# ben-hayes/neural-waveshaping-synthesis

Hardware: AMD Instinct MI355X
Metric: audio_samples_per_sec (higher is better)
Workload: dtype f32 (fp16x2-split MFMA contractions = 22-bit products, fp32 accumulate; FiLM interpolation bf16x3-split MFMA = exact fp32 operands); 1 GPU; NEWT forward, vn checkpoint, FastNEWT LUT, batch 64/GPU x 500 frames (4 s @ 16 kHz), torch.rand F0/control, RNG draws on device; batch_per_gpu=64, frames=500, samples_per_utterance=64000, parallelism=batch-shard x1, exciter_opts=0, streams=2

## Files before the change

### include/nws_hip.h

```cpp
#ifndef NWS_HIP_H
#define NWS_HIP_H

#include <stddef.h>
#include <stdint.h>

#ifdef __cplusplus
extern "C" {
#endif

#define NWS_ABI_VERSION 6

#define NWS_N_HARMONICS 101
#define NWS_N_SHAPERS 64
#define NWS_HIDDEN 128
#define NWS_HOP 128
#define NWS_FIR_LEN 256
#define NWS_N_BANDS 129
#define NWS_FIR_HALF 128
#define NWS_SHAPER_WIDTH 8
#define NWS_FILM_CH 256

enum {
  NWS_OK = 0,
  NWS_ERR_UNSUPPORTED = -1,
  NWS_ERR_BAD_ARG = -2,
  NWS_ERR_WORKSPACE = -3
};

typedef struct NwsWeights {
  const float* gru_w_ih;
  const float* gru_w_hh;
  const float* gru_b_ih;
  const float* gru_b_hh;
  const float* proj_w;
  const float* proj_b;
  const float* mixer_w;
  const float* mixer_b;
  const void* mixer_frags;
  const float* newt_mlp_w[4];
  const float* newt_mlp_b[4];
  const float* newt_ln_g[3];
  const float* newt_ln_b[3];
  const float* hgen_w[4];
  const float* hgen_b[4];
  const float* hgen_ln_g[3];
  const float* hgen_ln_b[3];
  const void* mlp_frags;
  const float* shaper_in_scale;
  const float* shaper_w0;
  const float* shaper_b0;
  const float* shaper_w2;
  const float* shaper_b2;
  const float* shaper_w4;
  const float* shaper_b4;
  const float* shaper_w6;
  const float* shaper_b6;
  const float* shaper_turns;
  const float* lut;
  const float* lut_pairs;
  int32_t lut_size;
  float lut_min;
  float lut_max;
  const float* newt_out_w;
  const float* newt_out_b;
  const float* noise_window;
  int32_t exciter_opts;
  const float* exciter_bound;
} NwsWeights;
#define NWS_EXCITER_VALU_FILM 1
#define NWS_EXCITER_ONE_TERM 2
#define NWS_EXCITER_HYBRID 4
#define NWS_EXCITER_HYBRID_W 8
#define NWS_EXCITER_BANK_NOFRACT 16

int nws_abi_version(void);
size_t nws_sizeof(int which);
const char* nws_error_string(int code);

int nws_selftest_mfma(int32_t* bad_out , void* stream);

int nws_sin(const float* x, float* y, int64_t n, void* stream);

int nws_phase_carry(const float* f0, const float* f0_up, int B, int T, double* carry , void* stream);

int nws_exciter_newt(const NwsWeights* w, const float* f0, const float* f0_up, const double* carry,
                     const float* phase_u, const float* rand_phase, const float* film, int B, int T,
                     float sample_rate, float* exciter_out, float* newt_out, void* stream);
int nws_exciter_newt_add(const NwsWeights* w, const float* f0, const float* f0_up, const double* carry,
                         const float* phase_u, const float* rand_phase, const float* film, const float* add_in, int B,
                         int T, float sample_rate, float* exciter_out, float* newt_out, void* stream);

int nws_control_gru(const NwsWeights* w, const float* control, int B, int C, int T, float* gru_out, void* stream);
int nws_control_gru_state(const NwsWeights* w, const float* control, int B, int C, int T, const float* h0, float* gru_out,
                          float* hT, void* stream);
int nws_control_gru_carry(const NwsWeights* w, const float* control, const float* f0, int B, int C, int T, float* gru_out,
                          double* carry_out, void* stream);
int nws_control_gru_batched(const NwsWeights* w, const float* control, int B, int C, int T, const float* h0, float* gru_out,
                            float* hT, void* stream);

int nws_frame_mlps(const NwsWeights* w, const float* gru_out, const float* fir_design, int B, int T,
                   float* emb_out, float* film_out, float* H_out, float* fir_out, void* stream);

#define NWS_MLP_FRAGS_BYTES 1474560
int nws_mlp_frags(const NwsWeights* w, const float* fir_design , void* frags_out, void* stream);

int nws_fir_design_matrix(const float* window , float* D_out, void* stream);

int nws_fir_noise(const float* fir , const float* noise , const float* add_in ,
                  int B, int T, float* out , void* stream);
int nws_fir_noise_window(const float* fir, const float* noise, int noise_len, int origin, const float* add_in, int B, int T,
                         float* out, void* stream);

int nws_fir_noise_grad(const float* noise , const float* grad_out , int B, int T,
                       float* grad_fir , void* stream);
int nws_fir_from_h_grad(const float* grad_fir , const float* fir_design , int B, int T,
                        float* grad_H , void* stream);
int nws_sum_batch_time(const float* x , int B, int C, int T, float* out , void* stream);

typedef struct NwsReverbPlan {
  int32_t L;
  int32_t N1;
  int32_t N2;
  int32_t Lc;
  int32_t hist;
  int32_t nblk;
  int32_t reserved[2];
} NwsReverbPlan;

int nws_reverb_plan(int N, int ir_len_plus1, NwsReverbPlan* plan );
int nws_reverb_plan_serves(const NwsReverbPlan* plan, int N, int ir_len_plus1);
size_t nws_reverb_table_bytes(const NwsReverbPlan* plan);
size_t nws_reverb_spectrum_bytes(const NwsReverbPlan* plan);
size_t nws_reverb_workspace_bytes(const NwsReverbPlan* plan, int B);
int nws_reverb_build_tables(const NwsReverbPlan* plan, void* tables, void* stream);
int nws_reverb_ir_spectrum(const NwsReverbPlan* plan, const void* tables, const float* ir, int ir_len,
                           void* spectrum, void* workspace, size_t workspace_bytes, void* stream);
int nws_reverb(const NwsReverbPlan* plan, const void* tables, const void* spectrum, const float* x ,
               int B, int N, float* y , void* workspace, size_t workspace_bytes, void* stream);

size_t nws_reverb_grad_workspace_bytes(const NwsReverbPlan* plan, int B, int want_ir);
int nws_reverb_grad_x(const NwsReverbPlan* plan, const void* tables, const void* spectrum, const float* g ,
                      int B, int N, float* dx , void* workspace, size_t workspace_bytes, void* stream);
int nws_reverb_grad_ir(const NwsReverbPlan* plan, const void* tables, const float* x , const float* g ,
                       int B, int N, int ir_len, float* dir , void* workspace, size_t workspace_bytes,
                       void* stream);

int nws_reverb_linear_chunk(const NwsReverbPlan* plan, const void* tables, const void* spectrum, const float* x, int B, int M,
                            const float* tail_in, float* tail_out, int tail_len, float* y, void* workspace,
                            size_t workspace_bytes, void* stream);

size_t nws_stream_state_bytes(int B, int max_frames, int ir_len, const NwsReverbPlan* plan);
int nws_stream_reset(void* state, size_t state_bytes, void* stream);
int nws_stream_out_samples(int K, int first, int final);
long long nws_stream_noise_start(int first, long long frames_seen);
int nws_stream_noise_draws(int K, int first, long long frames_seen);
int nws_stream_step(const NwsWeights* w, const float* fir_design, const NwsReverbPlan* plan, const void* reverb_tables,
                    const void* reverb_spectrum, void* state, size_t state_bytes, int B, int max_frames, const float* f0 ,
                    const float* control , int C, int K, int first, int final, long long frames_seen,
                    long long nz_prev_start, float sample_rate, const float* phase_u, const float* rand_phase,
                    const float* noise_new, const float* noise_all, int noise_all_len, const float* ir, int ir_len,
                    float* out , float* pre_out , void* stream);
int nws_stream_reverb_tail(const NwsReverbPlan* plan, const void* reverb_tables, const void* reverb_spectrum, void* state,
                           size_t state_bytes, int B, int max_frames, int ir_len, float* tail_out ,
                           void* workspace, size_t workspace_bytes, void* stream);

size_t nws_stream_counters_offset(int B, int max_frames, int ir_len);
size_t nws_stream_slot_state_bytes(int B, int max_frames, int ir_len);
#define NWS_SLOT_START 1
#define NWS_SLOT_STOP 2
#define NWS_SLOT_RELEASE 4
#define NWS_SLOT_ACTIVE 8
int nws_stream_step_slots(const NwsWeights* w, const float* fir_design, void* state, size_t state_bytes, int B, int max_frames,
                          const float* f0 , const float* control , int C, int K, long long frames_seen,
                          long long nz_prev_start, float sample_rate, const float* phase_u, const float* rand_phase,
                          const float* noise_new, const float* noise_all, int noise_all_len, const float* ir, int ir_len,
                          const int* events , float* out , float* pre_out ,
                          void* stream);

int nws_oscillator(const float* f0_up, const double* carry, const float* phase_u, const float* rand_phase, int B, int N,
                   float sample_rate, float* out, void* stream);
int nws_newt_apply(const NwsWeights* w, const float* exciter, const float* film, int B, int T, float* out, void* stream);
int nws_td_mlp(const float* x, int B, int in_size, int hidden, int out_size, int depth, int T, const float* const* w,
               const float* const* b, const float* const* ln_g, const float* const* ln_b, float ln_eps, float leaky_slope,
               float* y, void* stream);
int nws_td_layer_norm(const float* x, const float* gain, const float* bias, int B, int C, int T, float eps, float* y,
                      void* stream);
int nws_film(const float* x, const float* gamma, const float* beta, int64_t n, float* y, void* stream);
int nws_fir_from_h(const float* H, const float* fir_design , int B, int T, float* fir_out, void* stream);

int nws_shaper_table(const NwsWeights* w, int table_size, float table_min, float table_max, float* table_out, void* stream);

#define NWS_MIXER_FRAGS_BYTES 28672
int nws_mixer_frags(const float* mixer_w, const float* mixer_b, void* frags_out, void* stream);
int nws_exciter_bound(const float* mixer_w, const float* mixer_b, float* bound_out , void* stream);
#define NWS_SHAPER_TURNS_ROW 176
int nws_shaper_turns(const NwsWeights* w, float* table_out , void* stream);

int nws_lut_pairs(const float* table , int table_size, float* pairs_out , void* stream);

int nws_shaper_apply(const NwsWeights* w, const float* x, int64_t B, int64_t N, float* y, void* stream);

typedef struct NwsForwardAux {
  const float* fir_design;
  const NwsReverbPlan* plan;
  const void* reverb_tables;
  const void* reverb_spectrum;
} NwsForwardAux;

size_t nws_forward_workspace_bytes(const NwsReverbPlan* plan, int B, int T);
int nws_forward(const NwsWeights* w, const NwsForwardAux* aux, const float* f0 , const float* control ,
                int B, int C, int T, float sample_rate, const float* phase_u, const float* rand_phase,
                const float* noise, float* out , void* workspace, size_t workspace_bytes, void* stream);

size_t nws_forward_control_bytes(int B, int T);
int nws_forward_control(const NwsWeights* w, const float* f0, const float* control, int B, int C, int T, int batched_gru,
                        void* workspace, size_t workspace_bytes, void* stream);
int nws_forward_audio(const NwsWeights* w, const NwsForwardAux* aux, const float* f0, int B, int T, float sample_rate,
                      const float* phase_u, const float* rand_phase, const float* noise, float* out, void* workspace,
                      size_t workspace_bytes, void* stream);

int nws_forward_audio_ev(const NwsWeights* w, const NwsForwardAux* aux, const float* f0, int B, int T, float sample_rate,
                         const float* phase_u, const float* rand_phase, const float* noise, float* out, void* workspace,
                         size_t workspace_bytes, void* stream, void* wait_before_exciter, void* record_after_exciter);

int nws_forward_audio_pre(const NwsWeights* w, const NwsForwardAux* aux, const float* f0, int B, int T, float sample_rate,
                          const float* phase_u, const float* rand_phase, const float* noise, void* workspace,
                          size_t workspace_bytes, void* stream);
int nws_forward_reverb_rows(const NwsForwardAux* aux, int B, int T, int row0, int nrows, float* out, void* workspace,
                            size_t workspace_bytes, void* stream);
int nws_forward_audio_blocks(const NwsWeights* w, const NwsForwardAux* aux, const float* f0, int B, int T, float sample_rate,
                             const float* phase_u, const float* rand_phase, const float* noise, float* out, void* workspace,
                             size_t workspace_bytes, void* stream, const int32_t* row0, const int32_t* nrows,
                             void* const* events , int nblocks);

size_t nws_loudness_dft_bytes(int n_fft);
int nws_loudness_dft_matrix(int n_fft, float* dft_out, void* stream);
int nws_loudness_frames(int N, int hop);
size_t nws_loudness_workspace_bytes(int B, int N, int n_fft, int hop);
int nws_loudness(const float* audio, int B, int N, int n_fft, int hop, const float* dft, float amin, float top_db,
                 int normalise, float* out, void* workspace, size_t workspace_bytes, void* stream);

int nws_pyin_frames(int N, int hop);
int nws_pyin_dims(double sample_rate, double fmin, double fmax, int frame_length, int hop, int32_t* dims);
size_t nws_pyin_table_bytes(double sample_rate, double fmin, double fmax, int frame_length, int hop);
int nws_pyin_table(double sample_rate, double fmin, double fmax, int frame_length, int hop, double* table_host);
size_t nws_pyin_workspace_bytes(int B, int N, double sample_rate, double fmin, double fmax, int frame_length, int hop);
int nws_pyin_cmnd(const float* audio, int B, int N, double sample_rate, double fmin, double fmax, int frame_length, int hop,
                  float* yin, void* stream);
int nws_pyin_observe(const float* yin, int B, int T, double sample_rate, double fmin, double fmax, int frame_length, int hop,
                     const double* table, int* cand_bin, double* cand_prob, int* count, double* voiced_prob, void* stream);
int nws_pyin_viterbi(const int* cand_bin, const double* cand_prob, const int* count, const double* voiced_prob, int B, int T,
                     double sample_rate, double fmin, double fmax, int frame_length, int hop, const double* table,
                     int fill_unvoiced, float fill_value, int* states, float* f0, void* workspace, size_t workspace_bytes,
                     void* stream);
int nws_pyin(const float* audio, int B, int N, double sample_rate, double fmin, double fmax, int frame_length, int hop,
             const double* table, int fill_unvoiced, float fill_value, float* f0, double* voiced_prob, int* states,
             void* workspace, size_t workspace_bytes, void* stream);

int nws_resample_dims(int sr_in, int sr_out, int32_t* dims);
int64_t nws_resample_length(int64_t N, int sr_in, int sr_out);
size_t nws_resample_bank_bytes(int sr_in, int sr_out);
int nws_resample_bank(int sr_in, int sr_out, float* bank_host);
int nws_resample(const float* x, int B, int N, int sr_in, int sr_out, const float* bank_dev, float* y, void* stream);

int nws_mfcc_dims(double sample_rate, int n_fft, int n_mfcc, int n_mels, int32_t* dims);
size_t nws_mfcc_table_bytes(double sample_rate, int n_fft, int n_mfcc, int n_mels);
int nws_mfcc_table(double sample_rate, int n_fft, int n_mfcc, int n_mels, float* table_host);
size_t nws_mfcc_workspace_bytes(int B, int N, int n_fft, int hop, int n_mels);
int nws_mfcc(const float* audio, int B, int N, double sample_rate, int n_fft, int hop, int n_mfcc, int n_mels, const float* dft,
             const float* table, float* out, void* workspace, size_t workspace_bytes, void* stream);

#define NWS_STFT_LOSS_MAX_RES 8
size_t nws_stft_loss_dft_bytes(int n_fft, int win_length);
int nws_stft_loss_dft_matrix(int n_fft, int win_length, float* dft_out, void* stream);
size_t nws_stft_loss_workspace_bytes(int B, int N, int R, const int* n_ffts, const int* hops);
int nws_stft_loss(const float* x, const float* y, int B, int N, int R, const int* n_ffts, const int* hops, const int* win_lengths,
                  const float* const* dfts, float w_sc, float w_log_mag, float w_lin_mag, float eps, float* out, void* workspace,
                  size_t workspace_bytes, void* stream);

size_t nws_stft_grad_workspace_bytes(int B, int N, int R, const int* n_ffts, const int* hops, const int* win_lengths);
int nws_stft_grad(const float* x, const float* y, int B, int N, int R, const int* n_ffts, const int* hops, const int* win_lengths,
                  const float* const* dfts, float w_sc, float w_log_mag, float w_lin_mag, float eps, float* grad_out, void* workspace,
                  size_t workspace_bytes, void* stream);

typedef struct NwsShaperDesc {
  int32_t n_shapers, width, depth, lut_size;
  float lut_min, lut_max;
  const float* in_scale;
  const float* w[8];
  const float* b[8];
  const float* lut;
} NwsShaperDesc;

typedef struct NwsGenericModel {
  int32_t control_size;
  int32_t gru_hidden, embedding, n_harmonics, n_shapers;
  int32_t hop;
  int32_t newt_mlp_depth;
  int32_t hgen_depth, hgen_hidden;
  int32_t fir_len;
  int32_t out_channels;
  int32_t ir_len;
  float ln_eps, leaky_slope;
  const float *gru_w_ih, *gru_w_hh, *gru_b_ih, *gru_b_hh;
  const float *proj_w, *proj_b;
  const float *mixer_w, *mixer_b;
  const float* newt_mlp_w[8];
  const float* newt_mlp_b[8];
  const float* newt_ln_g[8];
  const float* newt_ln_b[8];
  const float* hgen_w[8];
  const float* hgen_b[8];
  const float* hgen_ln_g[8];
  const float* hgen_ln_b[8];
  const float *newt_out_w, *newt_out_b;
  const float* noise_window;
  const float* ir;
  NwsShaperDesc shaper;
} NwsGenericModel;

size_t nws_g_gru_workspace_bytes(int hidden);
int nws_g_gru(const float* w_ih, const float* w_hh, const float* b_ih, const float* b_hh, const float* control, int B,
              int C_total, int C_in, int hidden, int T, const float* h0, float* out, float* hT, void* workspace,
              size_t workspace_bytes, void* stream);
int nws_g_bth_to_bht(const float* x, int B, int T, int H, float* y, void* stream);
int nws_g_phase(const float* f0, const float* f0_up, int B, int T, int hop, float sample_rate, float* f0_up_out,
                float* phase_out, void* stream);
int nws_g_upsample(const float* x, int64_t rows, int T, int hop, float* y, void* stream);
int nws_g_oscillator(const float* f0_up, const float* phase, const float* phase_u, const float* rand_phase, int K, int B, int N,
                     float sample_rate, float* out, void* stream);
int nws_g_conv1x1(const float* x, const float* w, const float* bias, int B, int Cin, int Cout, int N, float* y, void* stream);
int nws_g_shaper_apply(const NwsShaperDesc* d, const float* x, int64_t rows, int64_t N, float* y, void* stream);
int nws_g_shaper_table(const NwsShaperDesc* d, int table_size, float table_min, float table_max, float* table_out, void* stream);
int nws_g_film_shaper(const NwsShaperDesc* d, const float* exciter, const float* film, int B, int T, int hop, float* out,
                      void* stream);
int nws_g_fir_design(const float* H, const float* window, int fir_len, int B, int T, float* fir_out, void* stream);
int nws_g_fir_noise(const float* fir, const float* noise, int fir_len, int hop, int B, int T, const float* add_in,
                    int add_channels, float* out, void* stream);
int nws_g_reverb_direct(const float* x, const float* ir, int ir_len, int B, int N, float* y, void* stream);

size_t nws_forward_generic_workspace_bytes(const NwsGenericModel* m, int B, int T);
int nws_forward_generic(const NwsGenericModel* m, const float* f0, const float* control, int B, int C, int T, float sample_rate,
                        const float* phase_u, const float* rand_phase, const float* noise, const NwsReverbPlan* plan,
                        const void* reverb_tables, const void* reverb_spectrum, void* reverb_workspace,
                        size_t reverb_workspace_bytes, float* out, void* workspace, size_t workspace_bytes, void* stream);


#define NWS_N_STAGES 6
int nws_profile_begin(int slots, unsigned stage_mask);
int nws_profile_collect(float* ms_out , int* n_out );
int nws_profile_end(void);

int nws_peer_push(int n, void* const* dst, const void* src, size_t bytes, void* const* streams, void* const* events);
int nws_events_wait(int n, void* const* events);
int nws_streams_wait(int n, void* const* streams);

int nws_queue_probe(void* stream_hold, void* stream_touch, int groups, int spin_us, unsigned long long* scratch, float* frac_out );

#ifdef __cplusplus
}
#endif
#endif
```

### neural-waveshaping-synthesis_amd/_cops.py

```python
from __future__ import annotations

import ctypes as C

import torch

from . import _lib
from ._lib import NwsForwardAux, NwsGenericModel, NwsReverbPlan, NwsShaperDesc, NwsWeights, check, ptr

HOP = _lib.HOP


def _stream(dev):
    return torch.cuda.current_stream(dev).cuda_stream


def _struct(desc: torch.Tensor, cls):
    return cls.from_buffer_copy(desc.numpy())


def _plan(plan: torch.Tensor | None):
    return NwsReverbPlan(*plan.tolist()[:6]) if plan is not None else None


def _ref(struct):
    return C.byref(struct) if struct is not None else None


def _aux(fir_design, plan, tables, spectrum) -> NwsForwardAux:
    aux = NwsForwardAux()
    aux.fir_design = ptr(fir_design)
    aux.plan = C.pointer(_plan(plan))
    aux.reverb_tables = ptr(tables)
    aux.reverb_spectrum = ptr(spectrum)
    return aux


def _new(like: torch.Tensor, *shape, dtype=torch.float32):
    return torch.empty(shape, dtype=dtype, device=like.device)


def _ptrs(tensors):
    return (C.c_void_p * max(1, len(tensors)))(*[t.data_ptr() for t in tensors])


def _pyin_dims(cfg, table=None):
    dims = (C.c_int32 * 8)()
    L = _lib.lib()
    if L.nws_pyin_dims(*cfg, dims) != 0:
        raise RuntimeError(f"pyin: unsupported configuration (sample_rate, fmin, fmax, frame_length, hop) = {cfg}: at most 512 "
                           "lags (frame_length <= 1024), 1024 pitch bins and a transition window of 127; hop <= frame_length")
    n = L.nws_pyin_table_bytes(*cfg) // 8
    if isinstance(table, torch.Tensor) and (not table.is_cuda or table.dtype != torch.float64 or table.numel() != n):
        raise RuntimeError("pyin: table does not belong to this configuration (expected a float64 CUDA tensor of nws_pyin_table)")
    return (*dims, n)


def _resample_dims(sr_in, sr_out):
    dims = (C.c_int32 * 6)()
    if not (1 <= sr_in < 2 ** 31 and 1 <= sr_out < 2 ** 31) or _lib.lib().nws_resample_dims(sr_in, sr_out, dims) != 0:
        raise RuntimeError(f"resample: unsupported rates {sr_in} -> {sr_out}: integers >= 1 whose weight bank (sr_out / gcd rows) "
                           "stays below 64 MB")
    return tuple(dims)


def _mfcc_dims(sample_rate, n_fft, n_mfcc, n_mels):
    dims = (C.c_int32 * 8)()
    ok = all(0 <= v < 2 ** 31 for v in (n_fft, n_mfcc, n_mels))
    if not ok or _lib.lib().nws_mfcc_dims(sample_rate, n_fft, n_mfcc, n_mels, dims) != 0:
        raise RuntimeError(f"mfcc: unsupported configuration (sample_rate {sample_rate}, n_fft {n_fft}, n_mfcc {n_mfcc}, n_mels "
                           f"{n_mels}): sample_rate > 0, n_fft a power of two in [64, 2048], 1 <= n_mfcc <= n_mels <= 1024")
    return tuple(dims)


class CtypesOps:
    def abi_version(self):
        return int(_lib.lib().nws_abi_version())

    def forward(self, wdesc, f0, control, phase_u, rand_phase, noise, fir_design, plan, reverb_tables, reverb_spectrum,
                workspace, sample_rate):
        B, Cc, T = control.shape
        aux = _aux(fir_design, plan, reverb_tables, reverb_spectrum)
        with torch.cuda.device(f0.device):
            out = _new(f0, B, T * HOP)
            check(_lib.lib().nws_forward(C.byref(_struct(wdesc, NwsWeights)), C.byref(aux), ptr(f0), ptr(control), B, Cc, T,
                                         sample_rate, ptr(phase_u), ptr(rand_phase), ptr(noise), ptr(out), ptr(workspace),
                                         workspace.numel(), _stream(f0.device)), "nws_forward")
        return out

    def forward_control(self, wdesc, f0, control, workspace, batched_gru):
        B, Cc, T = control.shape
        with torch.cuda.device(f0.device):
            check(_lib.lib().nws_forward_control(C.byref(_struct(wdesc, NwsWeights)), ptr(f0), ptr(control), B, Cc, T,
                                                 1 if batched_gru else 0, ptr(workspace), workspace.numel(), _stream(f0.device)),
                  "nws_forward_control")

    def forward_audio(self, wdesc, f0, phase_u, rand_phase, noise, fir_design, plan, reverb_tables, reverb_spectrum, workspace,
                      sample_rate, out, wait_event, record_event):
        B, _, T = f0.shape
        aux = _aux(fir_design, plan, reverb_tables, reverb_spectrum)
        with torch.cuda.device(f0.device):
            if out is None:
                out = _new(f0, B, T * HOP)
            check(_lib.lib().nws_forward_audio_ev(C.byref(_struct(wdesc, NwsWeights)), C.byref(aux), ptr(f0), B, T, sample_rate,
                                                  ptr(phase_u), ptr(rand_phase), ptr(noise), ptr(out), ptr(workspace),
                                                  workspace.numel(), _stream(f0.device), wait_event or None, record_event or None),
                  "nws_forward_audio_ev")
        return out

    def forward_audio_pre(self, wdesc, f0, phase_u, rand_phase, noise, fir_design, plan, reverb_tables, reverb_spectrum,
                          workspace, sample_rate):
        B, _, T = f0.shape
        aux = _aux(fir_design, plan, reverb_tables, reverb_spectrum)
        with torch.cuda.device(f0.device):
            check(_lib.lib().nws_forward_audio_pre(C.byref(_struct(wdesc, NwsWeights)), C.byref(aux), ptr(f0), B, T, sample_rate,
                                                   ptr(phase_u), ptr(rand_phase), ptr(noise), ptr(workspace), workspace.numel(),
                                                   _stream(f0.device)), "nws_forward_audio_pre")

    def forward_audio_blocks(self, wdesc, f0, phase_u, rand_phase, noise, fir_design, plan, reverb_tables, reverb_spectrum,
                             workspace, sample_rate, out, row0, nrows, events):
        B, _, T = f0.shape
        n = len(row0)
        aux = _aux(fir_design, plan, reverb_tables, reverb_spectrum)
        with torch.cuda.device(f0.device):
            check(_lib.lib().nws_forward_audio_blocks(C.byref(_struct(wdesc, NwsWeights)), C.byref(aux), ptr(f0), B, T, sample_rate,
                                                      ptr(phase_u), ptr(rand_phase), ptr(noise), ptr(out), ptr(workspace),
                                                      workspace.numel(), _stream(f0.device), (C.c_int32 * n)(*row0),
                                                      (C.c_int32 * n)(*nrows), (C.c_void_p * n)(*events) if events else None, n),
                  "nws_forward_audio_blocks")

    def forward_reverb_rows(self, fir_design, plan, reverb_tables, reverb_spectrum, workspace, T, row0, nrows, out):
        aux = _aux(fir_design, plan, reverb_tables, reverb_spectrum)
        with torch.cuda.device(out.device):
            check(_lib.lib().nws_forward_reverb_rows(C.byref(aux), out.shape[0], T, row0, nrows, ptr(out), ptr(workspace),
                                                     workspace.numel(), _stream(out.device)), "nws_forward_reverb_rows")

    def phase_carry(self, f0, f0_up):
        src = f0 if f0 is not None else f0_up
        B = src.shape[0]
        T = src.shape[-1] if f0 is not None else src.shape[-1] // HOP
        with torch.cuda.device(src.device):
            carry = _new(src, B, T * HOP // 32, dtype=torch.float64)
            check(_lib.lib().nws_phase_carry(ptr(f0), ptr(f0_up), B, T, ptr(carry), _stream(src.device)), "nws_phase_carry")
        return carry

    def exciter_newt(self, wdesc, f0, f0_up, carry, phase_u, rand_phase, film, sample_rate, want_exciter, want_newt):
        src = f0 if f0 is not None else f0_up
        B = src.shape[0]
        T = src.shape[-1] if f0 is not None else src.shape[-1] // HOP
        with torch.cuda.device(src.device):
            exc = _new(src, B, _lib.N_SHAPERS, T * HOP) if want_exciter else None
            out = _new(src, B, T * HOP) if want_newt else None
            check(_lib.lib().nws_exciter_newt(C.byref(_struct(wdesc, NwsWeights)), ptr(f0), ptr(f0_up), ptr(carry), ptr(phase_u),
                                              ptr(rand_phase), ptr(film), B, T, sample_rate, ptr(exc), ptr(out),
                                              _stream(src.device)), "nws_exciter_newt")
        return exc, out

    def oscillator(self, f0_up, phase_u, rand_phase, sample_rate):
        B, N = f0_up.shape
        with torch.cuda.device(f0_up.device):
            st = _stream(f0_up.device)
            carry = _new(f0_up, B, N // 32, dtype=torch.float64)
            out = _new(f0_up, B, _lib.N_HARMONICS, N)
            check(_lib.lib().nws_phase_carry(None, ptr(f0_up), B, N // HOP, ptr(carry), st), "nws_phase_carry")
            check(_lib.lib().nws_oscillator(ptr(f0_up), ptr(carry), ptr(phase_u), ptr(rand_phase), B, N, sample_rate, ptr(out), st),
                  "nws_oscillator")
        return out

    def control_gru(self, wdesc, control, h0, batched):
        B, Cc, T = control.shape
        fn = _lib.lib().nws_control_gru_batched if batched else _lib.lib().nws_control_gru_state
        with torch.cuda.device(control.device):
            out = _new(control, B, T, _lib.HIDDEN)
            hT = _new(control, B, _lib.HIDDEN)
            check(fn(C.byref(_struct(wdesc, NwsWeights)), ptr(control), B, Cc, T, ptr(h0), ptr(out), ptr(hT),
                     _stream(control.device)), "nws_control_gru")
        return out, hT

    def frame_mlps(self, wdesc, gru_out, fir_design, want_emb, want_H):
        B, T, _ = gru_out.shape
        with torch.cuda.device(gru_out.device):
            emb = _new(gru_out, B, _lib.HIDDEN, T) if want_emb else None
            film = _new(gru_out, B, T, _lib.FILM_CH)
            H = _new(gru_out, B, T, _lib.N_BANDS) if want_H else None
            fir = _new(gru_out, B, T, _lib.FIR_HALF)
            check(_lib.lib().nws_frame_mlps(C.byref(_struct(wdesc, NwsWeights)), ptr(gru_out), ptr(fir_design), B, T, ptr(emb),
                                            ptr(film), ptr(H), ptr(fir), _stream(gru_out.device)), "nws_frame_mlps")
        return emb, film, H, fir

    def fir_noise(self, fir, noise, add_in, origin):
        B, T, _ = fir.shape
        with torch.cuda.device(fir.device):
            out = _new(fir, B, T * HOP)
            if origin < 0:
                check(_lib.lib().nws_fir_noise(ptr(fir), ptr(noise), ptr(add_in), B, T, ptr(out), _stream(fir.device)), "nws_fir_noise")
            else:
                check(_lib.lib().nws_fir_noise_window(ptr(fir), ptr(noise), noise.numel(), origin, ptr(add_in), B, T, ptr(out),
                                                      _stream(fir.device)), "nws_fir_noise_window")
        return out

    def fir_from_h(self, H, fir_design):
        B, _, T = H.shape
        with torch.cuda.device(H.device):
            fir = _new(H, B, T, _lib.FIR_HALF)
            check(_lib.lib().nws_fir_from_h(ptr(H), ptr(fir_design), B, T, ptr(fir), _stream(H.device)), "nws_fir_from_h")
        return fir

    def fir_noise_grad(self, noise, grad_out):
        B, N = grad_out.shape
        T = N // HOP
        if N != T * HOP or T < 2 or noise.numel() != N - 1:
            raise RuntimeError(f"fir_noise_grad: grad_out {tuple(grad_out.shape)} must be (B, 128 T) with T >= 2 and noise "
                               f"{tuple(noise.shape)} its {N - 1} samples")
        with torch.cuda.device(grad_out.device):
            grad_fir = _new(grad_out, B, T, _lib.FIR_HALF)
            check(_lib.lib().nws_fir_noise_grad(ptr(noise), ptr(grad_out), B, T, ptr(grad_fir), _stream(grad_out.device)),
                  "nws_fir_noise_grad")
        return grad_fir

    def fir_from_h_grad(self, grad_fir, fir_design):
        B, T, _ = grad_fir.shape
        with torch.cuda.device(grad_fir.device):
            grad_H = _new(grad_fir, B, _lib.N_BANDS, T)
            check(_lib.lib().nws_fir_from_h_grad(ptr(grad_fir), ptr(fir_design), B, T, ptr(grad_H), _stream(grad_fir.device)),
                  "nws_fir_from_h_grad")
        return grad_H

    def sum_batch_time(self, x):
        B, Cc, T = x.shape
        with torch.cuda.device(x.device):
            out = _new(x, Cc)
            check(_lib.lib().nws_sum_batch_time(ptr(x), B, Cc, T, ptr(out), _stream(x.device)), "nws_sum_batch_time")
        return out

    def reverb(self, plan, tables, spectrum, x):
        B, N = x.shape
        p = _plan(plan)
        with torch.cuda.device(x.device):
            nbytes = _lib.lib().nws_reverb_workspace_bytes(C.byref(p), B)
            ws = _new(x, nbytes, dtype=torch.uint8)
            y = torch.empty_like(x)
            check(_lib.lib().nws_reverb(C.byref(p), ptr(tables), ptr(spectrum), ptr(x), B, N, ptr(y), ptr(ws), nbytes,
                                        _stream(x.device)), "nws_reverb")
        return y

    def reverb_grad_x(self, plan, tables, spectrum, grad_out):
        B, N = grad_out.shape
        p = _plan(plan)
        with torch.cuda.device(grad_out.device):
            nbytes = _lib.lib().nws_reverb_grad_workspace_bytes(C.byref(p), B, 0)
            ws = _new(grad_out, nbytes, dtype=torch.uint8)
            dx = torch.empty_like(grad_out)
            check(_lib.lib().nws_reverb_grad_x(C.byref(p), ptr(tables), ptr(spectrum), ptr(grad_out), B, N, ptr(dx), ptr(ws), nbytes,
                                               _stream(grad_out.device)), "nws_reverb_grad_x")
        return dx

    def reverb_grad_ir(self, plan, tables, x, grad_out, ir_len):
        B, N = x.shape
        if tuple(grad_out.shape) != (B, N):
            raise RuntimeError(f"reverb_grad_ir: x {tuple(x.shape)} and grad_out {tuple(grad_out.shape)} differ in shape")
        p = _plan(plan)
        with torch.cuda.device(x.device):
            nbytes = _lib.lib().nws_reverb_grad_workspace_bytes(C.byref(p), B, 1)
            ws = _new(x, nbytes, dtype=torch.uint8)
            dir_ = _new(x, ir_len)
            check(_lib.lib().nws_reverb_grad_ir(C.byref(p), ptr(tables), ptr(x), ptr(grad_out), B, N, ir_len, ptr(dir_), ptr(ws),
                                                nbytes, _stream(x.device)), "nws_reverb_grad_ir")
        return dir_

    def reverb_linear_chunk(self, plan, tables, spectrum, x, tail_in):
        B, M = x.shape
        p = _plan(plan)
        with torch.cuda.device(x.device):
            nfl = (2 * ((B + 1) // 2) + B) * p.L
            ws = _new(x, nfl)
            y, tail_out = torch.empty_like(x), torch.empty_like(tail_in)
            check(_lib.lib().nws_reverb_linear_chunk(C.byref(p), ptr(tables), ptr(spectrum), ptr(x), B, M, ptr(tail_in),
                                                     ptr(tail_out), tail_in.shape[1], ptr(y), ptr(ws), nfl * 4, _stream(x.device)),
                  "nws_reverb_linear_chunk")
        return y, tail_out

    def shaper_apply(self, wdesc, x):
        with torch.cuda.device(x.device):
            y = torch.empty_like(x)
            check(_lib.lib().nws_shaper_apply(C.byref(_struct(wdesc, NwsWeights)), ptr(x), x.shape[0], x.shape[2], ptr(y),
                                              _stream(x.device)), "nws_shaper_apply")
        return y

    def shaper_table(self, wdesc, like, size, tmin, tmax):
        with torch.cuda.device(like.device):
            table = _new(like, _lib.N_SHAPERS, size)
            check(_lib.lib().nws_shaper_table(C.byref(_struct(wdesc, NwsWeights)), size, tmin, tmax, ptr(table), _stream(like.device)),
                  "nws_shaper_table")
        return table

    def newt_apply(self, wdesc, exciter, film):
        B, _, N = exciter.shape
        T = film.shape[2]
        if film.shape[1] != _lib.FILM_CH or N != T * HOP:
            raise RuntimeError(f"NEWT: exciter {tuple(exciter.shape)} and FiLM parameters {tuple(film.shape)} disagree")
        with torch.cuda.device(exciter.device):
            out = _new(exciter, B, 1, N)
            check(_lib.lib().nws_newt_apply(C.byref(_struct(wdesc, NwsWeights)), ptr(exciter), ptr(film), B, T, ptr(out),
                                            _stream(exciter.device)), "nws_newt_apply")
        return out

    def td_mlp(self, x, weights, biases, ln_w, ln_b, eps, slope):
        B, in_size, T = x.shape
        hidden, out_size = weights[0].shape[0], weights[-1].shape[0]
        with torch.cuda.device(x.device):
            y = _new(x, B, out_size, T)
            check(_lib.lib().nws_td_mlp(ptr(x), B, in_size, hidden, out_size, len(weights), T, _ptrs(weights), _ptrs(biases),
                                        _ptrs(ln_w), _ptrs(ln_b), eps, slope, ptr(y), _stream(x.device)), "nws_td_mlp")
        return y

    def td_layer_norm(self, x, weight, bias, eps):
        with torch.cuda.device(x.device):
            y = torch.empty_like(x)
            check(_lib.lib().nws_td_layer_norm(ptr(x), ptr(weight), ptr(bias), x.shape[0], x.shape[1], x.shape[2], eps, ptr(y),
                                               _stream(x.device)), "nws_td_layer_norm")
        return y

    def film(self, x, gamma, beta):
        with torch.cuda.device(x.device):
            y = torch.empty_like(x)
            check(_lib.lib().nws_film(ptr(x), ptr(gamma), ptr(beta), x.numel(), ptr(y), _stream(x.device)), "nws_film")
        return y

    def sine(self, x):
        with torch.cuda.device(x.device):
            y = torch.empty_like(x)
            check(_lib.lib().nws_sin(ptr(x), ptr(y), x.numel(), _stream(x.device)), "nws_sin")
        return y

    def loudness(self, audio, dft, n_fft, hop, amin, top_db, normalise):
        B, N = audio.shape
        L = _lib.lib()
        with torch.cuda.device(audio.device):
            ws = _new(audio, L.nws_loudness_workspace_bytes(B, N, n_fft, hop), dtype=torch.uint8)
            out = _new(audio, B, L.nws_loudness_frames(N, hop))
            check(L.nws_loudness(ptr(audio), B, N, n_fft, hop, ptr(dft), amin, top_db, 1 if normalise else 0, ptr(out), ptr(ws),
                                 ws.numel(), _stream(audio.device)), "nws_loudness")
        return out

    def pyin_table(self, sample_rate, fmin, fmax, frame_length, hop):
        cfg = (sample_rate, fmin, fmax, frame_length, hop)
        table = torch.empty(_pyin_dims(cfg)[8], dtype=torch.float64)
        check(_lib.lib().nws_pyin_table(*cfg, table.data_ptr()), "nws_pyin_table")
        return table

    def pyin_cmnd(self, audio, sample_rate, fmin, fmax, frame_length, hop):
# ... 297 lines not shown
```

### neural-waveshaping-synthesis_amd/_lib.py

```python
from __future__ import annotations

import ctypes as C
import os

_HERE = os.path.dirname(os.path.abspath(__file__))
LIB_PATH = os.path.join(_HERE, "libnws_hip.so")

PROBE_LIB_PATH = os.path.join(_HERE, "libnws_probe.so")

ABI_VERSION = 6
EXCITER_VALU_FILM = 1
EXCITER_ONE_TERM = 2
EXCITER_HYBRID = 4
EXCITER_HYBRID_W = 8
EXCITER_BANK_NOFRACT = 16
N_HARMONICS = 101
N_SHAPERS = 64
HIDDEN = 128
HOP = 128
FIR_LEN = 256
FIR_HALF = 128
MLP_FRAGS_BYTES = 1474560
N_BANDS = 129
FILM_CH = 256
SHAPER_WIDTH = 8
SHAPER_TURNS_ROW = 176
FIR_DESIGN_COLS = 132

_fp = C.c_void_p


class NwsWeights(C.Structure):
    _fields_ = [
        ("gru_w_ih", _fp), ("gru_w_hh", _fp), ("gru_b_ih", _fp), ("gru_b_hh", _fp),
        ("proj_w", _fp), ("proj_b", _fp),
        ("mixer_w", _fp), ("mixer_b", _fp), ("mixer_frags", _fp),
        ("newt_mlp_w", _fp * 4), ("newt_mlp_b", _fp * 4), ("newt_ln_g", _fp * 3), ("newt_ln_b", _fp * 3),
        ("hgen_w", _fp * 4), ("hgen_b", _fp * 4), ("hgen_ln_g", _fp * 3), ("hgen_ln_b", _fp * 3),
        ("mlp_frags", _fp),
        ("shaper_in_scale", _fp),
        ("shaper_w0", _fp), ("shaper_b0", _fp), ("shaper_w2", _fp), ("shaper_b2", _fp),
        ("shaper_w4", _fp), ("shaper_b4", _fp), ("shaper_w6", _fp), ("shaper_b6", _fp), ("shaper_turns", _fp),
        ("lut", _fp), ("lut_pairs", _fp), ("lut_size", C.c_int32), ("lut_min", C.c_float), ("lut_max", C.c_float),
        ("newt_out_w", _fp), ("newt_out_b", _fp),
        ("noise_window", _fp),
        ("exciter_opts", C.c_int32),
        ("exciter_bound", _fp),
    ]


class NwsReverbPlan(C.Structure):
    _fields_ = [("L", C.c_int32), ("N1", C.c_int32), ("N2", C.c_int32), ("Lc", C.c_int32), ("hist", C.c_int32), ("nblk", C.c_int32),
                ("reserved", C.c_int32 * 2)]

    def as_tensor(self):
        import torch
        return torch.tensor([self.L, self.N1, self.N2, self.Lc, self.hist, self.nblk, 0, 0], dtype=torch.int32)


class NwsForwardAux(C.Structure):
    _fields_ = [("fir_design", _fp), ("plan", C.POINTER(NwsReverbPlan)), ("reverb_tables", _fp),
                ("reverb_spectrum", _fp)]


class NwsShaperDesc(C.Structure):
    _fields_ = [("n_shapers", C.c_int32), ("width", C.c_int32), ("depth", C.c_int32), ("lut_size", C.c_int32),
                ("lut_min", C.c_float), ("lut_max", C.c_float),
                ("in_scale", _fp), ("w", _fp * 8), ("b", _fp * 8), ("lut", _fp)]


class NwsGenericModel(C.Structure):
    _fields_ = [("control_size", C.c_int32), ("gru_hidden", C.c_int32), ("embedding", C.c_int32), ("n_harmonics", C.c_int32),
                ("n_shapers", C.c_int32), ("hop", C.c_int32), ("newt_mlp_depth", C.c_int32), ("hgen_depth", C.c_int32),
                ("hgen_hidden", C.c_int32), ("fir_len", C.c_int32), ("out_channels", C.c_int32), ("ir_len", C.c_int32),
                ("ln_eps", C.c_float), ("leaky_slope", C.c_float),
                ("gru_w_ih", _fp), ("gru_w_hh", _fp), ("gru_b_ih", _fp), ("gru_b_hh", _fp),
                ("proj_w", _fp), ("proj_b", _fp), ("mixer_w", _fp), ("mixer_b", _fp),
                ("newt_mlp_w", _fp * 8), ("newt_mlp_b", _fp * 8), ("newt_ln_g", _fp * 8), ("newt_ln_b", _fp * 8),
                ("hgen_w", _fp * 8), ("hgen_b", _fp * 8), ("hgen_ln_g", _fp * 8), ("hgen_ln_b", _fp * 8),
                ("newt_out_w", _fp), ("newt_out_b", _fp), ("noise_window", _fp), ("ir", _fp),
                ("shaper", NwsShaperDesc)]


_PYIN_CFG = (C.c_double, C.c_double, C.c_double, C.c_int, C.c_int)

_MFCC_CFG = (C.c_double, C.c_int, C.c_int, C.c_int)

_PROTOTYPES = {
    "nws_abi_version": (C.c_int, []),
    "nws_sizeof": (C.c_size_t, [C.c_int]),
    "nws_error_string": (C.c_char_p, [C.c_int]),
    "nws_selftest_mfma": (C.c_int, [_fp, _fp]),
    "nws_peer_push": (C.c_int, [C.c_int, C.POINTER(C.c_void_p), _fp, C.c_size_t, C.POINTER(C.c_void_p), C.POINTER(C.c_void_p)]),
    "nws_events_wait": (C.c_int, [C.c_int, C.POINTER(C.c_void_p)]),
    "nws_streams_wait": (C.c_int, [C.c_int, C.POINTER(C.c_void_p)]),
    "nws_queue_probe": (C.c_int, [_fp, _fp, C.c_int, C.c_int, _fp, C.POINTER(C.c_float)]),
    "nws_debug_queue_busy": (C.c_int, [C.c_int, C.c_int, _fp, _fp]),
    "nws_sin": (C.c_int, [_fp, _fp, C.c_int64, _fp]),
    "nws_phase_carry": (C.c_int, [_fp, _fp, C.c_int, C.c_int, _fp, _fp]),
    "nws_exciter_newt": (C.c_int, [C.POINTER(NwsWeights), _fp, _fp, _fp, _fp, _fp, _fp, C.c_int, C.c_int, C.c_float,
                                   _fp, _fp, _fp]),
    "nws_exciter_newt_add": (C.c_int, [C.POINTER(NwsWeights), _fp, _fp, _fp, _fp, _fp, _fp, _fp, C.c_int, C.c_int, C.c_float,
                                       _fp, _fp, _fp]),
    "nws_control_gru": (C.c_int, [C.POINTER(NwsWeights), _fp, C.c_int, C.c_int, C.c_int, _fp, _fp]),
    "nws_control_gru_state": (C.c_int, [C.POINTER(NwsWeights), _fp, C.c_int, C.c_int, C.c_int, _fp, _fp, _fp, _fp]),
    "nws_control_gru_carry": (C.c_int, [C.POINTER(NwsWeights), _fp, _fp, C.c_int, C.c_int, C.c_int, _fp, _fp, _fp]),
    "nws_control_gru_batched": (C.c_int, [C.POINTER(NwsWeights), _fp, C.c_int, C.c_int, C.c_int, _fp, _fp, _fp, _fp]),
    "nws_frame_mlps": (C.c_int, [C.POINTER(NwsWeights), _fp, _fp, C.c_int, C.c_int, _fp, _fp, _fp, _fp, _fp]),
    "nws_mlp_frags": (C.c_int, [C.POINTER(NwsWeights), _fp, _fp, _fp]),
    "nws_debug_frame_mlps_kernel": (C.c_int, [C.c_int]),
    "nws_fir_design_matrix": (C.c_int, [_fp, _fp, _fp]),
    "nws_fir_noise": (C.c_int, [_fp, _fp, _fp, C.c_int, C.c_int, _fp, _fp]),
    "nws_fir_noise_window": (C.c_int, [_fp, _fp, C.c_int, C.c_int, _fp, C.c_int, C.c_int, _fp, _fp]),
    "nws_fir_noise_grad": (C.c_int, [_fp, _fp, C.c_int, C.c_int, _fp, _fp]),
    "nws_fir_from_h_grad": (C.c_int, [_fp, _fp, C.c_int, C.c_int, _fp, _fp]),
    "nws_sum_batch_time": (C.c_int, [_fp, C.c_int, C.c_int, C.c_int, _fp, _fp]),
    "nws_reverb_linear_chunk": (C.c_int, [C.POINTER(NwsReverbPlan), _fp, _fp, _fp, C.c_int, C.c_int, _fp, _fp, C.c_int, _fp, _fp,
                                          C.c_size_t, _fp]),
    "nws_reverb_plan": (C.c_int, [C.c_int, C.c_int, C.POINTER(NwsReverbPlan)]),
    "nws_reverb_plan_serves": (C.c_int, [C.POINTER(NwsReverbPlan), C.c_int, C.c_int]),
    "nws_reverb_table_bytes": (C.c_size_t, [C.POINTER(NwsReverbPlan)]),
    "nws_reverb_spectrum_bytes": (C.c_size_t, [C.POINTER(NwsReverbPlan)]),
    "nws_reverb_workspace_bytes": (C.c_size_t, [C.POINTER(NwsReverbPlan), C.c_int]),
    "nws_reverb_build_tables": (C.c_int, [C.POINTER(NwsReverbPlan), _fp, _fp]),
    "nws_reverb_ir_spectrum": (C.c_int, [C.POINTER(NwsReverbPlan), _fp, _fp, C.c_int, _fp, _fp, C.c_size_t, _fp]),
    "nws_reverb": (C.c_int, [C.POINTER(NwsReverbPlan), _fp, _fp, _fp, C.c_int, C.c_int, _fp, _fp, C.c_size_t, _fp]),
    "nws_reverb_grad_workspace_bytes": (C.c_size_t, [C.POINTER(NwsReverbPlan), C.c_int, C.c_int]),
    "nws_reverb_grad_x": (C.c_int, [C.POINTER(NwsReverbPlan), _fp, _fp, _fp, C.c_int, C.c_int, _fp, _fp, C.c_size_t, _fp]),
    "nws_reverb_grad_ir": (C.c_int, [C.POINTER(NwsReverbPlan), _fp, _fp, _fp, C.c_int, C.c_int, C.c_int, _fp, _fp, C.c_size_t, _fp]),
    "nws_shaper_table": (C.c_int, [C.POINTER(NwsWeights), C.c_int, C.c_float, C.c_float, _fp, _fp]),
    "nws_mixer_frags": (C.c_int, [_fp, _fp, _fp, _fp]),
    "nws_exciter_bound": (C.c_int, [_fp, _fp, _fp, _fp]),
    "nws_shaper_turns": (C.c_int, [_fp, _fp, _fp]),
    "nws_lut_pairs": (C.c_int, [_fp, C.c_int, _fp, _fp]),
    "nws_shaper_apply": (C.c_int, [C.POINTER(NwsWeights), _fp, C.c_int64, C.c_int64, _fp, _fp]),
    "nws_forward_workspace_bytes": (C.c_size_t, [C.POINTER(NwsReverbPlan), C.c_int, C.c_int]),
    "nws_forward": (C.c_int, [C.POINTER(NwsWeights), C.POINTER(NwsForwardAux), _fp, _fp, C.c_int, C.c_int, C.c_int,
                              C.c_float, _fp, _fp, _fp, _fp, _fp, C.c_size_t, _fp]),
    "nws_forward_control_bytes": (C.c_size_t, [C.c_int, C.c_int]),
    "nws_forward_control": (C.c_int, [C.POINTER(NwsWeights), _fp, _fp, C.c_int, C.c_int, C.c_int, C.c_int, _fp, C.c_size_t, _fp]),
    "nws_forward_audio": (C.c_int, [C.POINTER(NwsWeights), C.POINTER(NwsForwardAux), _fp, C.c_int, C.c_int, C.c_float,
                                    _fp, _fp, _fp, _fp, _fp, C.c_size_t, _fp]),
    "nws_forward_audio_ev": (C.c_int, [C.POINTER(NwsWeights), C.POINTER(NwsForwardAux), _fp, C.c_int, C.c_int, C.c_float,
                                       _fp, _fp, _fp, _fp, _fp, C.c_size_t, _fp, _fp, _fp]),
    "nws_forward_audio_pre": (C.c_int, [C.POINTER(NwsWeights), C.POINTER(NwsForwardAux), _fp, C.c_int, C.c_int, C.c_float,
                                        _fp, _fp, _fp, _fp, C.c_size_t, _fp]),
    "nws_forward_reverb_rows": (C.c_int, [C.POINTER(NwsForwardAux), C.c_int, C.c_int, C.c_int, C.c_int, _fp, _fp, C.c_size_t, _fp]),
    "nws_forward_audio_blocks": (C.c_int, [C.POINTER(NwsWeights), C.POINTER(NwsForwardAux), _fp, C.c_int, C.c_int, C.c_float, _fp, _fp, _fp, _fp,
                                           _fp, C.c_size_t, _fp, C.POINTER(C.c_int32), C.POINTER(C.c_int32), C.POINTER(C.c_void_p), C.c_int]),
    "nws_loudness_dft_bytes": (C.c_size_t, [C.c_int]),
    "nws_loudness_dft_matrix": (C.c_int, [C.c_int, _fp, _fp]),
    "nws_loudness_frames": (C.c_int, [C.c_int, C.c_int]),
    "nws_loudness_workspace_bytes": (C.c_size_t, [C.c_int, C.c_int, C.c_int, C.c_int]),
    "nws_loudness": (C.c_int, [_fp, C.c_int, C.c_int, C.c_int, C.c_int, _fp, C.c_float, C.c_float, C.c_int, _fp, _fp,
                               C.c_size_t, _fp]),
    "nws_pyin_frames": (C.c_int, [C.c_int, C.c_int]),
    "nws_pyin_dims": (C.c_int, [*_PYIN_CFG, C.POINTER(C.c_int32)]),
    "nws_pyin_table_bytes": (C.c_size_t, [*_PYIN_CFG]),
    "nws_pyin_table": (C.c_int, [*_PYIN_CFG, C.c_void_p]),
    "nws_pyin_workspace_bytes": (C.c_size_t, [C.c_int, C.c_int, *_PYIN_CFG]),
    "nws_pyin_cmnd": (C.c_int, [_fp, C.c_int, C.c_int, *_PYIN_CFG, _fp, _fp]),
    "nws_pyin_observe": (C.c_int, [_fp, C.c_int, C.c_int, *_PYIN_CFG, _fp, _fp, _fp, _fp, _fp, _fp]),
    "nws_pyin_viterbi": (C.c_int, [_fp, _fp, _fp, _fp, C.c_int, C.c_int, *_PYIN_CFG, _fp, C.c_int, C.c_float, _fp, _fp, _fp,
                                   C.c_size_t, _fp]),
    "nws_pyin": (C.c_int, [_fp, C.c_int, C.c_int, *_PYIN_CFG, _fp, C.c_int, C.c_float, _fp, _fp, _fp, _fp, C.c_size_t, _fp]),
    "nws_resample_dims": (C.c_int, [C.c_int, C.c_int, C.POINTER(C.c_int32)]),
    "nws_resample_length": (C.c_int64, [C.c_int64, C.c_int, C.c_int]),
    "nws_resample_bank_bytes": (C.c_size_t, [C.c_int, C.c_int]),
    "nws_resample_bank": (C.c_int, [C.c_int, C.c_int, C.c_void_p]),
    "nws_resample": (C.c_int, [_fp, C.c_int, C.c_int, C.c_int, C.c_int, _fp, _fp, _fp]),
    "nws_mfcc_dims": (C.c_int, [*_MFCC_CFG, C.POINTER(C.c_int32)]),
    "nws_mfcc_table_bytes": (C.c_size_t, [*_MFCC_CFG]),
    "nws_mfcc_table": (C.c_int, [*_MFCC_CFG, C.c_void_p]),
    "nws_mfcc_workspace_bytes": (C.c_size_t, [C.c_int, C.c_int, C.c_int, C.c_int, C.c_int]),
    "nws_mfcc": (C.c_int, [_fp, C.c_int, C.c_int, C.c_double, C.c_int, C.c_int, C.c_int, C.c_int, _fp, _fp, _fp, _fp, C.c_size_t,
                           _fp]),
    "nws_stft_loss_dft_bytes": (C.c_size_t, [C.c_int, C.c_int]),
    "nws_stft_loss_dft_matrix": (C.c_int, [C.c_int, C.c_int, _fp, _fp]),
    "nws_stft_loss_workspace_bytes": (C.c_size_t, [C.c_int, C.c_int, C.c_int, C.POINTER(C.c_int), C.POINTER(C.c_int)]),
    "nws_stft_loss": (C.c_int, [_fp, _fp, C.c_int, C.c_int, C.c_int, C.POINTER(C.c_int), C.POINTER(C.c_int), C.POINTER(C.c_int),
                                C.POINTER(_fp), C.c_float, C.c_float, C.c_float, C.c_float, _fp, _fp, C.c_size_t, _fp]),
    "nws_stft_grad_workspace_bytes": (C.c_size_t, [C.c_int, C.c_int, C.c_int, C.POINTER(C.c_int), C.POINTER(C.c_int),
                                                   C.POINTER(C.c_int)]),
    "nws_stft_grad": (C.c_int, [_fp, _fp, C.c_int, C.c_int, C.c_int, C.POINTER(C.c_int), C.POINTER(C.c_int), C.POINTER(C.c_int),
                                C.POINTER(_fp), C.c_float, C.c_float, C.c_float, C.c_float, _fp, _fp, C.c_size_t, _fp]),
    "nws_oscillator": (C.c_int, [_fp, _fp, _fp, _fp, C.c_int, C.c_int, C.c_float, _fp, _fp]),
    "nws_newt_apply": (C.c_int, [C.POINTER(NwsWeights), _fp, _fp, C.c_int, C.c_int, _fp, _fp]),
    "nws_td_mlp": (C.c_int, [_fp, C.c_int, C.c_int, C.c_int, C.c_int, C.c_int, C.c_int, C.POINTER(_fp), C.POINTER(_fp),
                             C.POINTER(_fp), C.POINTER(_fp), C.c_float, C.c_float, _fp, _fp]),
    "nws_td_layer_norm": (C.c_int, [_fp, _fp, _fp, C.c_int, C.c_int, C.c_int, C.c_float, _fp, _fp]),
    "nws_film": (C.c_int, [_fp, _fp, _fp, C.c_int64, _fp, _fp]),
    "nws_fir_from_h": (C.c_int, [_fp, _fp, C.c_int, C.c_int, _fp, _fp]),
    "nws_g_gru_workspace_bytes": (C.c_size_t, [C.c_int]),
    "nws_g_gru": (C.c_int, [_fp, _fp, _fp, _fp, _fp, C.c_int, C.c_int, C.c_int, C.c_int, C.c_int, _fp, _fp, _fp, _fp,
                            C.c_size_t, _fp]),
    "nws_g_bth_to_bht": (C.c_int, [_fp, C.c_int, C.c_int, C.c_int, _fp, _fp]),
    "nws_g_phase": (C.c_int, [_fp, _fp, C.c_int, C.c_int, C.c_int, C.c_float, _fp, _fp, _fp]),
    "nws_g_upsample": (C.c_int, [_fp, C.c_int64, C.c_int, C.c_int, _fp, _fp]),
    "nws_g_oscillator": (C.c_int, [_fp, _fp, _fp, _fp, C.c_int, C.c_int, C.c_int, C.c_float, _fp, _fp]),
    "nws_g_conv1x1": (C.c_int, [_fp, _fp, _fp, C.c_int, C.c_int, C.c_int, C.c_int, _fp, _fp]),
    "nws_g_shaper_apply": (C.c_int, [C.POINTER(NwsShaperDesc), _fp, C.c_int64, C.c_int64, _fp, _fp]),
    "nws_g_shaper_table": (C.c_int, [C.POINTER(NwsShaperDesc), C.c_int, C.c_float, C.c_float, _fp, _fp]),
    "nws_g_film_shaper": (C.c_int, [C.POINTER(NwsShaperDesc), _fp, _fp, C.c_int, C.c_int, C.c_int, _fp, _fp]),
    "nws_g_fir_design": (C.c_int, [_fp, _fp, C.c_int, C.c_int, C.c_int, _fp, _fp]),
    "nws_g_fir_noise": (C.c_int, [_fp, _fp, C.c_int, C.c_int, C.c_int, C.c_int, _fp, C.c_int, _fp, _fp]),
    "nws_g_reverb_direct": (C.c_int, [_fp, _fp, C.c_int, C.c_int, C.c_int, _fp, _fp]),
    "nws_forward_generic_workspace_bytes": (C.c_size_t, [C.POINTER(NwsGenericModel), C.c_int, C.c_int]),
    "nws_debug_generic_exciter_plan": (C.c_int, [C.POINTER(NwsGenericModel), C.c_int, C.c_int, C.POINTER(C.c_int)]),
    "nws_debug_generic_gru_plan": (C.c_int, [C.c_int, C.c_int, C.POINTER(C.c_int)]),
    "nws_forward_generic": (C.c_int, [C.POINTER(NwsGenericModel), _fp, _fp, C.c_int, C.c_int, C.c_int, C.c_float, _fp, _fp, _fp,
                                      C.POINTER(NwsReverbPlan), _fp, _fp, _fp, C.c_size_t, _fp, _fp, C.c_size_t, _fp]),
    "nws_stream_state_bytes": (C.c_size_t, [C.c_int, C.c_int, C.c_int, C.POINTER(NwsReverbPlan)]),
    "nws_stream_reset": (C.c_int, [_fp, C.c_size_t, _fp]),
    "nws_stream_out_samples": (C.c_int, [C.c_int, C.c_int, C.c_int]),
    "nws_stream_noise_start": (C.c_longlong, [C.c_int, C.c_longlong]),
    "nws_stream_noise_draws": (C.c_int, [C.c_int, C.c_int, C.c_longlong]),
    "nws_stream_step": (C.c_int, [C.POINTER(NwsWeights), _fp, C.POINTER(NwsReverbPlan), _fp, _fp, _fp, C.c_size_t, C.c_int, C.c_int,
                                  _fp, _fp, C.c_int, C.c_int, C.c_int, C.c_int, C.c_longlong, C.c_longlong, C.c_float, _fp, _fp,
                                  _fp, _fp, C.c_int, _fp, C.c_int, _fp, _fp, _fp]),
    "nws_stream_counters_offset": (C.c_size_t, [C.c_int, C.c_int, C.c_int]),
    "nws_stream_slot_state_bytes": (C.c_size_t, [C.c_int, C.c_int, C.c_int]),
    "nws_stream_step_slots": (C.c_int, [C.POINTER(NwsWeights), _fp, _fp, C.c_size_t, C.c_int, C.c_int, _fp, _fp, C.c_int, C.c_int,
                                        C.c_longlong, C.c_longlong, C.c_float, _fp, _fp, _fp, _fp, C.c_int, _fp, C.c_int, _fp, _fp,
                                        _fp, _fp]),
    "nws_stream_reverb_tail": (C.c_int, [C.POINTER(NwsReverbPlan), _fp, _fp, _fp, C.c_size_t, C.c_int, C.c_int, C.c_int, _fp, _fp,
                                         C.c_size_t, _fp]),
    "nws_profile_begin": (C.c_int, [C.c_int, C.c_uint]),
    "nws_profile_collect": (C.c_int, [C.POINTER(C.c_float), C.POINTER(C.c_int)]),
    "nws_profile_end": (C.c_int, []),
}

_PROBE_PROTOTYPES = {
    "nws_coexec_pk_probe": (C.c_int, [C.c_int, C.c_int, _fp, _fp]),
    "nws_coexec_pk_probe2": (C.c_int, [C.c_int, C.c_int, _fp, _fp]),
    "nws_coexec_pk_probe_mixed": (C.c_int, [C.c_int, C.c_int, C.c_int, _fp, _fp, _fp]),
    "nws_coexec_mfma_load": (C.c_int, [C.c_int, C.c_int, C.c_int, _fp, _fp]),
}

STAGE_NAMES = ("phase_carry", "control_gru", "frame_mlps", "exciter_newt", "fir_noise", "reverb")

EXPORTED_SYMBOLS = tuple(_PROTOTYPES)
PROBE_SYMBOLS = tuple(_PROBE_PROTOTYPES)

_lib = None
_probe = None


class NwsError(RuntimeError):
    pass


def lib():
    global _lib
    if _lib is None:
        if not os.path.exists(LIB_PATH):
            raise NwsError(
                f"{LIB_PATH} not found: build the HIP kernels first "
                "(python __graft_entry__.py build, or python neural-waveshaping-synthesis_amd/build.py). "
                "There is no CPU/PyTorch fallback for the NEWT forward path.")
        handle = C.CDLL(LIB_PATH)
        for name, (res, args) in _PROTOTYPES.items():
            fn = getattr(handle, name)
            fn.restype = res
            fn.argtypes = args
        if handle.nws_abi_version() != ABI_VERSION:
            raise NwsError(f"{LIB_PATH} has ABI version {handle.nws_abi_version()}, this package binds version "
                           f"{ABI_VERSION}: rebuild it (python __graft_entry__.py build)")
        for which, struct in enumerate((NwsWeights, NwsReverbPlan, NwsForwardAux, NwsShaperDesc, NwsGenericModel)):
            if handle.nws_sizeof(which) != C.sizeof(struct):
                raise NwsError(f"struct layout mismatch for {struct.__name__}: library {handle.nws_sizeof(which)} B, "
                               f"binding {C.sizeof(struct)} B")
        _lib = handle
    return _lib


def probe_lib():
    global _probe
    if _probe is None:
        if not os.path.exists(PROBE_LIB_PATH):
            raise NwsError(f"{PROBE_LIB_PATH} not found: python neural-waveshaping-synthesis_amd/build.py builds it next to libnws_hip.so")
        handle = C.CDLL(PROBE_LIB_PATH)
        for name, (res, args) in _PROBE_PROTOTYPES.items():
            fn = getattr(handle, name)
            fn.restype = res
            fn.argtypes = args
        _probe = handle
    return _probe


def check(rc: int, what: str = ""):
    if rc != 0:
        msg = lib().nws_error_string(rc)
        raise NwsError(f"{what or 'nws call'} failed ({rc}): {msg.decode() if msg else '?'}")
# ... 13 lines not shown
```

### neural-waveshaping-synthesis_amd/csrc/fir_noise.hip

```cpp
#include "nws_common.h"
#include "fir_spectral_fft.h"

template <>
struct SpOps<f32x2> {
  static __device__ __forceinline__ f32x2 fma(f32x2 a, f32x2 b, f32x2 c) { return __builtin_elementwise_fma(a, b, c); }
  static __device__ __forceinline__ f32x2 of(float v) { return f32x2{v, v}; }
  static __device__ __forceinline__ f32x2 at(const float* p) { return *reinterpret_cast<const f32x2*>(p); }
};

namespace {

constexpr int kL = NWS_FIR_LEN;
constexpr int kHop = NWS_HOP;
constexpr int kHalf = NWS_FIR_HALF;
constexpr int kHopsPerBlock = 4;

struct NoiseLds {
  float taps[kHopsPerBlock + 1][kL];
  float taps1[kHopsPerBlock + 1][kL];
  float sig[(kHopsPerBlock + 1) * kHop + kHop];
};

__device__ __forceinline__ float padded_noise(const float* __restrict__ noise, int len, int origin, int i) {
  int s = i - origin;
  if (s < 0) s = -s;
  if (s > len - 1) s = 2 * (len - 1) - s;
  s = s < 0 ? 0 : s;
  return noise[s];
}

__device__ __forceinline__ float row_noise(const float* __restrict__ noise, int lo, int hi, int origin, int i) {
  int s = i - origin;
  if (s < lo) s = 2 * lo - s;
  if (s > hi) s = 2 * hi - s;
  s = s < 0 ? 0 : s;
  return noise[s];
}

template <bool ROWS>
__global__ __launch_bounds__(256) void fir_noise_kernel(const float* __restrict__ fir, const float* __restrict__ noise,
                                                        const float* __restrict__ add_in, int T, int len, int origin,
                                                        float* __restrict__ out, const int4* __restrict__ rows) {
  __shared__ __attribute__((aligned(16))) NoiseLds L;
  const int tid = threadIdx.x, lane = tid & 63, wave = tid >> 6;
  const int half = lane >> 5, q = lane & 31;
  const int b = blockIdx.y;
  const int t0 = blockIdx.x * kHopsPerBlock;
  const int N = T * kHop;
  int4 rb = make_int4(0, 0, 0, 0);
  if constexpr (ROWS) rb = rows[b];
  const int t_lo = ROWS ? rb.z : 0;

  for (int e = tid; e < (kHopsPerBlock + 1) * kL; e += 256) {
    const int fr = e >> 8, k = e & 255;
    const int t = t0 - 1 + fr;
    const int d = k >= kHalf ? k - kHalf : kHalf - k;
    const float v = (t >= t_lo && t < T && d < kHalf) ? fir[((size_t)b * T + t) * kHalf + d] : 0.0f;
    L.taps[fr][k] = v;
    L.taps1[fr][(k + 1) & 255] = v;
  }
  for (int e = tid; e < (kHopsPerBlock + 1) * kHop + kHop; e += 256) {
    const int i = (t0 - 1) * kHop + e;
    float v = 0.0f;
    if (i >= 0 && i < N + kL - 1) v = ROWS ? row_noise(noise, rb.x, rb.y, origin, i) : padded_noise(noise, len, origin, i);
    L.sig[e] = v;
  }
  __syncthreads();

  const int t = t0 + wave;
  if (t >= T) return;
  const int slot = wave + 1 - half;
  const int nb = half * kHop + 4 * q;
  const float* f = &L.sig[slot * kHop];
  const float* h = L.taps[slot];

  const float* h1 = L.taps1[slot];
  f32x2 a0 = {0.0f, 0.0f}, a1 = {0.0f, 0.0f}, a2 = {0.0f, 0.0f}, a3 = {0.0f, 0.0f};
  float4 hi0 = *reinterpret_cast<const float4*>(&h[nb & 255]);
  float4 hi1 = *reinterpret_cast<const float4*>(&h1[nb & 255]);
#pragma unroll 4
  for (int m0 = 0; m0 < kL; m0 += 4) {
    const float4 lo0 = *reinterpret_cast<const float4*>(&h[(nb - m0 - 4) & 255]);
    const float4 lo1 = *reinterpret_cast<const float4*>(&h1[(nb - m0 - 4) & 255]);
    const float4 fv = *reinterpret_cast<const float4*>(&f[m0]);
    const f32x2 fs0 = {fv.y, fv.x}, fs1 = {fv.w, fv.z};
    a1 = fma2(fs0, f32x2{hi0.x, hi0.y}, a1);
    a3 = fma2(fs0, f32x2{hi0.z, hi0.w}, a3);
    a1 = fma2(fs1, f32x2{lo0.z, lo0.w}, a1);
    a3 = fma2(fs1, f32x2{hi0.x, hi0.y}, a3);
    a0 = fma2(fs0, f32x2{hi1.x, hi1.y}, a0);
    a2 = fma2(fs0, f32x2{hi1.z, hi1.w}, a2);
    a0 = fma2(fs1, f32x2{lo1.z, lo1.w}, a0);
    a2 = fma2(fs1, f32x2{hi1.x, hi1.y}, a2);
    hi0 = lo0;
    hi1 = lo1;
  }
  const float y0 = a0.x + a0.y, y1 = a1.x + a1.y, y2 = a2.x + a2.y, y3 = a3.x + a3.y;
  const float o0 = y0 + nws_swap_halves(y0);
  const float o1 = y1 + nws_swap_halves(y1);
  const float o2 = y2 + nws_swap_halves(y2);
  const float o3 = y3 + nws_swap_halves(y3);
  if (half == 0) {
    const float inv = t == t_lo ? 1.0f : 0.5f;
    const size_t o = (size_t)b * N + (size_t)t * kHop + 4 * q;
    float4 r = make_float4(o0 * inv, o1 * inv, o2 * inv, o3 * inv);
    if (add_in != nullptr) {
      const float4 a = *reinterpret_cast<const float4*>(&add_in[o]);
      r.x = a.x + r.x;
      r.y = a.y + r.y;
      r.z = a.z + r.z;
      r.w = a.w + r.w;
    }
    *reinterpret_cast<float4*>(&out[o]) = r;
  }
}

constexpr int kSpWaves = 4;
constexpr int kSpUtt = 2 * kSpWaves;
constexpr int kSpPairs = 4;
constexpr int kSpHops = 2 * kSpPairs - 1;

struct SpectralLds {
  float4 sd[kSpPairs][9][16];
  float4 tw[256];
  f32x2 x[kSpWaves][kSpPairs * kSpPlane];
};

__device__ __forceinline__ void sp_wave_sync() {
  __builtin_amdgcn_fence(__ATOMIC_RELEASE, "wavefront");
  __builtin_amdgcn_wave_barrier();
  __builtin_amdgcn_fence(__ATOMIC_ACQUIRE, "wavefront");
}

template <class T>
__device__ __forceinline__ void sp_transpose(T (&v)[16], T* x, int l) {
#pragma unroll
  for (int k = 0; k < 16; ++k) x[k * kSpRow + l] = v[k];
  sp_wave_sync();
#pragma unroll
  for (int j = 0; j < 16; ++j) v[j] = x[l * kSpRow + j];
  sp_wave_sync();
}
template <bool INV, class T>
__device__ __forceinline__ void sp_fft256(C16T<T>& z, const float* tw, T* x, int l) {
  sp_pass1<INV>(z, tw);
  sp_transpose(z.re, x, l);
  sp_transpose(z.im, x, l);
  sp_dft16<INV>(z);
}

__device__ __forceinline__ f32x2 sp_shfl(f32x2 v, int src) { return f32x2{__shfl(v.x, src, 64), __shfl(v.y, src, 64)}; }
__device__ __forceinline__ f32x2 sp_select(bool c, f32x2 a, f32x2 b) { return f32x2{c ? a.x : b.x, c ? a.y : b.y}; }

__device__ __forceinline__ void sp_filter_spectrum(C16T<f32x2>& z, const f32x2 (&ua)[8], const f32x2 (&ub)[8], const float* tw,
                                                   f32x2* x, int lane, int l) {
  const int src = (lane & 48) | ((16 - l) & 15);
  const f32x2 zero = {0.0f, 0.0f};
#pragma unroll
  for (int j = 0; j < 8; ++j) {
    z.re[j] = ua[j];
    z.im[j] = ub[j];
  }
#pragma unroll
  for (int j = 8; j < 16; ++j) {
    const f32x2 ma = sp_shfl(ua[15 - j], src), mb = sp_shfl(ub[15 - j], src);
    const f32x2 oa = j == 8 ? zero : ua[(16 - j) & 7], ob = j == 8 ? zero : ub[(16 - j) & 7];
    z.re[j] = sp_select(l == 0, oa, ma);
    z.im[j] = sp_select(l == 0, ob, mb);
  }
  sp_fft256<false>(z, tw, x, l);
}

__global__ __launch_bounds__(64 * kSpWaves, 3) void fir_noise_spectral_kernel(const float* __restrict__ fir,
                                                                             const float* __restrict__ noise,
                                                                             const float* __restrict__ add_in, int B, int T, int len,
                                                                             int origin, float* __restrict__ out, int nruns, int total) {
  __shared__ __attribute__((aligned(16))) SpectralLds L;
  const int tid = threadIdx.x, lane = tid & 63, wave = tid >> 6;
  const int g = lane >> 4, l = lane & 15;
  const int per_xcd = gridDim.x >> 3;
  const int id = (blockIdx.x & 7) * per_xcd + (blockIdx.x >> 3);
  if (id >= total) return;
  const int run = id % nruns;
  const int b0 = (id / nruns) * kSpUtt + 2 * wave, b1 = b0 + 1;
  const int t0 = run * kSpHops;
  const int ta = t0 - 1 + 2 * g, tb = ta + 1;
  const int N = T * kHop;
  const bool oka = ta >= 0 && ta < T, okb = tb < T;
  const int tac = ta < 0 ? 0 : (ta < T ? ta : T - 1), tbc = tb < T ? tb : T - 1;

  const int bc0 = b0 < B ? b0 : B - 1, bc1 = b1 < B ? b1 : B - 1;
  const float* rowa0 = &fir[((size_t)bc0 * T + tac) * kHalf + l];
  const float* rowb0 = &fir[((size_t)bc0 * T + tbc) * kHalf + l];
  const float* rowa1 = &fir[((size_t)bc1 * T + tac) * kHalf + l];
  const float* rowb1 = &fir[((size_t)bc1 * T + tbc) * kHalf + l];
  f32x2 ua[8], ub[8];
#pragma unroll
  for (int j = 0; j < 8; ++j) {
    ua[j] = f32x2{rowa0[16 * j], rowa1[16 * j]};
    ub[j] = f32x2{rowb0[16 * j], rowb1[16 * j]};
  }
  {
    float c, s;
    sp_twiddle((tid & 15) * (tid >> 4), c, s);
    L.tw[tid] = make_float4(c, c, s, s);
  }
  const float* tw = reinterpret_cast<const float*>(&L.tw[l]);
  __syncthreads();

  f32x2* x = &L.x[wave][g * kSpPlane];
  if (wave == 0) {
    C16 z;
    float* xs = reinterpret_cast<float*>(x);
#pragma unroll
    for (int j = 0; j < 16; ++j) {
      const int i0 = kHop * ta + 16 * j + l, i1 = i0 + kHop;
      const bool in0 = i0 >= 0 && i0 < N + kL - 1, in1 = i1 >= 0 && i1 < N + kL - 1;
      const float v0 = padded_noise(noise, len, origin, in0 ? i0 : origin);
      const float v1 = padded_noise(noise, len, origin, in1 ? i1 : origin);
      z.re[j] = in0 ? v0 : 0.0f;
      z.im[j] = in1 ? v1 : 0.0f;
    }
    sp_fft256<false>(z, tw, xs, l);
    float mr[16], mi[16];
    auto mirror = [&](const float (&v)[16], float (&m)[16]) {
#pragma unroll
      for (int j = 0; j < 16; ++j) xs[l + 16 * j] = v[j];
      sp_wave_sync();
#pragma unroll
      for (int j = 0; j < 16; ++j) m[j] = xs[(256 - (l + 16 * j)) & 255];
      sp_wave_sync();
    };
    mirror(z.re, mr);
    mirror(z.im, mi);
    const float c = (l & 1) ? -(1.0f / 512.0f) : (1.0f / 512.0f);
#pragma unroll
    for (int j = 0; j < 9; ++j)
      L.sd[g][j][l] = make_float4(c * (z.re[j] + mr[j]), c * (z.im[j] - mi[j]), c * (z.re[j] - mr[j]), c * (z.im[j] + mi[j]));
  }
  const f32x2 zero = {0.0f, 0.0f};
#pragma unroll
  for (int j = 0; j < 8; ++j) {
    ua[j] = sp_select(oka, ua[j], zero);
    ub[j] = sp_select(okb, ub[j], zero);
  }
  C16T<f32x2> z;
  sp_filter_spectrum(z, ua, ub, tw, x, lane, l);
  __syncthreads();

  const bool has_add = add_in != nullptr;
  const bool sta = g > 0 && ta < T, stb = tb < T;
  const size_t oa0 = (size_t)bc0 * N + (size_t)tac * kHop + l, ob0 = (size_t)bc0 * N + (size_t)tbc * kHop + l;
  const size_t oa1 = (size_t)bc1 * N + (size_t)tac * kHop + l, ob1 = (size_t)bc1 * N + (size_t)tbc * kHop + l;
  f32x2 adda[8], addb[8];
  if (has_add) {
#pragma unroll
    for (int j = 0; j < 8; ++j) {
      adda[j] = f32x2{add_in[oa0 + 16 * j], add_in[oa1 + 16 * j]};
      addb[j] = f32x2{add_in[ob0 + 16 * j], add_in[ob1 + 16 * j]};
    }
  }
  const float4* sdm = &L.sd[g][l == 0 ? 1 : 0][(16 - l) & 15];
#pragma unroll
  for (int j = 0; j < 16; ++j) {
    const f32x2 ga = z.re[j], gb = z.im[j];
    if (j < 9) {
      const float4 sd = L.sd[g][j][l];
      z.re[j] = f32x2{fmaf(ga.x, sd.x, gb.x * sd.z), fmaf(ga.y, sd.x, gb.y * sd.z)};
      z.im[j] = f32x2{fmaf(ga.x, sd.y, gb.x * sd.w), fmaf(ga.y, sd.y, gb.y * sd.w)};
    } else {
      const float4 sd = sdm[(15 - j) * 16];
      z.re[j] = f32x2{fmaf(ga.x, sd.x, -(gb.x * sd.z)), fmaf(ga.y, sd.x, -(gb.y * sd.z))};
      z.im[j] = f32x2{fmaf(gb.x, sd.w, -(ga.x * sd.y)), fmaf(gb.y, sd.w, -(ga.y * sd.y))};
    }
  }
  sp_fft256<true>(z, tw, x, l);
  const float invb = tb == 0 ? 1.0f : 0.5f;
  f32x2 ha[8], hb[8];
#pragma unroll
  for (int j = 0; j < 8; ++j) {
    const f32x2 ya0 = sp_select(oka, z.re[j], zero), ya1 = sp_select(oka, z.re[j + 8], zero);
    const f32x2 yb0 = sp_select(okb, z.im[j], zero), yb1 = sp_select(okb, z.im[j + 8], zero);
    const f32x2 prev = sp_shfl(yb1, (lane - 16) & 63);
    ha[j] = (ya0 + prev) * 0.5f;
    hb[j] = (yb0 + ya1) * invb;
    if (has_add) {
      ha[j] = adda[j] + ha[j];
      hb[j] = addb[j] + hb[j];
    }
  }
  if (sta) {
    if (b0 < B) {
#pragma unroll
      for (int j = 0; j < 8; ++j) out[oa0 + 16 * j] = ha[j].x;
    }
    if (b1 < B) {
#pragma unroll
      for (int j = 0; j < 8; ++j) out[oa1 + 16 * j] = ha[j].y;
    }
  }
  if (stb) {
    if (b0 < B) {
#pragma unroll
      for (int j = 0; j < 8; ++j) out[ob0 + 16 * j] = hb[j].x;
    }
    if (b1 < B) {
#pragma unroll
      for (int j = 0; j < 8; ++j) out[ob1 + 16 * j] = hb[j].y;
    }
  }
}

}

extern "C" int nws_fir_noise_window(const float* fir, const float* noise, int noise_len, int origin, const float* add_in,
                                    int B, int T, float* out, void* stream) {
  if (!fir || !noise || !out || B <= 0 || T <= 0 || noise_len < 2 || origin < 0) return NWS_ERR_BAD_ARG;
  if (B > 65535) return NWS_ERR_UNSUPPORTED;
  if (B >= 16) {
    const long long nruns = (T + kSpHops - 1) / kSpHops, total = nruns * ((B + kSpUtt - 1) / kSpUtt);
    if (total > (1ll << 30)) return NWS_ERR_UNSUPPORTED;
    const dim3 grid((unsigned)(8 * ((total + 7) / 8)));
    fir_noise_spectral_kernel<<<grid, 64 * kSpWaves, 0, (hipStream_t)stream>>>(fir, noise, add_in, B, T, noise_len, origin, out,
                                                                             (int)nruns, (int)total);
    NWS_CHECK_LAUNCH();
    return NWS_OK;
  }
  const dim3 grid((T + kHopsPerBlock - 1) / kHopsPerBlock, B);
  fir_noise_kernel<false><<<grid, 256, 0, (hipStream_t)stream>>>(fir, noise, add_in, T, noise_len, origin, out, nullptr);
  NWS_CHECK_LAUNCH();
  return NWS_OK;
}

extern "C" int nws_fir_noise_window_rows(const float* fir, const float* noise, int origin, const int4* rows, int B, int T,
                                         float* out, void* stream) {
  if (!fir || !noise || !out || !rows || B <= 0 || T <= 0 || origin < 0) return NWS_ERR_BAD_ARG;
  if (B > 65535) return NWS_ERR_UNSUPPORTED;
  const dim3 grid((T + kHopsPerBlock - 1) / kHopsPerBlock, B);
  fir_noise_kernel<true><<<grid, 256, 0, (hipStream_t)stream>>>(fir, noise, nullptr, T, 0, origin, out, rows);
  NWS_CHECK_LAUNCH();
  return NWS_OK;
}

extern "C" int nws_fir_noise(const float* fir, const float* noise, const float* add_in, int B, int T, float* out,
                             void* stream) {
  return nws_fir_noise_window(fir, noise, T * kHop - 1, kL / 2, add_in, B, T, out, stream);
}
```

### neural-waveshaping-synthesis_amd/csrc/forward.hip

```cpp
#include "nws_common.h"

namespace {

struct Carve {
  char* p;
  size_t left;
  bool ok = true;
  void* take(size_t bytes) {
    bytes = (bytes + 255) & ~size_t(255);
    if (bytes > left) {
      ok = false;
      return nullptr;
    }
    void* r = p;
    p += bytes;
    left -= bytes;
    return r;
  }
};

size_t aligned(size_t b) { return (b + 255) & ~size_t(255); }

constexpr int kStages = 6;
struct Profile {
  int slots = 0;
  int used = 0;
  unsigned mask = 0;
  hipEvent_t* ev = nullptr;
} g_prof;

inline hipEvent_t* prof_events(int stage) {
  if (g_prof.ev == nullptr || g_prof.used >= g_prof.slots || !(g_prof.mask & (1u << stage))) return nullptr;
  return g_prof.ev + ((size_t)g_prof.used * kStages + stage) * 2;
}

}

extern "C" {

size_t nws_forward_workspace_bytes(const NwsReverbPlan* plan, int B, int T) {
  if (!plan || B <= 0 || T <= 0) return 0;
  const size_t N = (size_t)T * NWS_HOP;
  size_t total = 0;
  total += aligned((size_t)B * (N / 32) * sizeof(double));
  total += aligned((size_t)B * T * NWS_HIDDEN * sizeof(float));
  total += aligned((size_t)B * T * NWS_FILM_CH * sizeof(float));
  total += aligned((size_t)B * T * NWS_FIR_HALF * sizeof(float));
  total += aligned((size_t)B * N * sizeof(float));
  total += aligned((size_t)B * N * sizeof(float));
  total += aligned(nws_reverb_workspace_bytes(plan, B));
  return total;
}

}

namespace {

struct Arena {
  double* carry;
  float *gru_out, *film, *fir, *noise_out, *pre;
  void* rv_ws;
  size_t rv_bytes;
  bool ok;
};

Arena carve_arena(const NwsReverbPlan* plan, void* workspace, size_t bytes, int B, int T, bool head_only) {
  const size_t N = (size_t)T * NWS_HOP;
  Carve cv{static_cast<char*>(workspace), bytes};
  Arena a{};
  a.carry = static_cast<double*>(cv.take((size_t)B * (N / 32) * sizeof(double)));
  a.gru_out = static_cast<float*>(cv.take((size_t)B * T * NWS_HIDDEN * sizeof(float)));
  if (!head_only) {
    a.film = static_cast<float*>(cv.take((size_t)B * T * NWS_FILM_CH * sizeof(float)));
    a.fir = static_cast<float*>(cv.take((size_t)B * T * NWS_FIR_HALF * sizeof(float)));
    a.noise_out = static_cast<float*>(cv.take((size_t)B * N * sizeof(float)));
    a.pre = static_cast<float*>(cv.take((size_t)B * N * sizeof(float)));
    a.rv_bytes = nws_reverb_workspace_bytes(plan, B);
    a.rv_ws = cv.take(a.rv_bytes);
  }
  a.ok = cv.ok;
  return a;
}

#define NWS_STAGE(idx, call)                                   \
  do {                                                         \
    hipEvent_t* e__ = prof_events(idx);                        \
    if (e__) (void)hipEventRecord(e__[0], st);                 \
    rc = (call);                                               \
    if (e__) (void)hipEventRecord(e__[1], st);                 \
    if (rc != NWS_OK) return rc;                               \
  } while (0)

int control_half(const NwsWeights* w, const float* f0, const float* control, int B, int C, int T, int batched_gru,
                 const Arena& a, void* stream) {
  hipStream_t st = (hipStream_t)stream;
  int rc = NWS_OK;
  if (batched_gru) {
    NWS_STAGE(0, nws_phase_carry(f0, nullptr, B, T, a.carry, stream));
    NWS_STAGE(1, nws_control_gru_batched(w, control, B, C, T, nullptr, a.gru_out, nullptr, stream));
  } else {
    NWS_STAGE(0, NWS_OK);
    NWS_STAGE(1, nws_control_gru_carry(w, control, f0, B, C, T, a.gru_out, a.carry, stream));
  }
  return NWS_OK;
}

int audio_half(const NwsWeights* w, const NwsForwardAux* aux, const float* f0, int B, int T, float sample_rate,
               const float* phase_u, const float* rand_phase, const float* noise, float* out, const Arena& a, void* stream,
               void* wait_before_exciter = nullptr, void* record_after_exciter = nullptr, bool with_reverb = true) {
  hipStream_t st = (hipStream_t)stream;
  int rc = NWS_OK;
  const size_t N = (size_t)T * NWS_HOP;
  NWS_STAGE(2, nws_frame_mlps(w, a.gru_out, aux->fir_design, B, T, nullptr, a.film, nullptr, a.fir, stream));
  NWS_STAGE(4, nws_fir_noise(a.fir, noise, nullptr, B, T, a.noise_out, stream));
  if (wait_before_exciter != nullptr) {
    const hipError_t e = hipStreamWaitEvent(st, (hipEvent_t)wait_before_exciter, 0);
    if (e != hipSuccess) return (int)e;
  }
  NWS_STAGE(3, nws_exciter_newt_add(w, f0, nullptr, a.carry, phase_u, rand_phase, a.film, a.noise_out, B, T, sample_rate, nullptr, a.pre, stream));
  if (record_after_exciter != nullptr) {
    const hipError_t e = hipEventRecord((hipEvent_t)record_after_exciter, st);
    if (e != hipSuccess) return (int)e;
  }
  if (with_reverb)
    NWS_STAGE(5, nws_reverb(aux->plan, aux->reverb_tables, aux->reverb_spectrum, a.pre, B, (int)N, out, a.rv_ws, a.rv_bytes, stream));
  if (g_prof.ev != nullptr && g_prof.used < g_prof.slots) ++g_prof.used;
  return NWS_OK;
}
#undef NWS_STAGE

bool aux_ok(const NwsForwardAux* aux) {
  return aux && aux->plan && aux->fir_design && aux->reverb_tables && aux->reverb_spectrum;
}

}

extern "C" {

size_t nws_sizeof(int which) {
  switch (which) {
    case 0: return sizeof(NwsWeights);
    case 1: return sizeof(NwsReverbPlan);
    case 2: return sizeof(NwsForwardAux);
    case 3: return sizeof(NwsShaperDesc);
    case 4: return sizeof(NwsGenericModel);
    default: return 0;
  }
}

size_t nws_forward_control_bytes(int B, int T) {
  if (B <= 0 || T <= 0) return 0;
  const size_t N = (size_t)T * NWS_HOP;
  return aligned((size_t)B * (N / 32) * sizeof(double)) + aligned((size_t)B * T * NWS_HIDDEN * sizeof(float));
}

int nws_forward(const NwsWeights* w, const NwsForwardAux* aux, const float* f0, const float* control, int B, int C,
                int T, float sample_rate, const float* phase_u, const float* rand_phase, const float* noise, float* out,
                void* workspace, size_t workspace_bytes, void* stream) {
  if (!w || !aux_ok(aux)) return NWS_ERR_BAD_ARG;
  if (!f0 || !control || !phase_u || !rand_phase || !noise || !out || !workspace) return NWS_ERR_BAD_ARG;
  if (B <= 0 || T < 2 || C < 2) return NWS_ERR_BAD_ARG;
  if (T > (1 << 23) || !nws_reverb_plan_serves(aux->plan, T * NWS_HOP, 0)) return NWS_ERR_BAD_ARG;
  const Arena a = carve_arena(aux->plan, workspace, workspace_bytes, B, T, false);
  if (!a.ok) return NWS_ERR_WORKSPACE;
  const int rc = control_half(w, f0, control, B, C, T, 0, a, stream);
  if (rc != NWS_OK) return rc;
  return audio_half(w, aux, f0, B, T, sample_rate, phase_u, rand_phase, noise, out, a, stream);
}

int nws_forward_control(const NwsWeights* w, const float* f0, const float* control, int B, int C, int T, int batched_gru,
                        void* workspace, size_t workspace_bytes, void* stream) {
  if (!w || !f0 || !control || !workspace) return NWS_ERR_BAD_ARG;
  if (B <= 0 || T < 2 || C < 2) return NWS_ERR_BAD_ARG;
  const Arena a = carve_arena(nullptr, workspace, workspace_bytes, B, T, true);
  if (!a.ok) return NWS_ERR_WORKSPACE;
  return control_half(w, f0, control, B, C, T, batched_gru, a, stream);
}

int nws_forward_audio(const NwsWeights* w, const NwsForwardAux* aux, const float* f0, int B, int T, float sample_rate,
                      const float* phase_u, const float* rand_phase, const float* noise, float* out, void* workspace,
                      size_t workspace_bytes, void* stream) {
  if (!w || !aux_ok(aux)) return NWS_ERR_BAD_ARG;
  if (!f0 || !phase_u || !rand_phase || !noise || !out || !workspace) return NWS_ERR_BAD_ARG;
  if (B <= 0 || T < 2) return NWS_ERR_BAD_ARG;
  if (T > (1 << 23) || !nws_reverb_plan_serves(aux->plan, T * NWS_HOP, 0)) return NWS_ERR_BAD_ARG;
  const Arena a = carve_arena(aux->plan, workspace, workspace_bytes, B, T, false);
  if (!a.ok) return NWS_ERR_WORKSPACE;
  return audio_half(w, aux, f0, B, T, sample_rate, phase_u, rand_phase, noise, out, a, stream);
}

int nws_forward_audio_ev(const NwsWeights* w, const NwsForwardAux* aux, const float* f0, int B, int T, float sample_rate,
                         const float* phase_u, const float* rand_phase, const float* noise, float* out, void* workspace,
                         size_t workspace_bytes, void* stream, void* wait_before_exciter, void* record_after_exciter) {
  if (!w || !aux_ok(aux)) return NWS_ERR_BAD_ARG;
  if (!f0 || !phase_u || !rand_phase || !noise || !out || !workspace) return NWS_ERR_BAD_ARG;
  if (B <= 0 || T < 2) return NWS_ERR_BAD_ARG;
  if (T > (1 << 23) || !nws_reverb_plan_serves(aux->plan, T * NWS_HOP, 0)) return NWS_ERR_BAD_ARG;
  const Arena a = carve_arena(aux->plan, workspace, workspace_bytes, B, T, false);
  if (!a.ok) return NWS_ERR_WORKSPACE;
  return audio_half(w, aux, f0, B, T, sample_rate, phase_u, rand_phase, noise, out, a, stream, wait_before_exciter,
                    record_after_exciter);
}

int nws_forward_audio_pre(const NwsWeights* w, const NwsForwardAux* aux, const float* f0, int B, int T, float sample_rate,
                          const float* phase_u, const float* rand_phase, const float* noise, void* workspace,
                          size_t workspace_bytes, void* stream) {
  if (!w || !aux_ok(aux)) return NWS_ERR_BAD_ARG;
  if (!f0 || !phase_u || !rand_phase || !noise || !workspace) return NWS_ERR_BAD_ARG;
  if (B <= 0 || T < 2) return NWS_ERR_BAD_ARG;
  if (T > (1 << 23) || !nws_reverb_plan_serves(aux->plan, T * NWS_HOP, 0)) return NWS_ERR_BAD_ARG;
  const Arena a = carve_arena(aux->plan, workspace, workspace_bytes, B, T, false);
  if (!a.ok) return NWS_ERR_WORKSPACE;
  return audio_half(w, aux, f0, B, T, sample_rate, phase_u, rand_phase, noise, nullptr, a, stream, nullptr, nullptr, false);
}

int nws_forward_reverb_rows(const NwsForwardAux* aux, int B, int T, int row0, int nrows, float* out ,
                            void* workspace, size_t workspace_bytes, void* stream) {
  if (!aux_ok(aux) || !out || !workspace || B <= 0 || T < 2 || row0 < 0 || nrows <= 0 || row0 + nrows > B) return NWS_ERR_BAD_ARG;
  const Arena a = carve_arena(aux->plan, workspace, workspace_bytes, B, T, false);
  if (!a.ok) return NWS_ERR_WORKSPACE;
  const size_t N = (size_t)T * NWS_HOP;
  if (row0 & 1) return NWS_ERR_BAD_ARG;
  const size_t per_pair = 2 * (size_t)aux->plan->nblk * (size_t)aux->plan->L * sizeof(float);
  char* rv = static_cast<char*>(a.rv_ws) + (size_t)(row0 / 2) * per_pair;
  const size_t left = a.rv_bytes - (size_t)(row0 / 2) * per_pair;
  return nws_reverb(aux->plan, aux->reverb_tables, aux->reverb_spectrum, a.pre + (size_t)row0 * N, nrows, (int)N, out + (size_t)row0 * N, rv,
                    left, stream);
}

int nws_forward_audio_blocks(const NwsWeights* w, const NwsForwardAux* aux, const float* f0, int B, int T, float sample_rate,
                             const float* phase_u, const float* rand_phase, const float* noise, float* out, void* workspace,
                             size_t workspace_bytes, void* stream, const int32_t* row0, const int32_t* nrows, void* const* events,
                             int nblocks) {
  if (!row0 || !nrows || nblocks <= 0 || !out) return NWS_ERR_BAD_ARG;
  int next = 0;
  for (int q = 0; q < nblocks; ++q) {
    if (row0[q] != next || nrows[q] <= 0 || ((nrows[q] & 1) && q != nblocks - 1)) return NWS_ERR_BAD_ARG;
    next += nrows[q];
  }
  if (next != B) return NWS_ERR_BAD_ARG;
  int rc = nws_forward_audio_pre(w, aux, f0, B, T, sample_rate, phase_u, rand_phase, noise, workspace, workspace_bytes, stream);
  if (rc != NWS_OK) return rc;
  for (int q = 0; q < nblocks; ++q) {
    rc = nws_forward_reverb_rows(aux, B, T, row0[q], nrows[q], out, workspace, workspace_bytes, stream);
    if (rc != NWS_OK) return rc;
    if (events != nullptr && events[q] != nullptr) {
      const hipError_t e = hipEventRecord((hipEvent_t)events[q], (hipStream_t)stream);
      if (e != hipSuccess) return (int)e;
    }
  }
  return NWS_OK;
}

int nws_profile_begin(int slots, unsigned stage_mask) {
  nws_profile_end();
  if (slots <= 0) return NWS_ERR_BAD_ARG;
  g_prof.ev = new hipEvent_t[(size_t)slots * kStages * 2];
  for (size_t i = 0; i < (size_t)slots * kStages * 2; ++i) {
    hipError_t e = hipEventCreateWithFlags(&g_prof.ev[i], hipEventDisableSystemFence);
    if (e != hipSuccess) return (int)e;
  }
  g_prof.slots = slots;
  g_prof.used = 0;
  g_prof.mask = stage_mask;
  return NWS_OK;
}

int nws_profile_collect(float* ms_out, int* n_out) {
  if (!ms_out || !n_out) return NWS_ERR_BAD_ARG;
  const int n = g_prof.used;
  for (int i = 0; i < n; ++i)
    for (int s = 0; s < kStages; ++s) {
      float ms = -1.0f;
      if (g_prof.mask & (1u << s)) {
        hipEvent_t* e = g_prof.ev + ((size_t)i * kStages + s) * 2;
        hipError_t err = hipEventSynchronize(e[1]);
        if (err != hipSuccess) return (int)err;
        err = hipEventElapsedTime(&ms, e[0], e[1]);
        if (err != hipSuccess) return (int)err;
      }
      ms_out[(size_t)i * kStages + s] = ms;
    }
  *n_out = n;
  g_prof.used = g_prof.slots;
  return NWS_OK;
}

int nws_profile_end(void) {
  if (g_prof.ev != nullptr) {
    for (size_t i = 0; i < (size_t)g_prof.slots * kStages * 2; ++i) (void)hipEventDestroy(g_prof.ev[i]);
    delete[] g_prof.ev;
  }
  g_prof = Profile();
  return NWS_OK;
}

}
```

### neural-waveshaping-synthesis_amd/csrc/torch_ops.cpp

```cpp
#include <ATen/ATen.h>
#include <ATen/hip/impl/HIPGuardImplMasqueradingAsCUDA.h>
#include <ATen/hip/impl/HIPStreamMasqueradingAsCUDA.h>
#include <torch/library.h>

#include <algorithm>
#include <cstdlib>
#include <tuple>
#include <vector>

#include "../../include/nws_hip.h"
#include "../../include/nws_hip_debug.h"

namespace {

using at::Tensor;
using OptTensor = c10::optional<at::Tensor>;

const NwsWeights* weights_of(const Tensor& wdesc) {
  TORCH_CHECK(wdesc.device().is_cpu() && wdesc.scalar_type() == at::kByte && wdesc.is_contiguous() &&
                  (size_t)wdesc.numel() == sizeof(NwsWeights),
              "wdesc: expected a contiguous CPU uint8 tensor of ", sizeof(NwsWeights), " bytes (one NwsWeights struct), got ",
              wdesc.sizes(), " ", wdesc.scalar_type(), " on ", wdesc.device());
  return reinterpret_cast<const NwsWeights*>(wdesc.data_ptr());
}

void check_dev(const Tensor& t, const char* name, at::ScalarType st = at::kFloat) {
  TORCH_CHECK(t.is_cuda(), name, " lives on ", t.device(),
              ": the NEWT forward path only runs as HIP kernels on an AMD GPU (there is no CPU fallback)");
  TORCH_CHECK(t.scalar_type() == st, name, ": expected ", st, ", got ", t.scalar_type());
  TORCH_CHECK(t.is_contiguous(), name, ": expected a contiguous tensor");
}

void check_same_device(const Tensor& a, const char* an, const Tensor& b, const char* bn) {
  TORCH_CHECK(a.device() == b.device(), an, " is on ", a.device(), " but ", bn, " is on ", b.device(),
              ": all tensors of one call must live on the same GPU");
}

void nws_check(int rc, const char* what) {
  TORCH_CHECK(rc == NWS_OK, what, " failed (", rc, "): ", nws_error_string(rc));
}

const float* fptr(const OptTensor& t) { return t.has_value() ? t->data_ptr<float>() : nullptr; }

struct Launch {
  c10::hip::HIPGuardMasqueradingAsCUDA guard;
  void* stream;
  explicit Launch(const Tensor& t)
      : guard(t.device()), stream(c10::hip::getCurrentHIPStreamMasqueradingAsCUDA(t.device().index()).stream()) {}
};

NwsReverbPlan plan_of(const Tensor& plan) {
  TORCH_CHECK(plan.device().is_cpu() && plan.scalar_type() == at::kInt && plan.is_contiguous() && plan.numel() == 8,
              "plan: expected a CPU int32 tensor [L, N1, N2, Lc, hist, nblk, 0, 0] (the NwsReverbPlan of nws_reverb_plan)");
  const int32_t* p = plan.data_ptr<int32_t>();
  return NwsReverbPlan{p[0], p[1], p[2], p[3], p[4], p[5], {p[6], p[7]}};
}

void check_reverb_buffers(const NwsReverbPlan& plan, const Tensor& tables, const Tensor& spectrum) {
  TORCH_CHECK(plan.L > 0 && plan.N1 > 0 && plan.N2 > 0 && (int64_t)plan.N1 * plan.N2 == plan.L, "plan: inconsistent [L, N1, N2] = [",
              plan.L, ", ", plan.N1, ", ", plan.N2, "]");
  TORCH_CHECK((size_t)tables.numel() * tables.element_size() == nws_reverb_table_bytes(&plan), "reverb_tables: ",
              (size_t)tables.numel() * tables.element_size(), " bytes, the plan (L = ", plan.L, ") needs ", nws_reverb_table_bytes(&plan));
  TORCH_CHECK((size_t)spectrum.numel() * spectrum.element_size() == nws_reverb_spectrum_bytes(&plan), "reverb_spectrum: ",
              (size_t)spectrum.numel() * spectrum.element_size(), " bytes, the plan (L = ", plan.L, ") needs ",
              nws_reverb_spectrum_bytes(&plan), " (Sre | Sim | ir_)");
}

struct Aux {
  NwsReverbPlan plan;
  NwsForwardAux aux;
  Aux(const Tensor& fir_design, const Tensor& plan_t, const Tensor& tables, const Tensor& spectrum) : plan(plan_of(plan_t)) {
    check_dev(fir_design, "fir_design");
    check_dev(tables, "reverb_tables");
    check_dev(spectrum, "reverb_spectrum");
    TORCH_CHECK(fir_design.numel() == NWS_FIR_LEN * 132, "fir_design: expected (256, 132)");
    check_reverb_buffers(plan, tables, spectrum);
    aux.fir_design = fir_design.data_ptr<float>();
    aux.plan = &plan;
    aux.reverb_tables = tables.data_ptr();
    aux.reverb_spectrum = spectrum.data_ptr();
  }
};

void check_inputs(const Tensor& f0, const Tensor& control, int64_t& B, int64_t& C, int64_t& T) {
  check_dev(f0, "f0");
  check_dev(control, "control");
  check_same_device(f0, "f0", control, "control");
  TORCH_CHECK(f0.dim() == 3 && f0.size(1) == 1, "f0: expected (B, 1, T), got ", f0.sizes());
  TORCH_CHECK(control.dim() == 3 && control.size(1) >= 2, "control: expected (B, C>=2, T), got ", control.sizes());
  B = f0.size(0);
  T = f0.size(2);
  C = control.size(1);
  TORCH_CHECK(control.size(0) == B && control.size(2) == T, "f0 ", f0.sizes(), " and control ", control.sizes(),
              " disagree on batch / frames");
  TORCH_CHECK(T >= 2, "need at least 2 control frames (reflect padding of the noise STFT, generators.py:31)");
}

void check_draws(const Tensor& phase_u, const Tensor& rand_phase, const Tensor& noise, int64_t T, const Tensor& like) {
  check_dev(phase_u, "phase_u");
  check_dev(rand_phase, "rand_phase");
  check_dev(noise, "noise");
  check_same_device(like, "f0", phase_u, "phase_u");
  check_same_device(like, "f0", noise, "noise");
  check_same_device(like, "f0", rand_phase, "osc.rand_phase");
  TORCH_CHECK(phase_u.numel() == NWS_N_HARMONICS, "phase_u: expected 101 elements, got ", phase_u.sizes());
  TORCH_CHECK(rand_phase.numel() == NWS_N_HARMONICS, "rand_phase: expected 101 elements, got ", rand_phase.sizes());
  TORCH_CHECK(noise.numel() == NWS_HOP * T - 1, "noise: expected ", NWS_HOP * T - 1, " elements, got ", noise.sizes());
}

struct AudioShape {
  int64_t B, T;
  AudioShape(const Tensor& f0, const Tensor& phase_u, const Tensor& rand_phase, const Tensor& noise, const Tensor& workspace) {
    check_dev(f0, "f0");
    TORCH_CHECK(f0.dim() == 3 && f0.size(1) == 1 && f0.size(2) >= 2, "f0: expected (B, 1, T>=2), got ", f0.sizes());
    B = f0.size(0);
    T = f0.size(2);
    check_draws(phase_u, rand_phase, noise, T, f0);
    check_dev(workspace, "workspace", at::kByte);
    check_same_device(f0, "f0", workspace, "workspace");
  }
};

struct AudioArgs : AudioShape, Aux {
  AudioArgs(const Tensor& f0, const Tensor& phase_u, const Tensor& rand_phase, const Tensor& noise, const Tensor& fir_design,
            const Tensor& plan_t, const Tensor& tables, const Tensor& spectrum, const Tensor& workspace)
      : AudioShape(f0, phase_u, rand_phase, noise, workspace), Aux(fir_design, plan_t, tables, spectrum) {}
};

Tensor forward(const Tensor& wdesc, const Tensor& f0, const Tensor& control, const Tensor& phase_u, const Tensor& rand_phase,
               const Tensor& noise, const Tensor& fir_design, const Tensor& plan, const Tensor& reverb_tables,
               const Tensor& reverb_spectrum, Tensor& workspace, double sample_rate) {
  const NwsWeights* w = weights_of(wdesc);
  int64_t B, C, T;
  check_inputs(f0, control, B, C, T);
  check_draws(phase_u, rand_phase, noise, T, f0);
  check_dev(workspace, "workspace", at::kByte);
  check_same_device(f0, "f0", workspace, "workspace");
  Aux a(fir_design, plan, reverb_tables, reverb_spectrum);
  check_same_device(f0, "f0", fir_design, "the model's tables");
  Launch L(f0);
  Tensor out = at::empty({B, T * NWS_HOP}, f0.options());
  nws_check(nws_forward(w, &a.aux, f0.data_ptr<float>(), control.data_ptr<float>(), (int)B, (int)C, (int)T, (float)sample_rate,
                        phase_u.data_ptr<float>(), rand_phase.data_ptr<float>(), noise.data_ptr<float>(), out.data_ptr<float>(),
                        workspace.data_ptr(), (size_t)workspace.numel(), L.stream),
            "nws_forward");
  return out;
}

void forward_control(const Tensor& wdesc, const Tensor& f0, const Tensor& control, Tensor& workspace, bool batched_gru) {
  const NwsWeights* w = weights_of(wdesc);
  int64_t B, C, T;
  check_inputs(f0, control, B, C, T);
  check_dev(workspace, "workspace", at::kByte);
  check_same_device(f0, "f0", workspace, "workspace");
  Launch L(f0);
  nws_check(nws_forward_control(w, f0.data_ptr<float>(), control.data_ptr<float>(), (int)B, (int)C, (int)T, batched_gru ? 1 : 0,
                                workspace.data_ptr(), (size_t)workspace.numel(), L.stream),
            "nws_forward_control");
}

Tensor forward_audio(const Tensor& wdesc, const Tensor& f0, const Tensor& phase_u, const Tensor& rand_phase, const Tensor& noise,
                     const Tensor& fir_design, const Tensor& plan, const Tensor& reverb_tables, const Tensor& reverb_spectrum,
                     Tensor& workspace, double sample_rate, const OptTensor& out_opt, int64_t wait_event, int64_t record_event) {
  const NwsWeights* w = weights_of(wdesc);
  AudioArgs a(f0, phase_u, rand_phase, noise, fir_design, plan, reverb_tables, reverb_spectrum, workspace);
  const int64_t B = a.B, T = a.T;
  Launch L(f0);
  Tensor out;
  if (out_opt.has_value()) {
    out = *out_opt;
    check_dev(out, "out");
    check_same_device(f0, "f0", out, "out");
    TORCH_CHECK(out.dim() == 2 && out.size(0) == B && out.size(1) == T * NWS_HOP, "out: expected (", B, ", ", T * NWS_HOP, ")");
  } else {
    out = at::empty({B, T * NWS_HOP}, f0.options());
  }
  nws_check(nws_forward_audio_ev(w, &a.aux, f0.data_ptr<float>(), (int)B, (int)T, (float)sample_rate, phase_u.data_ptr<float>(),
                                 rand_phase.data_ptr<float>(), noise.data_ptr<float>(), out.data_ptr<float>(), workspace.data_ptr(),
                                 (size_t)workspace.numel(), L.stream, reinterpret_cast<void*>(wait_event),
                                 reinterpret_cast<void*>(record_event)),
            "nws_forward_audio");
  return out;
}

void forward_audio_pre(const Tensor& wdesc, const Tensor& f0, const Tensor& phase_u, const Tensor& rand_phase, const Tensor& noise,
                       const Tensor& fir_design, const Tensor& plan, const Tensor& reverb_tables, const Tensor& reverb_spectrum,
                       Tensor& workspace, double sample_rate) {
  const NwsWeights* w = weights_of(wdesc);
  AudioArgs a(f0, phase_u, rand_phase, noise, fir_design, plan, reverb_tables, reverb_spectrum, workspace);
  const int64_t B = a.B, T = a.T;
  Launch L(f0);
  nws_check(nws_forward_audio_pre(w, &a.aux, f0.data_ptr<float>(), (int)B, (int)T, (float)sample_rate, phase_u.data_ptr<float>(),
                                  rand_phase.data_ptr<float>(), noise.data_ptr<float>(), workspace.data_ptr(),
                                  (size_t)workspace.numel(), L.stream), "nws_forward_audio_pre");
}

void forward_reverb_rows(const Tensor& fir_design, const Tensor& plan, const Tensor& reverb_tables, const Tensor& reverb_spectrum,
                         Tensor& workspace, int64_t T, int64_t row0, int64_t nrows, Tensor& out) {
  check_dev(workspace, "workspace", at::kByte);
  check_dev(out, "out");
  check_same_device(out, "out", workspace, "workspace");
  TORCH_CHECK(out.dim() == 2 && out.size(1) == T * NWS_HOP, "out: expected (B, ", T * NWS_HOP, "), got ", out.sizes());
  TORCH_CHECK(row0 >= 0 && nrows > 0 && row0 + nrows <= out.size(0) && (row0 & 1) == 0, "forward_reverb_rows: bad row block");
  Aux a(fir_design, plan, reverb_tables, reverb_spectrum);
  Launch L(out);
  nws_check(nws_forward_reverb_rows(&a.aux, (int)out.size(0), (int)T, (int)row0, (int)nrows, out.data_ptr<float>(), workspace.data_ptr(),
                                    (size_t)workspace.numel(), L.stream), "nws_forward_reverb_rows");
}

void forward_audio_blocks(const Tensor& wdesc, const Tensor& f0, const Tensor& phase_u, const Tensor& rand_phase, const Tensor& noise,
                          const Tensor& fir_design, const Tensor& plan, const Tensor& reverb_tables, const Tensor& reverb_spectrum,
                          Tensor& workspace, double sample_rate, Tensor& out, at::IntArrayRef row0, at::IntArrayRef nrows,
                          at::IntArrayRef events) {
  const NwsWeights* w = weights_of(wdesc);
  AudioArgs a(f0, phase_u, rand_phase, noise, fir_design, plan, reverb_tables, reverb_spectrum, workspace);
  const int64_t B = a.B, T = a.T;
  check_dev(out, "out");
  check_same_device(f0, "f0", out, "out");
  TORCH_CHECK(out.dim() == 2 && out.size(0) == B && out.size(1) == T * NWS_HOP && out.is_contiguous(), "out: expected a contiguous (", B, ", ",
              T * NWS_HOP, "), got ", out.sizes());
  TORCH_CHECK(!row0.empty() && row0.size() == nrows.size() && (events.empty() || events.size() == row0.size()),
              "forward_audio_blocks: row0 / nrows / events must have one entry per block");
  std::vector<int32_t> r0(row0.begin(), row0.end()), nr(nrows.begin(), nrows.end());
  std::vector<void*> ev(events.size());
  for (size_t q = 0; q < events.size(); ++q) ev[q] = reinterpret_cast<void*>(static_cast<uintptr_t>(events[q]));
  Launch L(f0);
  nws_check(nws_forward_audio_blocks(w, &a.aux, f0.data_ptr<float>(), (int)B, (int)T, (float)sample_rate, phase_u.data_ptr<float>(),
                                     rand_phase.data_ptr<float>(), noise.data_ptr<float>(), out.data_ptr<float>(), workspace.data_ptr(),
                                     (size_t)workspace.numel(), L.stream, r0.data(), nr.data(), ev.empty() ? nullptr : ev.data(), (int)r0.size()),
            "nws_forward_audio_blocks");
}

Tensor phase_carry(const OptTensor& f0, const OptTensor& f0_up) {
  TORCH_CHECK(f0.has_value() != f0_up.has_value(), "phase_carry: give exactly one of f0 (B, T) and f0_up (B, 128 T)");
  const Tensor& src = f0.has_value() ? *f0 : *f0_up;
  check_dev(src, f0.has_value() ? "f0" : "f0_up");
  TORCH_CHECK(src.dim() == 2, "phase_carry: expected a 2-D tensor, got ", src.sizes());
  const int64_t B = src.size(0);
  TORCH_CHECK(f0.has_value() || src.size(1) % NWS_HOP == 0, "f0_up: the sample count must be a multiple of ", NWS_HOP);
  const int64_t T = f0.has_value() ? src.size(1) : src.size(1) / NWS_HOP;
  Launch L(src);
  Tensor carry = at::empty({B, T * NWS_HOP / 32}, src.options().dtype(at::kDouble));
  nws_check(nws_phase_carry(fptr(f0), fptr(f0_up), (int)B, (int)T, carry.data_ptr<double>(), L.stream), "nws_phase_carry");
  return carry;
}

std::tuple<Tensor, Tensor> exciter_newt(const Tensor& wdesc, const OptTensor& f0, const OptTensor& f0_up, const Tensor& carry,
                                        const Tensor& phase_u, const Tensor& rand_phase, const OptTensor& film,
                                        double sample_rate, bool want_exciter, bool want_newt) {
  const NwsWeights* w = weights_of(wdesc);
  TORCH_CHECK(f0.has_value() != f0_up.has_value(), "exciter_newt: give exactly one of f0 (B, T) and f0_up (B, 128 T)");
  TORCH_CHECK(want_exciter || want_newt, "exciter_newt: nothing to compute");
  const Tensor& src = f0.has_value() ? *f0 : *f0_up;
  check_dev(src, "f0");
  check_dev(carry, "carry", at::kDouble);
  check_dev(phase_u, "phase_u");
  check_dev(rand_phase, "rand_phase");
  check_same_device(src, "f0", carry, "carry");
  check_same_device(src, "f0", phase_u, "phase_u");
  TORCH_CHECK(src.dim() == 2, "exciter_newt: f0 / f0_up must be 2-D, got ", src.sizes());
  const int64_t B = src.size(0);
  const int64_t T = f0.has_value() ? src.size(1) : src.size(1) / NWS_HOP;
  const int64_t N = T * NWS_HOP;
  TORCH_CHECK(f0.has_value() || src.size(1) == N, "f0_up: the sample count must be a multiple of ", NWS_HOP);
  TORCH_CHECK(carry.numel() == B * (N / 32), "carry: expected (", B, ", ", N / 32, "), got ", carry.sizes());
  TORCH_CHECK(phase_u.numel() == NWS_N_HARMONICS && rand_phase.numel() == NWS_N_HARMONICS, "phase_u / rand_phase: 101 elements each");
  if (want_newt) {
    TORCH_CHECK(film.has_value(), "exciter_newt: the waveshaper bank needs the FiLM parameters (film)");
    check_dev(*film, "film");
    check_same_device(src, "f0", *film, "film");
    TORCH_CHECK(film->numel() == B * T * NWS_FILM_CH, "film: expected (", B, ", ", T, ", 256), got ", film->sizes());
  }
  Launch L(src);
  Tensor exc = want_exciter ? at::empty({B, NWS_N_SHAPERS, N}, src.options()) : at::empty({0}, src.options());
  Tensor out = want_newt ? at::empty({B, N}, src.options()) : at::empty({0}, src.options());
  nws_check(nws_exciter_newt(w, fptr(f0), fptr(f0_up), carry.data_ptr<double>(), phase_u.data_ptr<float>(),
                             rand_phase.data_ptr<float>(), fptr(film), (int)B, (int)T, (float)sample_rate,
                             want_exciter ? exc.data_ptr<float>() : nullptr, want_newt ? out.data_ptr<float>() : nullptr, L.stream),
            "nws_exciter_newt");
  return {exc, out};
}

Tensor oscillator(const Tensor& f0_up, const Tensor& phase_u, const Tensor& rand_phase, double sample_rate) {
  check_dev(f0_up, "f0");
  check_dev(phase_u, "phase_u");
  check_dev(rand_phase, "rand_phase");
  check_same_device(f0_up, "f0", phase_u, "phase_u");
  check_same_device(f0_up, "f0", rand_phase, "rand_phase");
  TORCH_CHECK(f0_up.dim() == 2, "HarmonicOscillator: expected f0 of shape (B, N), got ", f0_up.sizes());
  TORCH_CHECK(f0_up.size(1) % NWS_HOP == 0 && f0_up.size(1) > 0,
              "HarmonicOscillator on the HIP path: the sample count must be a multiple of ", NWS_HOP, ", got ", f0_up.size(1));
  TORCH_CHECK(phase_u.numel() == NWS_N_HARMONICS && rand_phase.numel() == NWS_N_HARMONICS,
              "kernels are specialised for 101 harmonics (gin/models/newt.gin)");
  const int64_t B = f0_up.size(0), N = f0_up.size(1);
  Launch L(f0_up);
  Tensor carry = at::empty({B, N / 32}, f0_up.options().dtype(at::kDouble));
  nws_check(nws_phase_carry(nullptr, f0_up.data_ptr<float>(), (int)B, (int)(N / NWS_HOP), carry.data_ptr<double>(), L.stream),
            "nws_phase_carry");
  Tensor out = at::empty({B, NWS_N_HARMONICS, N}, f0_up.options());
  nws_check(nws_oscillator(f0_up.data_ptr<float>(), carry.data_ptr<double>(), phase_u.data_ptr<float>(),
                           rand_phase.data_ptr<float>(), (int)B, (int)N, (float)sample_rate, out.data_ptr<float>(), L.stream),
            "nws_oscillator");
  return out;
}

std::tuple<Tensor, Tensor> control_gru(const Tensor& wdesc, const Tensor& control, const OptTensor& h0, bool batched) {
  const NwsWeights* w = weights_of(wdesc);
  check_dev(control, "control");
  TORCH_CHECK(control.dim() == 3 && control.size(1) >= 2, "control: expected (B, C>=2, T), got ", control.sizes());
  const int64_t B = control.size(0), C = control.size(1), T = control.size(2);
  TORCH_CHECK(T >= 1, "control: need at least one frame");
  if (h0.has_value()) {
    check_dev(*h0, "h0");
    check_same_device(control, "control", *h0, "h0");
    TORCH_CHECK(h0->numel() == B * NWS_HIDDEN, "h0: expected (", B, ", 128), got ", h0->sizes());
  }
  Launch L(control);
  Tensor out = at::empty({B, T, NWS_HIDDEN}, control.options());
  Tensor hT = at::empty({B, NWS_HIDDEN}, control.options());
  if (batched)
    nws_check(nws_control_gru_batched(w, control.data_ptr<float>(), (int)B, (int)C, (int)T, fptr(h0), out.data_ptr<float>(),
                                      hT.data_ptr<float>(), L.stream), "nws_control_gru_batched");
  else
    nws_check(nws_control_gru_state(w, control.data_ptr<float>(), (int)B, (int)C, (int)T, fptr(h0), out.data_ptr<float>(),
                                    hT.data_ptr<float>(), L.stream), "nws_control_gru_state");
  return {out, hT};
}

std::tuple<Tensor, Tensor, Tensor, Tensor> frame_mlps(const Tensor& wdesc, const Tensor& gru_out, const Tensor& fir_design,
                                                       bool want_emb, bool want_H) {
  const NwsWeights* w = weights_of(wdesc);
  check_dev(gru_out, "gru_out");
  check_dev(fir_design, "fir_design");
  check_same_device(gru_out, "gru_out", fir_design, "fir_design");
  TORCH_CHECK(gru_out.dim() == 3 && gru_out.size(2) == NWS_HIDDEN, "gru_out: expected (B, T, 128), got ", gru_out.sizes());
  TORCH_CHECK(fir_design.numel() == NWS_FIR_LEN * 132, "fir_design: expected (256, 132)");
  const int64_t B = gru_out.size(0), T = gru_out.size(1);
  Launch L(gru_out);
  const auto o = gru_out.options();
  Tensor emb = want_emb ? at::empty({B, NWS_HIDDEN, T}, o) : at::empty({0}, o);
  Tensor film = at::empty({B, T, NWS_FILM_CH}, o);
  Tensor H = want_H ? at::empty({B, T, NWS_N_BANDS}, o) : at::empty({0}, o);
  Tensor fir = at::empty({B, T, NWS_FIR_HALF}, o);
  nws_check(nws_frame_mlps(w, gru_out.data_ptr<float>(), fir_design.data_ptr<float>(), (int)B, (int)T,
                           want_emb ? emb.data_ptr<float>() : nullptr, film.data_ptr<float>(),
                           want_H ? H.data_ptr<float>() : nullptr, fir.data_ptr<float>(), L.stream), "nws_frame_mlps");
  return {emb, film, H, fir};
}

Tensor fir_noise(const Tensor& fir, const Tensor& noise, const OptTensor& add_in, int64_t origin) {
  check_dev(fir, "fir");
  check_dev(noise, "noise");
  check_same_device(fir, "fir", noise, "noise");
  TORCH_CHECK(fir.dim() == 3 && fir.size(2) == NWS_FIR_HALF, "fir: expected (B, T, 128) upper half-taps (nws_frame_mlps), got ", fir.sizes());
  const int64_t B = fir.size(0), T = fir.size(1);
  if (add_in.has_value()) {
    check_dev(*add_in, "add_in");
    check_same_device(fir, "fir", *add_in, "add_in");
    TORCH_CHECK(add_in->numel() == B * T * NWS_HOP, "add_in: expected (", B, ", ", T * NWS_HOP, "), got ", add_in->sizes());
  }
  Launch L(fir);
  Tensor out = at::empty({B, T * NWS_HOP}, fir.options());
  if (origin < 0) {
    TORCH_CHECK(noise.numel() == T * NWS_HOP - 1, "noise: expected ", T * NWS_HOP - 1, " samples, got ", noise.sizes());
    nws_check(nws_fir_noise(fir.data_ptr<float>(), noise.data_ptr<float>(), fptr(add_in), (int)B, (int)T, out.data_ptr<float>(),
                            L.stream), "nws_fir_noise");
  } else {
    nws_check(nws_fir_noise_window(fir.data_ptr<float>(), noise.data_ptr<float>(), (int)noise.numel(), (int)origin, fptr(add_in),
                                   (int)B, (int)T, out.data_ptr<float>(), L.stream), "nws_fir_noise_window");
  }
  return out;
}

Tensor fir_from_h(const Tensor& H, const Tensor& fir_design) {
  check_dev(H, "H");
  check_dev(fir_design, "fir_design");
  check_same_device(H, "H", fir_design, "fir_design");
  TORCH_CHECK(H.dim() == 3 && H.size(1) == NWS_N_BANDS, "FIRNoiseSynth: expected H of shape (B, 129, T), got ", H.sizes());
  TORCH_CHECK(fir_design.numel() == NWS_FIR_LEN * 132, "fir_design: expected (256, 132)");
  Launch L(H);
  Tensor fir = at::empty({H.size(0), H.size(2), NWS_FIR_HALF}, H.options());
  nws_check(nws_fir_from_h(H.data_ptr<float>(), fir_design.data_ptr<float>(), (int)H.size(0), (int)H.size(2), fir.data_ptr<float>(),
                           L.stream), "nws_fir_from_h");
  return fir;
}

Tensor fir_noise_grad(const Tensor& noise, const Tensor& grad_out) {
  check_dev(noise, "noise");
  check_dev(grad_out, "grad_out");
  check_same_device(grad_out, "grad_out", noise, "noise");
  TORCH_CHECK(grad_out.dim() == 2 && grad_out.size(1) % NWS_HOP == 0 && grad_out.size(1) >= 2 * NWS_HOP,
              "fir_noise_grad: expected grad_out (B, 128 T) with T >= 2, got ", grad_out.sizes());
  const int64_t B = grad_out.size(0), T = grad_out.size(1) / NWS_HOP;
  TORCH_CHECK(noise.numel() == T * NWS_HOP - 1, "noise: expected ", T * NWS_HOP - 1, " samples, got ", noise.sizes());
  Launch L(grad_out);
  Tensor grad_fir = at::empty({B, T, NWS_FIR_HALF}, grad_out.options());
  nws_check(nws_fir_noise_grad(noise.data_ptr<float>(), grad_out.data_ptr<float>(), (int)B, (int)T, grad_fir.data_ptr<float>(),
                               L.stream), "nws_fir_noise_grad");
  return grad_fir;
}

Tensor fir_from_h_grad(const Tensor& grad_fir, const Tensor& fir_design) {
  check_dev(grad_fir, "grad_fir");
  check_dev(fir_design, "fir_design");
  check_same_device(grad_fir, "grad_fir", fir_design, "fir_design");
  TORCH_CHECK(grad_fir.dim() == 3 && grad_fir.size(2) == NWS_FIR_HALF, "fir_from_h_grad: expected grad_fir (B, T, 128), got ", grad_fir.sizes());
  TORCH_CHECK(fir_design.numel() == NWS_FIR_LEN * 132, "fir_design: expected (256, 132)");
  Launch L(grad_fir);
  Tensor grad_H = at::empty({grad_fir.size(0), NWS_N_BANDS, grad_fir.size(1)}, grad_fir.options());
  nws_check(nws_fir_from_h_grad(grad_fir.data_ptr<float>(), fir_design.data_ptr<float>(), (int)grad_fir.size(0), (int)grad_fir.size(1),
                                grad_H.data_ptr<float>(), L.stream), "nws_fir_from_h_grad");
  return grad_H;
}

Tensor sum_batch_time(const Tensor& x) {
  check_dev(x, "x");
  TORCH_CHECK(x.dim() == 3, "sum_batch_time: expected (B, C, T), got ", x.sizes());
  Launch L(x);
  Tensor out = at::empty({x.size(1)}, x.options());
  nws_check(nws_sum_batch_time(x.data_ptr<float>(), (int)x.size(0), (int)x.size(1), (int)x.size(2), out.data_ptr<float>(), L.stream),
            "nws_sum_batch_time");
  return out;
}

Tensor reverb(const Tensor& plan_t, const Tensor& tables, const Tensor& spectrum, const Tensor& x) {
  NwsReverbPlan plan = plan_of(plan_t);
  check_dev(x, "x");
  check_dev(tables, "reverb_tables");
  check_dev(spectrum, "reverb_spectrum");
  check_same_device(x, "x", tables, "reverb tables");
  check_same_device(x, "x", spectrum, "reverb.ir spectrum");
  TORCH_CHECK(x.dim() == 2, "Reverb: expected (B, N), got ", x.sizes());
  check_reverb_buffers(plan, tables, spectrum);
  const int64_t B = x.size(0), N = x.size(1);
  TORCH_CHECK(nws_reverb_plan_serves(&plan, (int)N, 0), "Reverb: the plan [L ", plan.L, ", Lc ", plan.Lc, ", hist ", plan.hist, ", nblk ", plan.nblk,
              "] was not made for ", N, " samples");
  Launch L(x);
  const size_t nbytes = nws_reverb_workspace_bytes(&plan, (int)B);
  Tensor ws = at::empty({(int64_t)nbytes}, x.options().dtype(at::kByte));
  Tensor y = at::empty_like(x);
  nws_check(nws_reverb(&plan, tables.data_ptr(), spectrum.data_ptr(), x.data_ptr<float>(), (int)B, (int)N, y.data_ptr<float>(),
                       ws.data_ptr(), nbytes, L.stream), "nws_reverb");
  return y;
}

Tensor reverb_grad_x(const Tensor& plan_t, const Tensor& tables, const Tensor& spectrum, const Tensor& grad_out) {
  NwsReverbPlan plan = plan_of(plan_t);
  check_dev(grad_out, "grad_out");
  check_dev(tables, "reverb_tables");
  check_dev(spectrum, "reverb_spectrum");
  check_same_device(grad_out, "grad_out", tables, "reverb tables");
  check_same_device(grad_out, "grad_out", spectrum, "reverb.ir spectrum");
  TORCH_CHECK(grad_out.dim() == 2, "reverb_grad_x: expected (B, N), got ", grad_out.sizes());
  check_reverb_buffers(plan, tables, spectrum);
  const int64_t B = grad_out.size(0), N = grad_out.size(1);
  TORCH_CHECK(nws_reverb_plan_serves(&plan, (int)N, 0), "reverb_grad_x: the plan [L ", plan.L, ", Lc ", plan.Lc, ", hist ", plan.hist,
              ", nblk ", plan.nblk, "] was not made for ", N, " samples");
  Launch L(grad_out);
  const size_t nbytes = nws_reverb_grad_workspace_bytes(&plan, (int)B, 0);
  Tensor ws = at::empty({(int64_t)nbytes}, grad_out.options().dtype(at::kByte));
  Tensor dx = at::empty_like(grad_out);
  nws_check(nws_reverb_grad_x(&plan, tables.data_ptr(), spectrum.data_ptr(), grad_out.data_ptr<float>(), (int)B, (int)N,
                              dx.data_ptr<float>(), ws.data_ptr(), nbytes, L.stream), "nws_reverb_grad_x");
  return dx;
}

Tensor reverb_grad_ir(const Tensor& plan_t, const Tensor& tables, const Tensor& x, const Tensor& grad_out, int64_t ir_len) {
  NwsReverbPlan plan = plan_of(plan_t);
  check_dev(x, "x");
  check_dev(grad_out, "grad_out");
  check_dev(tables, "reverb_tables");
  check_same_device(x, "x", tables, "reverb tables");
  check_same_device(x, "x", grad_out, "grad_out");
  TORCH_CHECK(x.dim() == 2 && grad_out.sizes() == x.sizes(), "reverb_grad_ir: x ", x.sizes(), " and grad_out ", grad_out.sizes(),
              " differ in shape");
  TORCH_CHECK((size_t)tables.numel() * tables.element_size() == nws_reverb_table_bytes(&plan), "reverb_tables: ",
              (size_t)tables.numel() * tables.element_size(), " bytes, the plan (L = ", plan.L, ") needs ", nws_reverb_table_bytes(&plan));
  const int64_t B = x.size(0), N = x.size(1);
  TORCH_CHECK(ir_len > 0 && ir_len < (1 << 30) && nws_reverb_plan_serves(&plan, (int)N, (int)ir_len + 1), "reverb_grad_ir: the plan [L ",
              plan.L, ", Lc ", plan.Lc, ", hist ", plan.hist, ", nblk ", plan.nblk, "] was not made for ", N, " samples and an impulse response of ",
              ir_len);
  Launch L(x);
  const size_t nbytes = nws_reverb_grad_workspace_bytes(&plan, (int)B, 1);
  Tensor ws = at::empty({(int64_t)nbytes}, x.options().dtype(at::kByte));
  Tensor dir = at::empty({ir_len}, x.options());
  nws_check(nws_reverb_grad_ir(&plan, tables.data_ptr(), x.data_ptr<float>(), grad_out.data_ptr<float>(), (int)B, (int)N, (int)ir_len,
                               dir.data_ptr<float>(), ws.data_ptr(), nbytes, L.stream), "nws_reverb_grad_ir");
  return dir;
}

std::tuple<Tensor, Tensor> reverb_linear_chunk(const Tensor& plan_t, const Tensor& tables, const Tensor& spectrum, const Tensor& x,
                                               const Tensor& tail_in) {
  NwsReverbPlan plan = plan_of(plan_t);
  check_dev(x, "x");
  check_dev(tail_in, "tail_in");
  check_dev(tables, "reverb_tables");
  check_dev(spectrum, "reverb_spectrum");
  check_same_device(x, "x", tail_in, "tail_in");
  check_same_device(x, "x", tables, "reverb tables");
  TORCH_CHECK(x.dim() == 2 && tail_in.dim() == 2 && tail_in.size(0) == x.size(0), "reverb_linear_chunk: x (B, M), tail_in (B, tail)");
  const int64_t B = x.size(0), M = x.size(1), tail_len = tail_in.size(1);
  check_reverb_buffers(plan, tables, spectrum);
  check_same_device(x, "x", spectrum, "reverb.ir spectrum");
  TORCH_CHECK(plan.Lc == 0, "reverb_linear_chunk: needs a direct plan (one transform of M + tail_len samples)");
  TORCH_CHECK(M + tail_len <= plan.L, "reverb_linear_chunk: chunk of ", M, " + tail of ", tail_len, " samples wraps around L = ", plan.L);
  Launch L(x);
  const size_t nbytes = (size_t)(2 * ((B + 1) / 2) * plan.L + B * plan.L) * sizeof(float);
  Tensor ws = at::empty({(int64_t)nbytes}, x.options().dtype(at::kByte));
  Tensor y = at::empty_like(x);
  Tensor tail_out = at::empty_like(tail_in);
  nws_check(nws_reverb_linear_chunk(&plan, tables.data_ptr(), spectrum.data_ptr(), x.data_ptr<float>(), (int)B, (int)M,
                                    tail_in.data_ptr<float>(), tail_out.data_ptr<float>(), (int)tail_len, y.data_ptr<float>(),
                                    ws.data_ptr(), nbytes, L.stream), "nws_reverb_linear_chunk");
  return {y, tail_out};
}

Tensor shaper_apply(const Tensor& wdesc, const Tensor& x) {
  const NwsWeights* w = weights_of(wdesc);
  check_dev(x, "x");
  TORCH_CHECK(x.dim() == 3 && x.size(1) == NWS_N_SHAPERS, "expected (B, 64, N), got ", x.sizes());
  Launch L(x);
  Tensor y = at::empty_like(x);
  nws_check(nws_shaper_apply(w, x.data_ptr<float>(), x.size(0), x.size(2), y.data_ptr<float>(), L.stream), "nws_shaper_apply");
// ... 553 lines not shown
  TORCH_CHECK(T > 0 && N % T == 0, "NEWT: ", N, " samples are not a whole multiple of ", T, " control frames");
  TORCH_CHECK(mix_w.numel() % S == 0 && mix_b.numel() == mix_w.numel() / S, "NEWT: mixer weight ", mix_w.sizes(), " / bias ", mix_b.sizes());
  const int64_t O = mix_w.numel() / S;
  Launch L(exciter);
  Tensor shaped = at::empty_like(exciter);
  nws_check(nws_g_film_shaper(d, exciter.data_ptr<float>(), film.data_ptr<float>(), (int)B, (int)T, (int)(N / T),
                              shaped.data_ptr<float>(), L.stream), "nws_g_film_shaper");
  Tensor out = at::empty({B, O, N}, exciter.options());
  nws_check(nws_g_conv1x1(shaped.data_ptr<float>(), mix_w.data_ptr<float>(), mix_b.data_ptr<float>(), (int)B, (int)S, (int)O, (int)N,
                          out.data_ptr<float>(), L.stream), "nws_g_conv1x1");
  return out;
}

Tensor g_fir_noise(const Tensor& H, const Tensor& window, const Tensor& noise, int64_t hop) {
  check_dev(H, "H");
  check_dev(window, "window");
  check_dev(noise, "noise");
  check_same_device(H, "H", window, "noise_synth.window");
  check_same_device(H, "H", noise, "noise");
  const int64_t Lf = window.numel();
  TORCH_CHECK(H.dim() == 3 && H.size(1) == Lf / 2 + 1, "FIRNoiseSynth: expected H of shape (B, ", Lf / 2 + 1, ", T), got ", H.sizes());
  const int64_t B = H.size(0), T = H.size(2);
  TORCH_CHECK(noise.numel() == hop * T - 1, "noise: expected ", hop * T - 1, " samples, got ", noise.sizes());
  Launch L(H);
  Tensor fir = at::empty({B, T, Lf}, H.options());
  nws_check(nws_g_fir_design(H.data_ptr<float>(), window.data_ptr<float>(), (int)Lf, (int)B, (int)T, fir.data_ptr<float>(), L.stream),
            "nws_g_fir_design");
  Tensor out = at::empty({B, hop * T}, H.options());
  nws_check(nws_g_fir_noise(fir.data_ptr<float>(), noise.data_ptr<float>(), (int)Lf, (int)hop, (int)B, (int)T, nullptr, 0,
                            out.data_ptr<float>(), L.stream), "nws_g_fir_noise");
  return out;
}

Tensor g_reverb_direct(const Tensor& x, const Tensor& ir) {
  check_dev(x, "x");
  check_dev(ir, "reverb.ir");
  check_same_device(x, "x", ir, "reverb.ir");
  TORCH_CHECK(x.dim() == 2, "Reverb: expected (B, N), got ", x.sizes());
  Launch L(x);
  Tensor y = at::empty_like(x);
  nws_check(nws_g_reverb_direct(x.data_ptr<float>(), ir.data_ptr<float>(), (int)ir.numel(), (int)x.size(0), (int)x.size(1),
                                y.data_ptr<float>(), L.stream), "nws_g_reverb_direct");
  return y;
}

struct StepDims {
  int64_t B, K, C;
};

StepDims check_step_tensors(const char* op, const Tensor& f0, const Tensor& control, const Tensor& fir_design, const Tensor& state,
                            const Tensor& phase_u, const Tensor& rand_phase, const Tensor& ir, const Tensor& out) {
  check_dev(f0, "f0");
  check_dev(control, "control");
  check_dev(fir_design, "fir_design");
  check_dev(state, "state", at::kByte);
  check_dev(phase_u, "phase_u");
  check_dev(rand_phase, "rand_phase");
  check_dev(ir, "reverb.ir");
  check_dev(out, "out");
  check_same_device(f0, "f0", control, "control");
  check_same_device(f0, "f0", state, "state");
  check_same_device(f0, "f0", out, "out");
  check_same_device(f0, "f0", ir, "reverb.ir");
  TORCH_CHECK(f0.dim() == 2 && control.dim() == 3 && control.size(0) == f0.size(0) && control.size(2) == f0.size(1) && control.size(1) >= 2,
              op, ": f0 (B, K), control (B, C>=2, K); got ", f0.sizes(), " / ", control.sizes());
  return {f0.size(0), f0.size(1), control.size(1)};
}

void check_step_io(const char* op, const StepDims& d, bool first, bool final, int64_t frames_seen, const Tensor& phase_u,
                   const Tensor& rand_phase, const OptTensor& noise_new, const OptTensor& noise_all, const Tensor& out,
                   const OptTensor& pre_out) {
  TORCH_CHECK(phase_u.numel() == NWS_N_HARMONICS && rand_phase.numel() == NWS_N_HARMONICS, "phase_u / rand_phase: 101 elements each");
  TORCH_CHECK(noise_new.has_value() != noise_all.has_value(), op, ": give exactly one of noise_new and noise_all");
  const int M = nws_stream_out_samples((int)d.K, first, final);
  TORCH_CHECK(out.numel() == d.B * M, "out: expected (", d.B, ", ", M, "), got ", out.sizes());
  if (pre_out.has_value()) {
    check_dev(*pre_out, "pre_out");
    TORCH_CHECK(pre_out->numel() == d.B * M, "pre_out: expected (", d.B, ", ", M, ")");
  }
  if (noise_new.has_value()) {
    check_dev(*noise_new, "noise_new");
    TORCH_CHECK(noise_new->numel() >= nws_stream_noise_draws((int)d.K, first, frames_seen), "noise_new: expected ",
                nws_stream_noise_draws((int)d.K, first, frames_seen), " fresh samples");
  } else {
    check_dev(*noise_all, "noise_all");
  }
}

void stream_step(const Tensor& wdesc, const Tensor& fir_design, const OptTensor& plan_t, const OptTensor& tables,
                 const OptTensor& spectrum, Tensor& state, int64_t max_frames, const Tensor& f0, const Tensor& control, bool first,
                 bool final, int64_t frames_seen, int64_t nz_prev_start, double sample_rate, const Tensor& phase_u,
                 const Tensor& rand_phase, const OptTensor& noise_new, const OptTensor& noise_all, const Tensor& ir, Tensor& out,
                 const OptTensor& pre_out) {
  const NwsWeights* w = weights_of(wdesc);
  const StepDims d = check_step_tensors("stream_step", f0, control, fir_design, state, phase_u, rand_phase, ir, out);
  const int64_t B = d.B, K = d.K, C = d.C;
  TORCH_CHECK(K >= 1 && K <= max_frames, "stream_step: chunk of ", K, " frames, the stream was sized for ", max_frames);
  check_step_io("stream_step", d, first, final, frames_seen, phase_u, rand_phase, noise_new, noise_all, out, pre_out);
  NwsReverbPlan plan{};
  const bool fft = plan_t.has_value();
  if (fft) {
    TORCH_CHECK(tables.has_value() && spectrum.has_value(), "stream_step: plan without tables / spectrum");
    plan = plan_of(*plan_t);
    check_dev(*tables, "reverb_tables");
    check_dev(*spectrum, "reverb_spectrum");
    check_reverb_buffers(plan, *tables, *spectrum);
  }
  TORCH_CHECK((size_t)state.numel() >= nws_stream_state_bytes((int)B, (int)max_frames, (int)ir.numel(), fft ? &plan : nullptr),
              "stream_step: state blob too small");
  Launch L(f0);
  nws_check(nws_stream_step(w, fir_design.data_ptr<float>(), fft ? &plan : nullptr, fft ? tables->data_ptr() : nullptr,
                            fft ? spectrum->data_ptr() : nullptr, state.data_ptr(), (size_t)state.numel(), (int)B, (int)max_frames,
                            f0.data_ptr<float>(), control.data_ptr<float>(), (int)C, (int)K, first ? 1 : 0, final ? 1 : 0,
                            (long long)frames_seen, (long long)nz_prev_start, (float)sample_rate, phase_u.data_ptr<float>(),
                            rand_phase.data_ptr<float>(), fptr(noise_new), fptr(noise_all),
                            noise_all.has_value() ? (int)noise_all->numel() : 0, ir.data_ptr<float>(), (int)ir.numel(),
                            out.data_ptr<float>(), pre_out.has_value() ? pre_out->data_ptr<float>() : nullptr, L.stream),
            "nws_stream_step");
}

void stream_step_slots(const Tensor& wdesc, const Tensor& fir_design, Tensor& state, int64_t max_frames, const Tensor& f0,
                       const Tensor& control, int64_t frames_seen, int64_t nz_prev_start, double sample_rate, const Tensor& phase_u,
                       const Tensor& rand_phase, const OptTensor& noise_new, const OptTensor& noise_all, const Tensor& ir,
                       const Tensor& events, Tensor& out, const OptTensor& pre_out) {
  const NwsWeights* w = weights_of(wdesc);
  const StepDims d = check_step_tensors("stream_step_slots", f0, control, fir_design, state, phase_u, rand_phase, ir, out);
  const int64_t B = d.B, K = d.K, C = d.C;
  check_dev(events, "events", at::kInt);
  check_same_device(f0, "f0", events, "events");
  TORCH_CHECK(K >= 1 && K <= 16 && K <= max_frames, "stream_step_slots: hops of 1 .. 16 frames (sized for ", max_frames, "), got ", K);
  TORCH_CHECK(events.numel() == B, "stream_step_slots: events: one int32 word per slot, expected ", B, ", got ", events.numel());
  check_step_io("stream_step_slots", d, frames_seen == 0, false, frames_seen, phase_u, rand_phase, noise_new, noise_all, out, pre_out);
  TORCH_CHECK((size_t)state.numel() >= nws_stream_slot_state_bytes((int)B, (int)max_frames, (int)ir.numel()),
              "stream_step_slots: state blob too small");
  Launch L(f0);
  nws_check(nws_stream_step_slots(w, fir_design.data_ptr<float>(), state.data_ptr(), (size_t)state.numel(), (int)B, (int)max_frames,
                                  f0.data_ptr<float>(), control.data_ptr<float>(), (int)C, (int)K, (long long)frames_seen,
                                  (long long)nz_prev_start, (float)sample_rate, phase_u.data_ptr<float>(), rand_phase.data_ptr<float>(),
                                  fptr(noise_new), fptr(noise_all), noise_all.has_value() ? (int)noise_all->numel() : 0,
                                  ir.data_ptr<float>(), (int)ir.numel(), events.data_ptr<int>(), out.data_ptr<float>(),
                                  pre_out.has_value() ? pre_out->data_ptr<float>() : nullptr, L.stream),
            "nws_stream_step_slots");
}

int64_t abi_version() { return nws_abi_version(); }

}

TORCH_LIBRARY(newt_hip, m) {
  m.def("abi_version() -> int", &abi_version);
  m.def("forward(Tensor wdesc, Tensor f0, Tensor control, Tensor phase_u, Tensor rand_phase, Tensor noise, Tensor fir_design, "
        "Tensor plan, Tensor reverb_tables, Tensor reverb_spectrum, Tensor(a!) workspace, float sample_rate) -> Tensor", &forward);
  m.def("forward_control(Tensor wdesc, Tensor f0, Tensor control, Tensor(a!) workspace, bool batched_gru) -> ()", &forward_control);
  m.def("forward_audio(Tensor wdesc, Tensor f0, Tensor phase_u, Tensor rand_phase, Tensor noise, Tensor fir_design, Tensor plan, "
        "Tensor reverb_tables, Tensor reverb_spectrum, Tensor(a!) workspace, float sample_rate, Tensor? out, int wait_event, "
        "int record_event) -> Tensor", &forward_audio);
  m.def("forward_audio_pre(Tensor wdesc, Tensor f0, Tensor phase_u, Tensor rand_phase, Tensor noise, Tensor fir_design, Tensor plan, "
        "Tensor reverb_tables, Tensor reverb_spectrum, Tensor(a!) workspace, float sample_rate) -> ()", &forward_audio_pre);
  m.def("forward_audio_blocks(Tensor wdesc, Tensor f0, Tensor phase_u, Tensor rand_phase, Tensor noise, Tensor fir_design, Tensor plan, "
        "Tensor reverb_tables, Tensor reverb_spectrum, Tensor(a!) workspace, float sample_rate, Tensor(b!) out, int[] row0, int[] nrows, "
        "int[] events) -> ()", &forward_audio_blocks);
  m.def("forward_reverb_rows(Tensor fir_design, Tensor plan, Tensor reverb_tables, Tensor reverb_spectrum, Tensor(a!) workspace, int T, "
        "int row0, int nrows, Tensor(b!) out) -> ()", &forward_reverb_rows);
  m.def("phase_carry(Tensor? f0, Tensor? f0_up) -> Tensor", &phase_carry);
  m.def("exciter_newt(Tensor wdesc, Tensor? f0, Tensor? f0_up, Tensor carry, Tensor phase_u, Tensor rand_phase, Tensor? film, "
        "float sample_rate, bool want_exciter, bool want_newt) -> (Tensor, Tensor)", &exciter_newt);
  m.def("oscillator(Tensor f0_up, Tensor phase_u, Tensor rand_phase, float sample_rate) -> Tensor", &oscillator);
  m.def("control_gru(Tensor wdesc, Tensor control, Tensor? h0, bool batched) -> (Tensor, Tensor)", &control_gru);
  m.def("frame_mlps(Tensor wdesc, Tensor gru_out, Tensor fir_design, bool want_emb, bool want_H) -> (Tensor, Tensor, Tensor, Tensor)",
        &frame_mlps);
  m.def("fir_noise(Tensor fir, Tensor noise, Tensor? add_in, int origin) -> Tensor", &fir_noise);
  m.def("fir_from_h(Tensor H, Tensor fir_design) -> Tensor", &fir_from_h);
  m.def("fir_noise_grad(Tensor noise, Tensor grad_out) -> Tensor", &fir_noise_grad);
  m.def("fir_from_h_grad(Tensor grad_fir, Tensor fir_design) -> Tensor", &fir_from_h_grad);
  m.def("sum_batch_time(Tensor x) -> Tensor", &sum_batch_time);
  m.def("reverb(Tensor plan, Tensor tables, Tensor spectrum, Tensor x) -> Tensor", &reverb);
  m.def("reverb_grad_x(Tensor plan, Tensor tables, Tensor spectrum, Tensor grad_out) -> Tensor", &reverb_grad_x);
  m.def("reverb_grad_ir(Tensor plan, Tensor tables, Tensor x, Tensor grad_out, int ir_len) -> Tensor", &reverb_grad_ir);
  m.def("reverb_linear_chunk(Tensor plan, Tensor tables, Tensor spectrum, Tensor x, Tensor tail_in) -> (Tensor, Tensor)",
        &reverb_linear_chunk);
  m.def("shaper_apply(Tensor wdesc, Tensor x) -> Tensor", &shaper_apply);
  m.def("shaper_table(Tensor wdesc, Tensor like, int size, float tmin, float tmax) -> Tensor", &shaper_table);
  m.def("newt_apply(Tensor wdesc, Tensor exciter, Tensor film) -> Tensor", &newt_apply);
  m.def("td_mlp(Tensor x, Tensor[] weights, Tensor[] biases, Tensor[] ln_w, Tensor[] ln_b, float eps, float slope) -> Tensor", &td_mlp);
  m.def("td_layer_norm(Tensor x, Tensor weight, Tensor bias, float eps) -> Tensor", &td_layer_norm);
  m.def("film(Tensor x, Tensor gamma, Tensor beta) -> Tensor", &film);
  m.def("sine(Tensor x) -> Tensor", &sine);
  m.def("forward_generic(Tensor gdesc, Tensor f0, Tensor control, Tensor phase_u, Tensor rand_phase, Tensor noise, Tensor? plan, "
        "Tensor? reverb_tables, Tensor? reverb_spectrum, Tensor(a!) reverb_workspace, Tensor(b!) workspace, float sample_rate) -> Tensor",
        &forward_generic);
  m.def("g_gru(Tensor w_ih, Tensor w_hh, Tensor b_ih, Tensor b_hh, Tensor control, Tensor? h0) -> (Tensor, Tensor)", &g_gru);
  m.def("g_oscillator(Tensor f0_up, Tensor phase_u, Tensor rand_phase, float sample_rate) -> Tensor", &g_oscillator);
  m.def("g_conv1x1(Tensor x, Tensor weight, Tensor? bias) -> Tensor", &g_conv1x1);
  m.def("g_upsample(Tensor x, int hop) -> Tensor", &g_upsample);
  m.def("g_shaper_apply(Tensor sdesc, Tensor x) -> Tensor", &g_shaper_apply);
  m.def("g_shaper_table(Tensor sdesc, Tensor like, int size, float tmin, float tmax) -> Tensor", &g_shaper_table);
  m.def("g_newt_apply(Tensor sdesc, Tensor exciter, Tensor film, Tensor mix_w, Tensor mix_b) -> Tensor", &g_newt_apply);
  m.def("g_fir_noise(Tensor H, Tensor window, Tensor noise, int hop) -> Tensor", &g_fir_noise);
  m.def("g_reverb_direct(Tensor x, Tensor ir) -> Tensor", &g_reverb_direct);
  m.def("stream_step(Tensor wdesc, Tensor fir_design, Tensor? plan, Tensor? reverb_tables, Tensor? reverb_spectrum, Tensor(a!) state, "
        "int max_frames, Tensor f0, Tensor control, bool first, bool final, int frames_seen, int nz_prev_start, float sample_rate, "
        "Tensor phase_u, Tensor rand_phase, Tensor? noise_new, Tensor? noise_all, Tensor ir, Tensor(b!) out, Tensor(c!)? pre_out) -> ()",
        &stream_step);
  m.def("stream_step_slots(Tensor wdesc, Tensor fir_design, Tensor(a!) state, int max_frames, Tensor f0, Tensor control, int frames_seen, "
        "int nz_prev_start, float sample_rate, Tensor phase_u, Tensor rand_phase, Tensor? noise_new, Tensor? noise_all, Tensor ir, "
        "Tensor events, Tensor(b!) out, Tensor(c!)? pre_out) -> ()",
        &stream_step_slots);
  m.def("loudness(Tensor audio, Tensor dft, int n_fft, int hop, float amin, float top_db, bool normalise) -> Tensor", &loudness);
  m.def("pyin_table(float sample_rate, float fmin, float fmax, int frame_length, int hop) -> Tensor", &pyin_table);
  m.def("pyin_cmnd(Tensor audio, float sample_rate, float fmin, float fmax, int frame_length, int hop) -> Tensor", &pyin_cmnd);
  m.def("pyin_observe(Tensor yin, Tensor table, float sample_rate, float fmin, float fmax, int frame_length, int hop) -> "
        "(Tensor, Tensor, Tensor, Tensor)", &pyin_observe);
  m.def("pyin_viterbi(Tensor cand_bin, Tensor cand_prob, Tensor count, Tensor voiced_prob, Tensor table, float sample_rate, "
        "float fmin, float fmax, int frame_length, int hop, bool fill_unvoiced, float fill_value) -> (Tensor, Tensor)", &pyin_viterbi);
  m.def("pyin(Tensor audio, Tensor table, float sample_rate, float fmin, float fmax, int frame_length, int hop, bool fill_unvoiced, "
        "float fill_value) -> (Tensor, Tensor, Tensor)", &pyin);
  m.def("resample_bank(int sr_in, int sr_out) -> Tensor", &resample_bank);
  m.def("resample(Tensor audio, Tensor bank, int sr_in, int sr_out) -> Tensor", &resample);
  m.def("mfcc_table(float sample_rate, int n_fft, int n_mfcc, int n_mels) -> Tensor", &mfcc_table);
  m.def("stft_loss_dft(int n_fft, int win_length) -> Tensor", &stft_loss_dft);
  m.def("stft_loss(Tensor x, Tensor y, Tensor[] dfts, int[] n_ffts, int[] hops, int[] win_lengths, float w_sc, float w_log_mag, "
        "float w_lin_mag, float eps) -> Tensor[]", &stft_loss);
  m.def("stft_loss_grad(Tensor x, Tensor y, Tensor[] dfts, int[] n_ffts, int[] hops, int[] win_lengths, float w_sc, float w_log_mag, "
        "float w_lin_mag, float eps) -> Tensor", &stft_loss_grad);
  m.def("mfcc(Tensor audio, Tensor dft, Tensor table, float sample_rate, int n_fft, int hop, int n_mfcc, int n_mels) -> Tensor", &mfcc);
}
```

### neural-waveshaping-synthesis_amd/engine.py

```python
from __future__ import annotations

import ctypes as C
import itertools
import math
import os
from typing import NamedTuple

import torch

from . import _lib
from ._lib import NwsReverbPlan, NwsWeights, check, ptr


def _req(t: torch.Tensor, name: str, numel: int | None = None) -> torch.Tensor:
    if not isinstance(t, torch.Tensor):
        raise TypeError(f"{name}: expected a tensor")
    if t.device.type != "cuda":
        raise _lib.NwsError(
            f"{name} lives on {t.device}: the NEWT forward path only runs as HIP kernels on an AMD GPU "
            "(move the model and inputs with .to('cuda')); there is no CPU fallback.")
    if t.dtype != torch.float32:
        raise TypeError(f"{name}: expected float32, got {t.dtype}")
    if not t.is_contiguous():
        raise ValueError(f"{name}: expected a contiguous tensor")
# ... 267 lines not shown
            if table is not None:
                size = int(m.newt.table_size)
                w.lut = P(table, "newt.lookup_table", 64 * size)
                pairs = torch.empty((64, size, 2), dtype=torch.float32, device=table.device)
                check(L.nws_lut_pairs(w.lut, size, ptr(pairs), st), "nws_lut_pairs")
                keep.append(pairs)
                w.lut_pairs = pairs.data_ptr()
                w.lut_size = size
                w.lut_min = float(m.newt.table_min)
                w.lut_max = float(m.newt.table_max)
            else:
                w.lut = None
                w.lut_pairs = None
                w.lut_size, w.lut_min, w.lut_max = 0, 0.0, 0.0
            w.exciter_opts = self.exciter_opts()
            if getattr(m.newt, "lookup_table", None) is None and self.bank_nofract_safe():
                w.exciter_opts |= _lib.EXCITER_BANK_NOFRACT
            w.newt_out_w = P(m.newt.mixer[0].weight, "newt.mixer.0.weight", 64)
            w.newt_out_b = P(m.newt.mixer[0].bias, "newt.mixer.0.bias", 1)
            w.noise_window = P(m.noise_synth.window, "noise_synth.window", 256)
            fd = torch.empty(_lib.FIR_LEN * _lib.FIR_DESIGN_COLS, dtype=torch.float32, device=dev)
            check(L.nws_fir_design_matrix(w.noise_window, ptr(fd), st), "nws_fir_design_matrix")
            keep.append(fd)
            w.mlp_frags = None
            if self.fp16_mlp_safe():
                frags = torch.empty(_lib.MLP_FRAGS_BYTES, dtype=torch.uint8, device=dev)
                check(L.nws_mlp_frags(C.byref(w), ptr(fd), ptr(frags), st), "nws_mlp_frags")
                keep.append(frags)
                w.mlp_frags = frags.data_ptr()
            rand_phase = _req(m.osc.rand_phase.detach(), "osc.rand_phase", 101)
            ir = _req(m.reverb.ir.detach(), "reverb.ir")
            keep += [rand_phase, ir]
            devs = {t.device for t in keep}
            if len(devs) != 1:
                raise RuntimeError(f"model parameters are spread over several devices: {devs}")
            torch.cuda.current_stream(dev).synchronize()
        wdesc = torch.frombuffer(bytearray(bytes(w)), dtype=torch.uint8)
        self._w = Weights(w, wdesc, dev, rand_phase, ir, fd, keep)
        self._fp = fp
        return self._w

    HYBRID_W_BOUND = 1e-5

    def exciter_opts(self) -> int:
        v = getattr(self._model_ref, "exciter_opts", None)
        if v is None:
            v = os.environ.get("NWS_EXCITER_OPTS")
        if v is not None and str(v) != "auto":
            return int(v)
        b = self.hybrid_w_bound()
        return _lib.EXCITER_HYBRID_W if (b is not None and b["bound"] <= self.HYBRID_W_BOUND) else 0

    def bank_nofract_safe(self, limit_turns: float = 128.0) -> bool:
        sh = self._model_ref.newt._modules.get("shaping_fn")
        if sh is None or getattr(sh, "depth", 0) != 4:
            return False
        with torch.no_grad():
            worst = 0.0
            for i in (2, 4, 6):
                wt, b = sh.net[i].weight.detach(), sh.net[i].bias.detach()
                worst = max(worst, float((wt.abs().flatten(1).sum(1) + b.abs()).max()) / (2.0 * math.pi))
        return math.isfinite(worst) and worst < limit_turns

    def hybrid_w_bound(self):
        from . import precision

        m = self._model_ref
        table = getattr(m.newt, "lookup_table", None)
        if table is None:
            return None
        return precision.hybrid_w_error_bound(m, table, float(m.newt.table_min), float(m.newt.table_max))

    def fp16_mlp_safe(self, limit: float = 3.0e4) -> bool:
        m = self._model_ref
        with torch.no_grad():
            def l1(wt, b, scale):
                return float((wt.detach().abs().flatten(1).sum(1) * scale + b.detach().abs()).max())

            def ln(mod):
                return float(math.sqrt(_lib.HIDDEN - 1) * mod.layer_norm.weight.detach().abs().max()
                             + mod.layer_norm.bias.detach().abs().max())

            bounds = [l1(m.embedding.proj.weight, m.embedding.proj.bias, 1.0)]
            for mlp in (m.newt.mlp, m.h_generator):
                bounds += [ln(mlp.net[1]), ln(mlp.net[4]), ln(mlp.net[7])]
            bounds.append(l1(m.h_generator.net[9].weight, m.h_generator.net[9].bias, ln(m.h_generator.net[7])))
            wmax = max(float(p.detach().abs().max()) for mlp in (m.newt.mlp, m.h_generator) for p in mlp.parameters())
        return max(bounds + [wmax]) < limit and all(b == b for b in bounds)

    @property
    def device(self):
        return self._wd().device

    def rand_phase(self):
        return self._wd().rand_phase

    def ir(self):
        return self._wd().ir

    def fir_design(self):
        return self._wd().fir_design

    def osc_sample_rate(self) -> float:
        m = self._model_ref
        return float(getattr(getattr(m, "osc", None), "sample_rate", m.sample_rate))

    def reverb_aux(self, n_samples: int):
        self._wd()
        return self._reverb_aux(n_samples)

    def _reverb_aux(self, n_samples: int):
        ir, dev = self._w.ir, self._w.device
        plan, tables, plan_t = reverb_plan_and_tables(dev, n_samples, ir.numel() + 1)
        skey = (plan.L, plan.N1, plan.N2)
        spec = self._spectra.get(skey)
        if spec is None:
            with torch.cuda.device(dev):
                spec = torch.empty(_lib.lib().nws_reverb_spectrum_bytes(C.byref(plan)) // 4, dtype=torch.float32, device=dev)
                nbytes = _lib.lib().nws_reverb_workspace_bytes(C.byref(plan), 1)
                ws = torch.empty(nbytes, dtype=torch.uint8, device=dev)
                check(_lib.lib().nws_reverb_ir_spectrum(C.byref(plan), ptr(tables), ptr(ir), ir.numel(), ptr(spec), ptr(ws),
                                                        nbytes, stream_ptr(dev)), "nws_reverb_ir_spectrum")
                torch.cuda.current_stream(dev).synchronize()
            self._spectra[skey] = spec
        return plan, tables, spec, plan_t

    def phase_carry(self, f0=None, f0_up=None):
        return binding().phase_carry(f0, f0_up)

    def exciter_newt(self, f0, f0_up, carry, phase_u, film, want_exciter=False, want_newt=True):
        r = self._wd()
        same_device(r.device, f0=f0 if f0 is not None else f0_up, carry=carry, phase_u=phase_u, film=film)
        exc, out = binding().exciter_newt(r.wdesc, f0, f0_up, carry, phase_u, r.rand_phase, film, self.osc_sample_rate(),
                                          want_exciter, want_newt)
        return (exc if want_exciter else None), (out if want_newt else None)

    def control_gru(self, control, batched=False, h0=None, return_state=False):
        r = self._wd()
        same_device(r.device, control=control, h0=h0)
        out, hT = binding().control_gru(r.wdesc, control, h0, bool(batched))
        return (out, hT) if return_state else out

    def frame_mlps(self, gru_out, want_emb=False, want_H=False):
        r = self._wd()
        same_device(r.device, gru_out=gru_out)
        emb, film, H, fir = binding().frame_mlps(r.wdesc, gru_out, r.fir_design, want_emb, want_H)
        return (emb if want_emb else None), film, (H if want_H else None), fir

    def fir_noise(self, fir, noise, add_in=None, origin=None, noise_len=None):
        same_device(fir.device, noise=noise, add_in=add_in)
        nz = noise if noise_len is None or noise_len == noise.numel() else noise[:noise_len]
        return binding().fir_noise(fir, nz, add_in, -1 if origin is None else int(origin))

    def reverb(self, x):
        same_device(self._wd().device, x=x)
        _, tables, spec, plan_t = self._reverb_aux(x.shape[1])
        return binding().reverb(plan_t, tables, spec, x)

    def reverb_linear_chunk(self, plan_aux, x, tail_in):
        _, tables, spec, plan_t = plan_aux
        same_device(tables.device, x=x, tail_in=tail_in)
        return binding().reverb_linear_chunk(plan_t, tables, spec, x, tail_in)

    def shaper_table(self, size, tmin, tmax):
        r = self._wd()
        return binding().shaper_table(r.wdesc, r.rand_phase, int(size), float(tmin), float(tmax))

    def shaper_apply(self, x):
        r = self._wd()
        same_device(r.device, x=x)
        return binding().shaper_apply(r.wdesc, x)

    def newt_apply(self, exciter, film):
        r = self._wd()
        same_device(r.device, exciter=exciter, film=film)
        return binding().newt_apply(r.wdesc, exciter, film)

    def new_workspace(self, B, T):
        dev = self._wd().device
        plan, _, _, _ = self._reverb_aux(T * _lib.HOP)
        return torch.empty(_lib.lib().nws_forward_workspace_bytes(C.byref(plan), B, T), dtype=torch.uint8, device=dev)

    def forward_control(self, f0, control, ws, batched_gru=True):
        r = self._wd()
        same_device(r.device, f0=f0, control=control, workspace=ws)
        binding().forward_control(r.wdesc, f0, control, ws, bool(batched_gru))

    def forward_audio(self, f0, B, T, phase_u, noise, ws, out=None, wait_event=None, record_event=None, row_blocks=None,
                      on_block=None, block_events=None):
        r = self._wd()
        dev = r.device
        same_device(dev, f0=f0, phase_u=phase_u, noise=noise, workspace=ws, out=out)
        if block_events is not None and (row_blocks is None or len(row_blocks) < 2 or on_block is not None):
            raise RuntimeError("block_events are recorded by the one-call block path only: pass row_blocks of two or more blocks and "
                               "no on_block callback")
        N = T * _lib.HOP
        _, tables, spec, plan_t = self._reverb_aux(N)
        b = binding()
        audio = (r.wdesc, f0, phase_u, r.rand_phase, noise, r.fir_design, plan_t, tables, spec, ws, self.osc_sample_rate())
        if row_blocks is None or len(row_blocks) < 2:
            return b.forward_audio(*audio, out, wait_event.cuda_event if wait_event is not None else 0,
                                   record_event.cuda_event if record_event is not None else 0)
        nxt = 0
        for k, (row0, nrows) in enumerate(row_blocks):
            if int(row0) != nxt or int(nrows) <= 0 or (int(nrows) % 2 and k != len(row_blocks) - 1):
                raise RuntimeError(f"row_blocks must tile [0, {B}) in order, even sizes except the last, got {list(row_blocks)}")
            nxt += int(nrows)
        if nxt != B:
            raise RuntimeError(f"row_blocks cover {nxt} of {B} rows: {list(row_blocks)}")
        if wait_event is not None or record_event is not None:
            raise RuntimeError("wait_event / record_event hook the single-call form; they cannot be combined with row_blocks")
        if block_events is not None and len(block_events) != len(row_blocks):
            raise RuntimeError("block_events: one torch.cuda.Event per row block")
        with torch.cuda.device(dev):
            if out is None:
                out = torch.empty((B, N), dtype=torch.float32, device=dev)
            if block_events is not None:
                for ev in block_events:
                    if not ev.cuda_event:
                        ev.record()
                b.forward_audio_blocks(*audio, out, [int(r0) for r0, _ in row_blocks], [int(n) for _, n in row_blocks],
                                       [int(ev.cuda_event) for ev in block_events])
                return out
            b.forward_audio_pre(*audio)
            for row0, nrows in row_blocks:
                b.forward_reverb_rows(r.fir_design, plan_t, tables, spec, ws, T, int(row0), int(nrows), out)
                if on_block is not None:
                    on_block(int(row0), int(nrows), out)
        return out

    def forward(self, f0, control, phase_u, noise):
        if not self.specialised():
            return self.generic.forward(f0, control, phase_u, noise)
        r = self._wd()
        dev = r.device
        same_device(dev, f0=f0, control=control, phase_u=phase_u, noise=noise)
        B, _, T = control.shape
        plan, tables, spec, plan_t = self._reverb_aux(T * _lib.HOP)
        key = (B, T, stream_ptr(dev))
        ws = self._workspaces.get(key)
        if ws is None:
            nbytes = _lib.lib().nws_forward_workspace_bytes(C.byref(plan), B, T)
            ws = torch.empty(nbytes, dtype=torch.uint8, device=dev)
            if len(self._workspaces) >= 16:
                self._workspaces.pop(next(iter(self._workspaces)))
            self._workspaces[key] = ws
        return binding().forward(r.wdesc, f0, control, phase_u, r.rand_phase, noise, r.fir_design, plan_t, tables, spec, ws,
                                 self.osc_sample_rate())
```

### neural-waveshaping-synthesis_amd/pipeline.py

```python
from __future__ import annotations

import os

import torch

from . import _lib
from .engine import _req


class _Slot:
    __slots__ = ("ws", "ev_control", "ev_audio", "ev_exciter", "used", "keep", "pu", "nz")

    def __init__(self):
        self.ws = None
        self.pu = None
        self.nz = None
        self.ev_control = torch.cuda.Event()
        self.ev_audio = torch.cuda.Event()
        self.ev_exciter = torch.cuda.Event()
        self.used = False
        self.keep = None


_PLACED = {}
# ... 144 lines not shown
                          f"every kernel launch slows down by an order of magnitude; 16 is what this package is measured with",
                          RuntimeWarning, stacklevel=2)
        got, kept = None, []
        with torch.cuda.device(key):
            if mode != "order" and not os.environ.get("NWS_STREAM_ORDER"):
                got = _place_by_measurement(d, rep)
                kept = rep.pop("spare", [])
                if got is None or not rep.get("verified"):
                    rep["ok"] = False
                    warnings.warn(f"ForwardPipeline: no verified placement of the stream set on the command processor's pipes ({rep}); "
                                  f"{'falling back to first-use order' if got is None else 'using the unverified choice'} - the step can "
                                  f"be 12-35 % slower", RuntimeWarning, stacklevel=2)
            if got is None:
                rep["mode"] = "order" if (mode == "order" or os.environ.get("NWS_STREAM_ORDER")) else "order (fallback)"
                got = _place_in_fixed_order(d, rep)
                got = got[:3] + (got[3] + kept,)
        pl.exchange, pl.audio, pl.control, pl.spare = got
        pl.audio_anchors = rep.pop("_audio_anchors", None)
        pl.side = []
        pl.cur = torch.cuda.current_stream(d)
        rep["ms"] = round((time.perf_counter() - t0) * 1e3, 2)
        pl.report = rep
        _PLACED[key] = pl
    return pl.exchange, pl.audio[:audio_streams], pl.control[:control_streams]


def side_streams(dev, n: int, max_candidates: int = 0):
    d = torch.device(dev)
    key = d.index if d.index is not None else torch.cuda.current_device()
    placed_streams(d)
    pl = _PLACED[key]
    max_candidates = max_candidates or 2 * n + 2
    rep = pl.report.setdefault("side", {"kept": 0, "rejected": 0, "plain": 0, "reused": 0})
    with torch.cuda.device(key):
        if len(pl.side) < n and pl.audio_anchors:
            touch = torch.zeros(64, device=d)
            scratch = torch.zeros(4, dtype=torch.int64, device=d)
            torch.cuda.synchronize(d)
            while len(pl.side) < n and rep["kept"] + rep["rejected"] < max_candidates:
                st = torch.cuda.Stream(device=d)
                _first_use(st, touch)
                if any(_blocks(h, st, scratch) for h in pl.audio_anchors):
                    pl.spare.append(st)
                    rep["rejected"] += 1
                else:
                    pl.side.append(st)
                    rep["kept"] += 1
        if len(pl.side) < n:
            if pl.side and pl.audio_anchors:
                k = len(pl.side)
                rep["reused"] = n - k
                return [pl.side[i % k] for i in range(n)]
            while len(pl.side) < n:
                pl.side.append(torch.cuda.Stream(device=d))
                rep["plain"] += 1
    return pl.side[:n]


def placement_report(dev=None):
    d = torch.device(dev if dev is not None else "cuda")
    pl = _PLACED.get(d.index if d.index is not None else torch.cuda.current_device())
    return dict(pl.report) if pl is not None else None


def verify_placement(dev=None):
    d = torch.device(dev if dev is not None else "cuda")
    key = d.index if d.index is not None else torch.cuda.current_device()
    pl = _PLACED[key]
    with torch.cuda.device(key):
        scratch = torch.zeros(4, dtype=torch.int64, device=d)
        torch.cuda.synchronize(d)
        named = {"cur": pl.cur, "x": pl.exchange, "a0": pl.audio[0], "a1": pl.audio[1]}
        want = {"c0 blocks cur": True, "c0 blocks x": False, "c0 blocks a0": False, "c0 blocks a1": False,
                "c1 blocks cur": False, "c1 blocks x": True, "c1 blocks a0": False, "c1 blocks a1": False}
        seen = {k: _blocks(pl.control[int(k[1])], named[k.split()[-1]], scratch) for k in want}
    return {"ok": seen == want, "seen": seen, "want": want}


class ForwardPipeline:

    def __init__(self, model, depth: int = 4, audio_streams: int = 2, control_streams: int = 2, batched_gru: bool = False,
                 chain_exciters: bool = False, streams=None):
        if depth < 2 or audio_streams < 1 or control_streams < 1:
            raise ValueError("need depth >= 2 and at least one stream of each kind")
        self.model = model
        self.eng = model._engine
        _, _, dev = self.eng.weights()
        self.dev = dev
        if streams is not None:
            xs, au, co = streams
            if not au or not co:
                raise ValueError("streams=(exchange, audio streams, control streams) needs at least one stream of each kind")
            self.exchange, self.audio, self.control = xs, list(au), list(co)
            audio_streams = len(self.audio)
        else:
            self.exchange, self.audio, self.control = placed_streams(dev, audio_streams, control_streams)
        self.slots = [_Slot() for _ in range(depth)]
        self.batched_gru = batched_gru
        self.chain_exciters = bool(chain_exciters) and audio_streams > 1
        self._last_exciter = None
        self._n = 0
        self._shape = None
        self._outstanding = []

    def _prepare(self, B, T):
        if self._shape != (B, T):
            self.synchronize()
            for s in self.slots:
                s.ws = self.eng.new_workspace(B, T)
                s.used = False
                s.pu = torch.empty(_lib.N_HARMONICS, dtype=torch.float32, device=self.dev)
                s.nz = torch.empty(_lib.HOP * T - 1, dtype=torch.float32, device=self.dev)
            self._shape = (B, T)

    def next_audio_stream(self):
        return self.audio[self._n % len(self.audio)]

    @staticmethod
    def row_blocks(B: int, chunks: int):
        if chunks <= 1 or B % chunks or (B // chunks) % 2 or B // chunks < 4:
            return None
        n = B // chunks
        return [(q * n, n) for q in range(chunks)]

    def submit(self, f0, control, *, phase_u=None, noise=None, out=None, row_blocks=None, on_block=None, generator=None,
               block_events=None):
        m = self.model
        f0 = _req(f0 if f0.is_contiguous() else f0.contiguous(), "f0")
        control = _req(control if control.is_contiguous() else control.contiguous(), "control")
        if f0.dim() != 3 or f0.shape[1] != 1 or control.dim() != 3 or control.shape[1] < 2:
            raise RuntimeError(f"expected f0 (B,1,T) and control (B,C>=2,T), got {tuple(f0.shape)} / {tuple(control.shape)}")
        B, _, T = f0.shape
        if control.shape[0] != B or control.shape[2] != T or T < 2:
            raise RuntimeError("f0 and control disagree on batch / frames (or fewer than 2 frames)")
        if block_events is not None and (self.chain_exciters or on_block is not None or row_blocks is None or len(row_blocks) < 2):
            raise ValueError("block_events are recorded by the one-call block path only: they need row_blocks of two or more blocks, "
                             "no on_block callback and chain_exciters off")
        self._prepare(B, T)
        i = self._n
        self._n += 1
        slot = self.slots[i % len(self.slots)]
        cs = self.control[i % len(self.control)]
        au = self.audio[i % len(self.audio)]
        batched = bool(self.batched_gru)
        ready = torch.cuda.current_stream(self.dev).record_event()
        with torch.cuda.stream(cs):
            cs.wait_event(ready)
            if slot.used:
                cs.wait_event(slot.ev_audio)
            pu = torch.rand(_lib.N_HARMONICS, out=slot.pu, generator=generator) if phase_u is None else phase_u
            pu = _req(pu.reshape(-1), "phase_u", _lib.N_HARMONICS)
            nz = torch.rand(m.control_hop * T - 1, out=slot.nz, generator=generator) if noise is None else noise
            nz = _req(nz, "noise", m.control_hop * T - 1)
            self.eng.forward_control(f0, control, slot.ws, batched_gru=batched)
            slot.ev_control.record(cs)
        with torch.cuda.stream(au):
            au.wait_event(ready)
            au.wait_event(slot.ev_control)
            if self.chain_exciters:
                out = self.eng.forward_audio(f0, B, T, pu, nz, slot.ws, out=out, wait_event=self._last_exciter,
                                             record_event=slot.ev_exciter)
                self._last_exciter = slot.ev_exciter
            else:
                out = self.eng.forward_audio(f0, B, T, pu, nz, slot.ws, out=out, row_blocks=row_blocks, on_block=on_block,
                                             block_events=block_events)
            slot.ev_audio.record(au)
        slot.used = True
        slot.keep = (f0, control, pu, nz)
        self._outstanding.append((out, slot.ev_audio))
        if len(self._outstanding) > len(self.slots):
            del self._outstanding[:-len(self.slots)]
        return out

    def join_current_stream(self):
        cur = torch.cuda.current_stream(self.dev)
        for out, ev in self._outstanding[-len(self.slots):]:
            cur.wait_event(ev)
            out.record_stream(cur)
        self._outstanding.clear()

    def synchronize(self):
        for s in self.audio + self.control:
            s.synchronize()
        self._outstanding.clear()
```

Before: 10.73 billion samples/s.

## Precompute noise spectra on control stream and reuse them in the FIR noise kernel

Moves the FFT of the shared noise signal out of the per-utterance FIR-noise spectral kernel into a separate noise_spectra kernel launched on the control stream alongside the GRU. The spectral kernel gains a PREP template variant that loads the precomputed spectra from global memory instead of recomputing them in wave 0, and drops one block barrier. The noise is shared across the batch, so the old kernel recomputed the same spectra in every block, and wave 0's FFT serialized the block. The cost is an extra workspace buffer, an extra launch, and a cross-stream dependency.

```diff
diff --git a/include/nws_hip.h b/include/nws_hip.h
--- a/include/nws_hip.h
+++ b/include/nws_hip.h
@@ -111,6 +111,11 @@
 int nws_fir_noise_window(const float* fir, const float* noise, int noise_len, int origin, const float* add_in, int B, int T,
                          float* out, void* stream);
 
+size_t nws_noise_spectra_bytes(int T);
+int nws_noise_spectra(const float* noise , int T, void* spectra_out, void* stream);
+int nws_fir_noise_prepared(const float* fir, const float* noise, const void* spectra, const float* add_in, int B, int T,
+                           float* out , void* stream);
+
 int nws_fir_noise_grad(const float* noise , const float* grad_out , int B, int T,
                        float* grad_fir , void* stream);
 int nws_fir_from_h_grad(const float* grad_fir , const float* fir_design , int B, int T,
@@ -218,6 +223,14 @@
 int nws_forward_audio(const NwsWeights* w, const NwsForwardAux* aux, const float* f0, int B, int T, float sample_rate,
                       const float* phase_u, const float* rand_phase, const float* noise, float* out, void* workspace,
                       size_t workspace_bytes, void* stream);
+
+#define NWS_AUDIO_NOISE_SPECTRA_READY 1u
+int nws_forward_control_noise(const NwsWeights* w, const float* f0, const float* control, const float* noise, int B, int C, int T,
+                              int batched_gru, void* workspace, size_t workspace_bytes, void* stream);
+int nws_forward_audio_flags(const NwsWeights* w, const NwsForwardAux* aux, const float* f0, int B, int T, float sample_rate,
+                            const float* phase_u, const float* rand_phase, const float* noise, float* out, void* workspace,
+                            size_t workspace_bytes, void* stream, void* wait_before_exciter, void* record_after_exciter,
+                            unsigned flags);
 
 int nws_forward_audio_ev(const NwsWeights* w, const NwsForwardAux* aux, const float* f0, int B, int T, float sample_rate,
                          const float* phase_u, const float* rand_phase, const float* noise, float* out, void* workspace,
diff --git a/neural-waveshaping-synthesis_amd/_cops.py b/neural-waveshaping-synthesis_amd/_cops.py
--- a/neural-waveshaping-synthesis_amd/_cops.py
+++ b/neural-waveshaping-synthesis_amd/_cops.py
@@ -105,6 +105,28 @@
                                                   ptr(phase_u), ptr(rand_phase), ptr(noise), ptr(out), ptr(workspace),
                                                   workspace.numel(), _stream(f0.device), wait_event or None, record_event or None),
                   "nws_forward_audio_ev")
+        return out
+
+    def forward_control_noise(self, wdesc, f0, control, noise, workspace, batched_gru):
+        B, Cc, T = control.shape
+        if noise.numel() != HOP * T - 1:
+            raise RuntimeError(f"noise: expected {HOP * T - 1} elements, got {tuple(noise.shape)}")
+        with torch.cuda.device(f0.device):
+            check(_lib.lib().nws_forward_control_noise(C.byref(_struct(wdesc, NwsWeights)), ptr(f0), ptr(control), ptr(noise), B, Cc, T,
+                                                       1 if batched_gru else 0, ptr(workspace), workspace.numel(),
+                                                       _stream(f0.device)), "nws_forward_control_noise")
+
+    def forward_audio_flags(self, wdesc, f0, phase_u, rand_phase, noise, fir_design, plan, reverb_tables, reverb_spectrum, workspace,
+                            sample_rate, out, wait_event, record_event, flags):
+        B, _, T = f0.shape
+        aux = _aux(fir_design, plan, reverb_tables, reverb_spectrum)
+        with torch.cuda.device(f0.device):
+            if out is None:
+                out = _new(f0, B, T * HOP)
+            check(_lib.lib().nws_forward_audio_flags(C.byref(_struct(wdesc, NwsWeights)), C.byref(aux), ptr(f0), B, T, sample_rate,
+                                                     ptr(phase_u), ptr(rand_phase), ptr(noise), ptr(out), ptr(workspace),
+                                                     workspace.numel(), _stream(f0.device), wait_event or None, record_event or None,
+                                                     int(flags)), "nws_forward_audio_flags")
         return out
 
     def forward_audio_pre(self, wdesc, f0, phase_u, rand_phase, noise, fir_design, plan, reverb_tables, reverb_spectrum,
@@ -196,6 +218,24 @@
             else:
                 check(_lib.lib().nws_fir_noise_window(ptr(fir), ptr(noise), noise.numel(), origin, ptr(add_in), B, T, ptr(out),
                                                       _stream(fir.device)), "nws_fir_noise_window")
+        return out
+
+    def noise_spectra(self, noise, T):
+        if T < 1 or noise.numel() != HOP * T - 1:
+            raise RuntimeError(f"noise_spectra: noise {tuple(noise.shape)} must hold the {HOP * T - 1} samples of {T} frames")
+        with torch.cuda.device(noise.device):
+            out = _new(noise, _lib.lib().nws_noise_spectra_bytes(T) // 4)
+            check(_lib.lib().nws_noise_spectra(ptr(noise), T, ptr(out), _stream(noise.device)), "nws_noise_spectra")
+        return out
+
+    def fir_noise_prepared(self, fir, noise, spectra, add_in):
+        B, T, _ = fir.shape
+        if spectra.numel() * 4 != _lib.lib().nws_noise_spectra_bytes(T):
+            raise RuntimeError(f"spectra: expected the {_lib.lib().nws_noise_spectra_bytes(T)} bytes of noise_spectra(noise, {T})")
+        with torch.cuda.device(fir.device):
+            out = _new(fir, B, T * HOP)
+            check(_lib.lib().nws_fir_noise_prepared(ptr(fir), ptr(noise), ptr(spectra), ptr(add_in), B, T, ptr(out),
+                                                    _stream(fir.device)), "nws_fir_noise_prepared")
         return out
 
     def fir_from_h(self, H, fir_design):
diff --git a/neural-waveshaping-synthesis_amd/_lib.py b/neural-waveshaping-synthesis_amd/_lib.py
--- a/neural-waveshaping-synthesis_amd/_lib.py
+++ b/neural-waveshaping-synthesis_amd/_lib.py
@@ -14,6 +14,7 @@
 EXCITER_HYBRID = 4
 EXCITER_HYBRID_W = 8
 EXCITER_BANK_NOFRACT = 16
+AUDIO_NOISE_SPECTRA_READY = 1
 N_HARMONICS = 101
 N_SHAPERS = 64
 HIDDEN = 128
@@ -112,6 +113,9 @@
     "nws_fir_design_matrix": (C.c_int, [_fp, _fp, _fp]),
     "nws_fir_noise": (C.c_int, [_fp, _fp, _fp, C.c_int, C.c_int, _fp, _fp]),
     "nws_fir_noise_window": (C.c_int, [_fp, _fp, C.c_int, C.c_int, _fp, C.c_int, C.c_int, _fp, _fp]),
+    "nws_noise_spectra_bytes": (C.c_size_t, [C.c_int]),
+    "nws_noise_spectra": (C.c_int, [_fp, C.c_int, _fp, _fp]),
+    "nws_fir_noise_prepared": (C.c_int, [_fp, _fp, _fp, _fp, C.c_int, C.c_int, _fp, _fp]),
     "nws_fir_noise_grad": (C.c_int, [_fp, _fp, C.c_int, C.c_int, _fp, _fp]),
     "nws_fir_from_h_grad": (C.c_int, [_fp, _fp, C.c_int, C.c_int, _fp, _fp]),
     "nws_sum_batch_time": (C.c_int, [_fp, C.c_int, C.c_int, C.c_int, _fp, _fp]),
@@ -139,6 +143,10 @@
                               C.c_float, _fp, _fp, _fp, _fp, _fp, C.c_size_t, _fp]),
     "nws_forward_control_bytes": (C.c_size_t, [C.c_int, C.c_int]),
     "nws_forward_control": (C.c_int, [C.POINTER(NwsWeights), _fp, _fp, C.c_int, C.c_int, C.c_int, C.c_int, _fp, C.c_size_t, _fp]),
+    "nws_forward_control_noise": (C.c_int, [C.POINTER(NwsWeights), _fp, _fp, _fp, C.c_int, C.c_int, C.c_int, C.c_int, _fp, C.c_size_t,
+                                            _fp]),
+    "nws_forward_audio_flags": (C.c_int, [C.POINTER(NwsWeights), C.POINTER(NwsForwardAux), _fp, C.c_int, C.c_int, C.c_float,
+                                          _fp, _fp, _fp, _fp, _fp, C.c_size_t, _fp, _fp, _fp, C.c_uint]),
     "nws_forward_audio": (C.c_int, [C.POINTER(NwsWeights), C.POINTER(NwsForwardAux), _fp, C.c_int, C.c_int, C.c_float,
                                     _fp, _fp, _fp, _fp, _fp, C.c_size_t, _fp]),
     "nws_forward_audio_ev": (C.c_int, [C.POINTER(NwsWeights), C.POINTER(NwsForwardAux), _fp, C.c_int, C.c_int, C.c_float,
diff --git a/neural-waveshaping-synthesis_amd/csrc/fir_noise.hip b/neural-waveshaping-synthesis_amd/csrc/fir_noise.hip
--- a/neural-waveshaping-synthesis_amd/csrc/fir_noise.hip
+++ b/neural-waveshaping-synthesis_amd/csrc/fir_noise.hip
@@ -171,10 +171,61 @@
   sp_fft256<false>(z, tw, x, l);
 }
 
+__device__ __forceinline__ void sp_noise_spectra(const float* __restrict__ noise, int len, int origin, int N, int ta, int l,
+                                                 const float* tw, float* xs, float4* sd) {
+  C16 z;
+#pragma unroll
+  for (int j = 0; j < 16; ++j) {
+    const int i0 = kHop * ta + 16 * j + l, i1 = i0 + kHop;
+    const bool in0 = i0 >= 0 && i0 < N + kL - 1, in1 = i1 >= 0 && i1 < N + kL - 1;
+    const float v0 = padded_noise(noise, len, origin, in0 ? i0 : origin);
+    const float v1 = padded_noise(noise, len, origin, in1 ? i1 : origin);
+    z.re[j] = in0 ? v0 : 0.0f;
+    z.im[j] = in1 ? v1 : 0.0f;
+  }
+  sp_fft256<false>(z, tw, xs, l);
+  float mr[16], mi[16];
+  auto mirror = [&](const float (&v)[16], float (&m)[16]) {
+#pragma unroll
+    for (int j = 0; j < 16; ++j) xs[l + 16 * j] = v[j];
+    sp_wave_sync();
+#pragma unroll
+    for (int j = 0; j < 16; ++j) m[j] = xs[(256 - (l + 16 * j)) & 255];
+    sp_wave_sync();
+  };
+  mirror(z.re, mr);
+  mirror(z.im, mi);
+  const float c = (l & 1) ? -(1.0f / 512.0f) : (1.0f / 512.0f);
+#pragma unroll
+  for (int j = 0; j < 9; ++j)
+    sd[16 * j + l] = make_float4(c * (z.re[j] + mr[j]), c * (z.im[j] - mi[j]), c * (z.re[j] - mr[j]), c * (z.im[j] + mi[j]));
+}
+
+constexpr int kSpRunSd = kSpPairs * 9 * 16;
+
+__global__ __launch_bounds__(64) void noise_spectra_kernel(const float* __restrict__ noise, int T, int len, int origin,
+                                                           float4* __restrict__ spectra) {
+  __shared__ __attribute__((aligned(16))) float4 tws[256];
+  __shared__ float xs[kSpPairs][kSpPlane];
+  const int lane = threadIdx.x, g = lane >> 4, l = lane & 15;
+  for (int e = lane; e < 256; e += 64) {
+    float c, s;
+    sp_twiddle((e & 15) * (e >> 4), c, s);
+    tws[e] = make_float4(c, c, s, s);
+  }
+  __syncthreads();
+  const int run = blockIdx.x;
+  const int ta = run * kSpHops - 1 + 2 * g;
+  sp_noise_spectra(noise, len, origin, T * kHop, ta, l, reinterpret_cast<const float*>(&tws[l]), xs[g],
+                   spectra + (size_t)run * kSpRunSd + g * (9 * 16));
+}
+
+template <bool PREP>
 __global__ __launch_bounds__(64 * kSpWaves, 3) void fir_noise_spectral_kernel(const float* __restrict__ fir,
                                                                              const float* __restrict__ noise,
                                                                              const float* __restrict__ add_in, int B, int T, int len,
-                                                                             int origin, float* __restrict__ out, int nruns, int total) {
+                                                                             int origin, float* __restrict__ out, int nruns, int total,
+                                                                             const float4* __restrict__ spectra) {
   __shared__ __attribute__((aligned(16))) SpectralLds L;
   const int tid = threadIdx.x, lane = tid & 63, wave = tid >> 6;
   const int g = lane >> 4, l = lane & 15;
@@ -189,6 +240,13 @@
   const bool oka = ta >= 0 && ta < T, okb = tb < T;
   const int tac = ta < 0 ? 0 : (ta < T ? ta : T - 1), tbc = tb < T ? tb : T - 1;
 
+  float4 sdv[3];
+  if constexpr (PREP) {
+    const float4* sp = spectra + (size_t)run * kSpRunSd;
+    sdv[0] = sp[tid];
+    sdv[1] = sp[tid + 256];
+    sdv[2] = sp[tid < kSpRunSd - 512 ? tid + 512 : tid];
+  }
   const int bc0 = b0 < B ? b0 : B - 1, bc1 = b1 < B ? b1 : B - 1;
   const float* rowa0 = &fir[((size_t)bc0 * T + tac) * kHalf + l];
   const float* rowb0 = &fir[((size_t)bc0 * T + tbc) * kHalf + l];
@@ -206,38 +264,17 @@
     L.tw[tid] = make_float4(c, c, s, s);
   }
   const float* tw = reinterpret_cast<const float*>(&L.tw[l]);
+  if constexpr (PREP) {
+    float4* sdl = &L.sd[0][0][0];
+    sdl[tid] = sdv[0];
+    sdl[tid + 256] = sdv[1];
+    if (tid < kSpRunSd - 512) sdl[tid + 512] = sdv[2];
+  }
   __syncthreads();
 
   f32x2* x = &L.x[wave][g * kSpPlane];
-  if (wave == 0) {
-    C16 z;
-    float* xs = reinterpret_cast<float*>(x);
-#pragma unroll
-    for (int j = 0; j < 16; ++j) {
-      const int i0 = kHop * ta + 16 * j + l, i1 = i0 + kHop;
-      const bool in0 = i0 >= 0 && i0 < N + kL - 1, in1 = i1 >= 0 && i1 < N + kL - 1;
-      const float v0 = padded_noise(noise, len, origin, in0 ? i0 : origin);
-      const float v1 = padded_noise(noise, len, origin, in1 ? i1 : origin);
-      z.re[j] = in0 ? v0 : 0.0f;
-      z.im[j] = in1 ? v1 : 0.0f;
-    }
-    sp_fft256<false>(z, tw, xs, l);
-    float mr[16], mi[16];
-    auto mirror = [&](const float (&v)[16], float (&m)[16]) {
-#pragma unroll
-      for (int j = 0; j < 16; ++j) xs[l + 16 * j] = v[j];
-      sp_wave_sync();
-#pragma unroll
-      for (int j = 0; j < 16; ++j) m[j] = xs[(256 - (l + 16 * j)) & 255];
-      sp_wave_sync();
-    };
-    mirror(z.re, mr);
-    mirror(z.im, mi);
-    const float c = (l & 1) ? -(1.0f / 512.0f) : (1.0f / 512.0f);
-#pragma unroll
-    for (int j = 0; j < 9; ++j)
-      L.sd[g][j][l] = make_float4(c * (z.re[j] + mr[j]), c * (z.im[j] - mi[j]), c * (z.re[j] - mr[j]), c * (z.im[j] + mi[j]));
-  }
+  if (!PREP && wave == 0)
+    sp_noise_spectra(noise, len, origin, N, ta, l, tw, reinterpret_cast<float*>(x), &L.sd[g][0][0]);
   const f32x2 zero = {0.0f, 0.0f};
 #pragma unroll
   for (int j = 0; j < 8; ++j) {
@@ -246,7 +283,7 @@
   }
   C16T<f32x2> z;
   sp_filter_spectrum(z, ua, ub, tw, x, lane, l);
-  __syncthreads();
+  if constexpr (!PREP) __syncthreads();
 
   const bool has_add = add_in != nullptr;
   const bool sta = g > 0 && ta < T, stb = tb < T;
@@ -313,16 +350,22 @@
 
 }
 
-extern "C" int nws_fir_noise_window(const float* fir, const float* noise, int noise_len, int origin, const float* add_in,
-                                    int B, int T, float* out, void* stream) {
+namespace {
+
+int fir_noise_window(const float* fir, const float* noise, int noise_len, int origin, const float* add_in, int B, int T, float* out,
+                     const float4* spectra, void* stream) {
   if (!fir || !noise || !out || B <= 0 || T <= 0 || noise_len < 2 || origin < 0) return NWS_ERR_BAD_ARG;
   if (B > 65535) return NWS_ERR_UNSUPPORTED;
   if (B >= 16) {
     const long long nruns = (T + kSpHops - 1) / kSpHops, total = nruns * ((B + kSpUtt - 1) / kSpUtt);
     if (total > (1ll << 30)) return NWS_ERR_UNSUPPORTED;
     const dim3 grid((unsigned)(8 * ((total + 7) / 8)));
-    fir_noise_spectral_kernel<<<grid, 64 * kSpWaves, 0, (hipStream_t)stream>>>(fir, noise, add_in, B, T, noise_len, origin, out,
-                                                                             (int)nruns, (int)total);
+    if (spectra != nullptr)
+      fir_noise_spectral_kernel<true><<<grid, 64 * kSpWaves, 0, (hipStream_t)stream>>>(fir, noise, add_in, B, T, noise_len, origin, out,
+                                                                                       (int)nruns, (int)total, spectra);
+    else
+      fir_noise_spectral_kernel<false><<<grid, 64 * kSpWaves, 0, (hipStream_t)stream>>>(fir, noise, add_in, B, T, noise_len, origin, out,
+                                                                                        (int)nruns, (int)total, nullptr);
     NWS_CHECK_LAUNCH();
     return NWS_OK;
   }
@@ -330,6 +373,33 @@
   fir_noise_kernel<false><<<grid, 256, 0, (hipStream_t)stream>>>(fir, noise, add_in, T, noise_len, origin, out, nullptr);
   NWS_CHECK_LAUNCH();
   return NWS_OK;
+}
+
+}
+
+extern "C" int nws_fir_noise_window(const float* fir, const float* noise, int noise_len, int origin, const float* add_in,
+                                    int B, int T, float* out, void* stream) {
+  return fir_noise_window(fir, noise, noise_len, origin, add_in, B, T, out, nullptr, stream);
+}
+
+extern "C" size_t nws_noise_spectra_bytes(int T) {
+  if (T <= 0) return 0;
+  return (size_t)((T + kSpHops - 1) / kSpHops) * kSpRunSd * sizeof(float4);
+}
+
+extern "C" int nws_noise_spectra(const float* noise, int T, void* spectra_out, void* stream) {
+  if (!noise || !spectra_out || T <= 0 || T * kHop - 1 < 2) return NWS_ERR_BAD_ARG;
+  if (T > (1 << 23)) return NWS_ERR_UNSUPPORTED;
+  noise_spectra_kernel<<<(T + kSpHops - 1) / kSpHops, 64, 0, (hipStream_t)stream>>>(noise, T, T * kHop - 1, kL / 2,
+                                                                                  static_cast<float4*>(spectra_out));
+  NWS_CHECK_LAUNCH();
+  return NWS_OK;
+}
+
+extern "C" int nws_fir_noise_prepared(const float* fir, const float* noise, const void* spectra, const float* add_in, int B, int T,
+                                      float* out, void* stream) {
+  if (!spectra) return NWS_ERR_BAD_ARG;
+  return fir_noise_window(fir, noise, T * kHop - 1, kL / 2, add_in, B, T, out, static_cast<const float4*>(spectra), stream);
 }
 
 extern "C" int nws_fir_noise_window_rows(const float* fir, const float* noise, int origin, const int4* rows, int B, int T,
diff --git a/neural-waveshaping-synthesis_amd/csrc/forward.hip b/neural-waveshaping-synthesis_amd/csrc/forward.hip
--- a/neural-waveshaping-synthesis_amd/csrc/forward.hip
+++ b/neural-waveshaping-synthesis_amd/csrc/forward.hip
@@ -44,6 +44,7 @@
   size_t total = 0;
   total += aligned((size_t)B * (N / 32) * sizeof(double));
   total += aligned((size_t)B * T * NWS_HIDDEN * sizeof(float));
+  total += aligned(nws_noise_spectra_bytes(T));
   total += aligned((size_t)B * T * NWS_FILM_CH * sizeof(float));
   total += aligned((size_t)B * T * NWS_FIR_HALF * sizeof(float));
   total += aligned((size_t)B * N * sizeof(float));
@@ -59,6 +60,7 @@
 struct Arena {
   double* carry;
   float *gru_out, *film, *fir, *noise_out, *pre;
+  void* noise_sd;
   void* rv_ws;
   size_t rv_bytes;
   bool ok;
@@ -70,6 +72,7 @@
   Arena a{};
   a.carry = static_cast<double*>(cv.take((size_t)B * (N / 32) * sizeof(double)));
   a.gru_out = static_cast<float*>(cv.take((size_t)B * T * NWS_HIDDEN * sizeof(float)));
+  a.noise_sd = cv.take(nws_noise_spectra_bytes(T));
   if (!head_only) {
     a.film = static_cast<float*>(cv.take((size_t)B * T * NWS_FILM_CH * sizeof(float)));
     a.fir = static_cast<float*>(cv.take((size_t)B * T * NWS_FIR_HALF * sizeof(float)));
@@ -91,10 +94,16 @@
     if (rc != NWS_OK) return rc;                               \
   } while (0)
 
-int control_half(const NwsWeights* w, const float* f0, const float* control, int B, int C, int T, int batched_gru,
-                 const Arena& a, void* stream) {
+bool uses_noise_spectra(int B) { return B >= 16; }
+
+int control_half(const NwsWeights* w, const float* f0, const float* control, const float* noise, int B, int C, int T,
+                 int batched_gru, const Arena& a, void* stream) {
   hipStream_t st = (hipStream_t)stream;
   int rc = NWS_OK;
+  if (noise != nullptr && uses_noise_spectra(B)) {
+    rc = nws_noise_spectra(noise, T, a.noise_sd, stream);
+    if (rc != NWS_OK) return rc;
+  }
   if (batched_gru) {
     NWS_STAGE(0, nws_phase_carry(f0, nullptr, B, T, a.carry, stream));
     NWS_STAGE(1, nws_control_gru_batched(w, control, B, C, T, nullptr, a.gru_out, nullptr, stream));
@@ -107,12 +116,16 @@
 
 int audio_half(const NwsWeights* w, const NwsForwardAux* aux, const float* f0, int B, int T, float sample_rate,
                const float* phase_u, const float* rand_phase, const float* noise, float* out, const Arena& a, void* stream,
-               void* wait_before_exciter = nullptr, void* record_after_exciter = nullptr, bool with_reverb = true) {
+               void* wait_before_exciter = nullptr, void* record_after_exciter = nullptr, bool with_reverb = true,
+               bool noise_spectra_ready = false) {
   hipStream_t st = (hipStream_t)stream;
   int rc = NWS_OK;
   const size_t N = (size_t)T * NWS_HOP;
   NWS_STAGE(2, nws_frame_mlps(w, a.gru_out, aux->fir_design, B, T, nullptr, a.film, nullptr, a.fir, stream));
-  NWS_STAGE(4, nws_fir_noise(a.fir, noise, nullptr, B, T, a.noise_out, stream));
+  if (noise_spectra_ready && uses_noise_spectra(B))
+    NWS_STAGE(4, nws_fir_noise_prepared(a.fir, noise, a.noise_sd, nullptr, B, T, a.noise_out, stream));
+  else
+    NWS_STAGE(4, nws_fir_noise(a.fir, noise, nullptr, B, T, a.noise_out, stream));
   if (wait_before_exciter != nullptr) {
     const hipError_t e = hipStreamWaitEvent(st, (hipEvent_t)wait_before_exciter, 0);
     if (e != hipSuccess) return (int)e;
@@ -151,7 +164,8 @@
 size_t nws_forward_control_bytes(int B, int T) {
   if (B <= 0 || T <= 0) return 0;
   const size_t N = (size_t)T * NWS_HOP;
-  return aligned((size_t)B * (N / 32) * sizeof(double)) + aligned((size_t)B * T * NWS_HIDDEN * sizeof(float));
+  return aligned((size_t)B * (N / 32) * sizeof(double)) + aligned((size_t)B * T * NWS_HIDDEN * sizeof(float)) +
+         aligned(nws_noise_spectra_bytes(T));
 }
 
 int nws_forward(const NwsWeights* w, const NwsForwardAux* aux, const float* f0, const float* control, int B, int C,
@@ -163,7 +177,7 @@
   if (T > (1 << 23) || !nws_reverb_plan_serves(aux->plan, T * NWS_HOP, 0)) return NWS_ERR_BAD_ARG;
   const Arena a = carve_arena(aux->plan, workspace, workspace_bytes, B, T, false);
   if (!a.ok) return NWS_ERR_WORKSPACE;
-  const int rc = control_half(w, f0, control, B, C, T, 0, a, stream);
+  const int rc = control_half(w, f0, control, nullptr, B, C, T, 0, a, stream);
   if (rc != NWS_OK) return rc;
   return audio_half(w, aux, f0, B, T, sample_rate, phase_u, rand_phase, noise, out, a, stream);
 }
@@ -174,7 +188,16 @@
   if (B <= 0 || T < 2 || C < 2) return NWS_ERR_BAD_ARG;
   const Arena a = carve_arena(nullptr, workspace, workspace_bytes, B, T, true);
   if (!a.ok) return NWS_ERR_WORKSPACE;
-  return control_half(w, f0, control, B, C, T, batched_gru, a, stream);
+  return control_half(w, f0, control, nullptr, B, C, T, batched_gru, a, stream);
+}
+
+int nws_forward_control_noise(const NwsWeights* w, const float* f0, const float* control, const float* noise, int B, int C, int T,
+                              int batched_gru, void* workspace, size_t workspace_bytes, void* stream) {
+  if (!w || !f0 || !control || !noise || !workspace) return NWS_ERR_BAD_ARG;
+  if (B <= 0 || T < 2 || C < 2) return NWS_ERR_BAD_ARG;
+  const Arena a = carve_arena(nullptr, workspace, workspace_bytes, B, T, true);
+  if (!a.ok) return NWS_ERR_WORKSPACE;
+  return control_half(w, f0, control, noise, B, C, T, batched_gru, a, stream);
 }
 
 int nws_forward_audio(const NwsWeights* w, const NwsForwardAux* aux, const float* f0, int B, int T, float sample_rate,
@@ -200,6 +223,20 @@
   if (!a.ok) return NWS_ERR_WORKSPACE;
   return audio_half(w, aux, f0, B, T, sample_rate, phase_u, rand_phase, noise, out, a, stream, wait_before_exciter,
                     record_after_exciter);
+}
+
+int nws_forward_audio_flags(const NwsWeights* w, const NwsForwardAux* aux, const float* f0, int B, int T, float sample_rate,
+                            const float* phase_u, const float* rand_phase, const float* noise, float* out, void* workspace,
+                            size_t workspace_bytes, void* stream, void* wait_before_exciter, void* record_after_exciter,
+                            unsigned flags) {
+  if (!w || !aux_ok(aux)) return NWS_ERR_BAD_ARG;
+  if (!f0 || !phase_u || !rand_phase || !noise || !out || !workspace) return NWS_ERR_BAD_ARG;
+  if (B <= 0 || T < 2 || (flags & ~NWS_AUDIO_NOISE_SPECTRA_READY) != 0) return NWS_ERR_BAD_ARG;
+  if (T > (1 << 23) || !nws_reverb_plan_serves(aux->plan, T * NWS_HOP, 0)) return NWS_ERR_BAD_ARG;
+  const Arena a = carve_arena(aux->plan, workspace, workspace_bytes, B, T, false);
+  if (!a.ok) return NWS_ERR_WORKSPACE;
+  return audio_half(w, aux, f0, B, T, sample_rate, phase_u, rand_phase, noise, out, a, stream, wait_before_exciter,
+                    record_after_exciter, true, (flags & NWS_AUDIO_NOISE_SPECTRA_READY) != 0);
 }
 
 int nws_forward_audio_pre(const NwsWeights* w, const NwsForwardAux* aux, const float* f0, int B, int T, float sample_rate,
diff --git a/neural-waveshaping-synthesis_amd/csrc/torch_ops.cpp b/neural-waveshaping-synthesis_amd/csrc/torch_ops.cpp
--- a/neural-waveshaping-synthesis_amd/csrc/torch_ops.cpp
+++ b/neural-waveshaping-synthesis_amd/csrc/torch_ops.cpp
@@ -157,6 +157,48 @@
   nws_check(nws_forward_control(w, f0.data_ptr<float>(), control.data_ptr<float>(), (int)B, (int)C, (int)T, batched_gru ? 1 : 0,
                                 workspace.data_ptr(), (size_t)workspace.numel(), L.stream),
             "nws_forward_control");
+}
+
+void forward_control_noise(const Tensor& wdesc, const Tensor& f0, const Tensor& control, const Tensor& noise, Tensor& workspace,
+                           bool batched_gru) {
+  const NwsWeights* w = weights_of(wdesc);
+  int64_t B, C, T;
+  check_inputs(f0, control, B, C, T);
+  check_dev(noise, "noise");
+  check_same_device(f0, "f0", noise, "noise");
+  TORCH_CHECK(noise.numel() == NWS_HOP * T - 1, "noise: expected ", NWS_HOP * T - 1, " elements, got ", noise.sizes());
+  check_dev(workspace, "workspace", at::kByte);
+  check_same_device(f0, "f0", workspace, "workspace");
+  Launch L(f0);
+  nws_check(nws_forward_control_noise(w, f0.data_ptr<float>(), control.data_ptr<float>(), noise.data_ptr<float>(), (int)B, (int)C, (int)T,
+                                      batched_gru ? 1 : 0, workspace.data_ptr(), (size_t)workspace.numel(), L.stream),
+            "nws_forward_control_noise");
+}
+
+Tensor forward_audio_flags(const Tensor& wdesc, const Tensor& f0, const Tensor& phase_u, const Tensor& rand_phase, const Tensor& noise,
+                           const Tensor& fir_design, const Tensor& plan, const Tensor& reverb_tables, const Tensor& reverb_spectrum,
+                           Tensor& workspace, double sample_rate, const OptTensor& out_opt, int64_t wait_event, int64_t record_event,
+                           int64_t flags) {
+  const NwsWeights* w = weights_of(wdesc);
+  AudioArgs a(f0, phase_u, rand_phase, noise, fir_design, plan, reverb_tables, reverb_spectrum, workspace);
+  const int64_t B = a.B, T = a.T;
+  TORCH_CHECK(flags >= 0 && flags <= NWS_AUDIO_NOISE_SPECTRA_READY, "forward_audio_flags: unknown flags ", flags);
+  Launch L(f0);
+  Tensor out;
+  if (out_opt.has_value()) {
+    out = *out_opt;
+    check_dev(out, "out");
+    check_same_device(f0, "f0", out, "out");
+    TORCH_CHECK(out.dim() == 2 && out.size(0) == B && out.size(1) == T * NWS_HOP, "out: expected (", B, ", ", T * NWS_HOP, ")");
+  } else {
+    out = at::empty({B, T * NWS_HOP}, f0.options());
+  }
+  nws_check(nws_forward_audio_flags(w, &a.aux, f0.data_ptr<float>(), (int)B, (int)T, (float)sample_rate, phase_u.data_ptr<float>(),
+                                    rand_phase.data_ptr<float>(), noise.data_ptr<float>(), out.data_ptr<float>(), workspace.data_ptr(),
+                                    (size_t)workspace.numel(), L.stream, reinterpret_cast<void*>(wait_event),
+                                    reinterpret_cast<void*>(record_event), (unsigned)flags),
+            "nws_forward_audio_flags");
+  return out;
 }
 
 Tensor forward_audio(const Tensor& wdesc, const Tensor& f0, const Tensor& phase_u, const Tensor& rand_phase, const Tensor& noise,
@@ -369,6 +411,39 @@
     nws_check(nws_fir_noise_window(fir.data_ptr<float>(), noise.data_ptr<float>(), (int)noise.numel(), (int)origin, fptr(add_in),
                                    (int)B, (int)T, out.data_ptr<float>(), L.stream), "nws_fir_noise_window");
   }
+  return out;
+}
+
+Tensor noise_spectra(const Tensor& noise, int64_t T) {
+  check_dev(noise, "noise");
+  TORCH_CHECK(T >= 1 && T <= (1 << 23) && noise.numel() == T * NWS_HOP - 1, "noise_spectra: noise ", noise.sizes(), " must hold the ",
+              T * NWS_HOP - 1, " samples of ", T, " frames");
+  Launch L(noise);
+  Tensor out = at::empty({(int64_t)(nws_noise_spectra_bytes((int)T) / sizeof(float))}, noise.options());
+  nws_check(nws_noise_spectra(noise.data_ptr<float>(), (int)T, out.data_ptr(), L.stream), "nws_noise_spectra");
+  return out;
+}
+
+Tensor fir_noise_prepared(const Tensor& fir, const Tensor& noise, const Tensor& spectra, const OptTensor& add_in) {
+  check_dev(fir, "fir");
+  check_dev(noise, "noise");
+  check_dev(spectra, "spectra");
+  check_same_device(fir, "fir", noise, "noise");
+  check_same_device(fir, "fir", spectra, "spectra");
+  TORCH_CHECK(fir.dim() == 3 && fir.size(2) == NWS_FIR_HALF, "fir: expected (B, T, 128) upper half-taps (nws_frame_mlps), got ", fir.sizes());
+  const int64_t B = fir.size(0), T = fir.size(1);
+  TORCH_CHECK(noise.numel() == T * NWS_HOP - 1, "noise: expected ", T * NWS_HOP - 1, " samples, got ", noise.sizes());
+  TORCH_CHECK((size_t)spectra.numel() * sizeof(float) == nws_noise_spectra_bytes((int)T), "spectra: expected the ",
+              nws_noise_spectra_bytes((int)T), " bytes of noise_spectra(noise, ", T, "), got ", spectra.sizes());
+  if (add_in.has_value()) {
+    check_dev(*add_in, "add_in");
+    check_same_device(fir, "fir", *add_in, "add_in");
+    TORCH_CHECK(add_in->numel() == B * T * NWS_HOP, "add_in: expected (", B, ", ", T * NWS_HOP, "), got ", add_in->sizes());
+  }
+  Launch L(fir);
+  Tensor out = at::empty({B, T * NWS_HOP}, fir.options());
+  nws_check(nws_fir_noise_prepared(fir.data_ptr<float>(), noise.data_ptr<float>(), spectra.data_ptr(), fptr(add_in), (int)B, (int)T,
+                                   out.data_ptr<float>(), L.stream), "nws_fir_noise_prepared");
   return out;
 }
 
@@ -1228,6 +1303,11 @@
   m.def("forward(Tensor wdesc, Tensor f0, Tensor control, Tensor phase_u, Tensor rand_phase, Tensor noise, Tensor fir_design, "
         "Tensor plan, Tensor reverb_tables, Tensor reverb_spectrum, Tensor(a!) workspace, float sample_rate) -> Tensor", &forward);
   m.def("forward_control(Tensor wdesc, Tensor f0, Tensor control, Tensor(a!) workspace, bool batched_gru) -> ()", &forward_control);
+  m.def("forward_control_noise(Tensor wdesc, Tensor f0, Tensor control, Tensor noise, Tensor(a!) workspace, bool batched_gru) -> ()",
+        &forward_control_noise);
+  m.def("forward_audio_flags(Tensor wdesc, Tensor f0, Tensor phase_u, Tensor rand_phase, Tensor noise, Tensor fir_design, Tensor plan, "
+        "Tensor reverb_tables, Tensor reverb_spectrum, Tensor(a!) workspace, float sample_rate, Tensor? out, int wait_event, "
+        "int record_event, int flags) -> Tensor", &forward_audio_flags);
   m.def("forward_audio(Tensor wdesc, Tensor f0, Tensor phase_u, Tensor rand_phase, Tensor noise, Tensor fir_design, Tensor plan, "
         "Tensor reverb_tables, Tensor reverb_spectrum, Tensor(a!) workspace, float sample_rate, Tensor? out, int wait_event, "
         "int record_event) -> Tensor", &forward_audio);
@@ -1246,6 +1326,8 @@
   m.def("frame_mlps(Tensor wdesc, Tensor gru_out, Tensor fir_design, bool want_emb, bool want_H) -> (Tensor, Tensor, Tensor, Tensor)",
         &frame_mlps);
   m.def("fir_noise(Tensor fir, Tensor noise, Tensor? add_in, int origin) -> Tensor", &fir_noise);
+  m.def("noise_spectra(Tensor noise, int T) -> Tensor", &noise_spectra);
+  m.def("fir_noise_prepared(Tensor fir, Tensor noise, Tensor spectra, Tensor? add_in) -> Tensor", &fir_noise_prepared);
   m.def("fir_from_h(Tensor H, Tensor fir_design) -> Tensor", &fir_from_h);
   m.def("fir_noise_grad(Tensor noise, Tensor grad_out) -> Tensor", &fir_noise_grad);
   m.def("fir_from_h_grad(Tensor grad_fir, Tensor fir_design) -> Tensor", &fir_from_h_grad);
diff --git a/neural-waveshaping-synthesis_amd/engine.py b/neural-waveshaping-synthesis_amd/engine.py
--- a/neural-waveshaping-synthesis_amd/engine.py
+++ b/neural-waveshaping-synthesis_amd/engine.py
@@ -443,6 +443,13 @@
         nz = noise if noise_len is None or noise_len == noise.numel() else noise[:noise_len]
         return binding().fir_noise(fir, nz, add_in, -1 if origin is None else int(origin))
 
+    def noise_spectra(self, noise, T):
+        return binding().noise_spectra(noise, int(T))
+
+    def fir_noise_prepared(self, fir, noise, spectra, add_in=None):
+        same_device(fir.device, noise=noise, spectra=spectra, add_in=add_in)
+        return binding().fir_noise_prepared(fir, noise, spectra, add_in)
+
     def reverb(self, x):
         same_device(self._wd().device, x=x)
         _, tables, spec, plan_t = self._reverb_aux(x.shape[1])
@@ -472,13 +479,16 @@
         plan, _, _, _ = self._reverb_aux(T * _lib.HOP)
         return torch.empty(_lib.lib().nws_forward_workspace_bytes(C.byref(plan), B, T), dtype=torch.uint8, device=dev)
 
-    def forward_control(self, f0, control, ws, batched_gru=True):
-        r = self._wd()
-        same_device(r.device, f0=f0, control=control, workspace=ws)
-        binding().forward_control(r.wdesc, f0, control, ws, bool(batched_gru))
+    def forward_control(self, f0, control, ws, batched_gru=True, noise=None):
+        r = self._wd()
+        same_device(r.device, f0=f0, control=control, workspace=ws, noise=noise)
+        if noise is None:
+            binding().forward_control(r.wdesc, f0, control, ws, bool(batched_gru))
+        else:
+            binding().forward_control_noise(r.wdesc, f0, control, noise, ws, bool(batched_gru))
 
     def forward_audio(self, f0, B, T, phase_u, noise, ws, out=None, wait_event=None, record_event=None, row_blocks=None,
-                      on_block=None, block_events=None):
+                      on_block=None, block_events=None, noise_spectra_ready=False):
         r = self._wd()
         dev = r.device
         same_device(dev, f0=f0, phase_u=phase_u, noise=noise, workspace=ws, out=out)
@@ -490,8 +500,10 @@
         b = binding()
         audio = (r.wdesc, f0, phase_u, r.rand_phase, noise, r.fir_design, plan_t, tables, spec, ws, self.osc_sample_rate())
         if row_blocks is None or len(row_blocks) < 2:
-            return b.forward_audio(*audio, out, wait_event.cuda_event if wait_event is not None else 0,
-                                   record_event.cuda_event if record_event is not None else 0)
+            events = (wait_event.cuda_event if wait_event is not None else 0, record_event.cuda_event if record_event is not None else 0)
+            if noise_spectra_ready:
+                return b.forward_audio_flags(*audio, out, *events, _lib.AUDIO_NOISE_SPECTRA_READY)
+            return b.forward_audio(*audio, out, *events)
         nxt = 0
         for k, (row0, nrows) in enumerate(row_blocks):
             if int(row0) != nxt or int(nrows) <= 0 or (int(nrows) % 2 and k != len(row_blocks) - 1):
diff --git a/neural-waveshaping-synthesis_amd/pipeline.py b/neural-waveshaping-synthesis_amd/pipeline.py
--- a/neural-waveshaping-synthesis_amd/pipeline.py
+++ b/neural-waveshaping-synthesis_amd/pipeline.py
@@ -320,18 +320,19 @@
             pu = _req(pu.reshape(-1), "phase_u", _lib.N_HARMONICS)
             nz = torch.rand(m.control_hop * T - 1, out=slot.nz, generator=generator) if noise is None else noise
             nz = _req(nz, "noise", m.control_hop * T - 1)
-            self.eng.forward_control(f0, control, slot.ws, batched_gru=batched)
+            prepared = row_blocks is None or len(row_blocks) < 2
+            self.eng.forward_control(f0, control, slot.ws, batched_gru=batched, noise=nz if prepared else None)
             slot.ev_control.record(cs)
         with torch.cuda.stream(au):
             au.wait_event(ready)
             au.wait_event(slot.ev_control)
             if self.chain_exciters:
                 out = self.eng.forward_audio(f0, B, T, pu, nz, slot.ws, out=out, wait_event=self._last_exciter,
-                                             record_event=slot.ev_exciter)
+                                             record_event=slot.ev_exciter, noise_spectra_ready=prepared)
                 self._last_exciter = slot.ev_exciter
             else:
                 out = self.eng.forward_audio(f0, B, T, pu, nz, slot.ws, out=out, row_blocks=row_blocks, on_block=on_block,
-                                             block_events=block_events)
+                                             block_events=block_events, noise_spectra_ready=prepared)
             slot.ev_audio.record(au)
         slot.used = True
         slot.keep = (f0, control, pu, nz)
```

New measurement: 10.76 billion samples/s, median of 6. About the same (+0.3%).
